# RozDavid/UnScene3D

Measured on AMD Instinct MI355X. Metric: training scenes/sec (Res16UNet34C+Mask3D, 150k voxels), higher is better.
Workload: dtype f32

## Files before the change

### include/usc3d.h

```cpp
#ifndef USC3D_H
#define USC3D_H

#include <stdint.h>

#ifdef __cplusplus
extern "C" {
#endif

typedef void* usc_stream_t;

enum usc_status {
  USC_OK = 0,
  USC_ERR_ARG = -1,
  USC_ERR_LAUNCH = -2,
  USC_ERR_RANGE = -3
};

const char* usc_last_error(void);
int usc_abi_version(void);
const char* usc_build_info(void);
int usc_device_count(void);


int usc_voxel_floor_f64(const double* xyz, int64_t n, double voxel_size,
// ... 167 lines not shown
int usc_conv_backward(const usc_kmap* m, int32_t kind, const float* x,
                      int32_t cin, const float* W, int32_t cout,
                      const float* dy, float* dx, int32_t dx_accumulate,
                      float* dW, int32_t dW_accumulate, void* ws,
                      int64_t ws_bytes, usc_stream_t s);
int usc_bn_eval_stats(const float* gamma, const float* beta,
                      const float* running_mean, const float* running_var,
                      float eps, int32_t c, float* mean, float* invstd,
                      float* scale, float* shift, usc_stream_t s);
int usc_conv_bn_act_forward(const usc_kmap* m, int32_t kind, const float* x,
                            int32_t cin, const float* W, int32_t cout,
                            const usc_bn* bn, const float* residual,
                            int32_t relu, float* y, float* stats, float* out,
                            void* ws, int64_t ws_bytes, usc_stream_t s);
int usc_conv_bn_act_backward(const usc_kmap* m, int32_t kind, const float* x,
                             int32_t cin, const float* W, int32_t cout,
                             const usc_bn* bn, const float* y,
                             const float* stats, const float* out_relu,
                             const float* dout, float* dy, float* dres,
                             float* dx, int32_t dx_accumulate, float* dW,
                             int32_t dW_accumulate, float* dgamma,
                             float* dbeta, int32_t dbn_accumulate, void* ws,
                             int64_t ws_bytes, usc_stream_t s);
int64_t usc_unit_bf16_ws_bytes(const usc_kmap* m, int32_t kind, int32_t cin,
                               int32_t cout);
int usc_conv_bn_act_forward_bf16(const usc_kmap* m, int32_t kind,
                                 const float* x, int32_t cin,
                                 const uint16_t* Wp, int32_t cout,
                                 const usc_bn* bn, const float* residual,
                                 int32_t relu, float* y, float* stats,
                                 float* out, void* ws, int64_t ws_bytes,
                                 usc_stream_t s);

int64_t usc_unit_split_ws_bytes(const usc_kmap* m, int32_t kind, int32_t cin,
                                int32_t cout, int32_t P);
int usc_conv_bn_act_forward_split(const usc_kmap* m, int32_t kind,
                                  const float* x, int32_t cin, const float* W,
                                  int32_t cout, int32_t P, const usc_bn* bn,
                                  const float* residual, int32_t relu, float* y,
                                  float* stats, float* out, void* ws,
                                  int64_t ws_bytes, usc_stream_t s);
int usc_conv_bn_act_backward_split(const usc_kmap* m, int32_t kind,
                                   const float* x, int32_t cin, const float* W,
                                   int32_t cout, int32_t P, const usc_bn* bn,
                                   const float* y, const float* stats,
                                   const float* out_relu, const float* dout,
                                   float* dy, float* dres, float* dx,
                                   int32_t dx_accumulate, float* dW,
                                   int32_t dW_accumulate, float* dgamma,
                                   float* dbeta, int32_t dbn_accumulate,
                                   void* ws, int64_t ws_bytes, usc_stream_t s);

enum usc_step_op { USC_STEP_UNIT_FWD = 0, USC_STEP_UNIT_BWD = 1, USC_STEP_CAT = 2, USC_STEP_SPLIT = 3, USC_STEP_ADD = 4,
                   USC_STEP_UNIT_FWD_BF16 = 5 };
typedef struct usc_step {
  int32_t op, kind, cin, cout, relu;
  int32_t dx_accumulate, dW_accumulate, dbn_accumulate, defer_wgrad, accumulate;
  const usc_kmap* map;
  const usc_bn* bn;
  const float* x;
  const float* W;
  const float* residual;
  float* y;
  float* stats;
  float* out;
  const float* dout;
  float* dy;
  float* dres;
  float* dx;
  float* dW;
  float* dgamma;
  float* dbeta;
  const float* a;
  const float* b;
  float* dst;
  float* dst2;
  int64_t n;
  int32_t ca, cb;
  int32_t split_planes, reserved;
} usc_step;
int32_t usc_step_size(void);
int64_t usc_program_ws_bytes(const usc_step* steps, int32_t n_steps);
int usc_program_run(const usc_step* steps, int32_t begin, int32_t end, void* ws, int64_t ws_bytes, usc_stream_t s);


int64_t usc_colstats_ws_bytes(int64_t n, int32_t c);
int usc_colstats(const float* x, const float* y, int64_t n, int32_t c,
                 double* sum1, double* sum2, void* ws, int64_t ws_bytes,
                 usc_stream_t s);
int usc_bn_forward_stats(const float* x, int64_t n, int32_t c, const float* gamma,
                         const float* beta, float eps, float momentum,
                         float* running_mean, float* running_var, int64_t* num_batches_tracked, float* mean,
                         float* invstd, float* scale, float* shift, void* ws,
                         int64_t ws_bytes, usc_stream_t s);
int usc_bn_apply(const float* x, const float* scale, const float* shift,
                 const float* residual, int32_t relu, float* y, int64_t n,
                 int32_t c, usc_stream_t s);
int usc_bn_backward_dx(const float* x, const float* dy, const float* y_out,
                       const float* mean, const float* invstd,
                       const float* gamma, const float* mean_g,
                       const float* mean_gxhat, float* dx, float* dres,
                       int64_t n, int32_t c, usc_stream_t s);
int64_t usc_bn_tile_max_rows(void);
int64_t usc_bn_plan(int64_t n, int32_t c, int32_t backward);
int usc_bn_tile_ok(int64_t n, int32_t c);
int64_t usc_bn_tile_ws_bytes(int32_t c);
int usc_bn_tile_forward(const float* partial, int32_t G, float* y, int64_t n,
                        int32_t c, const float* gamma, const float* beta,
                        float eps, float momentum, float* running_mean,
                        float* running_var, int64_t* num_batches_tracked,
                        float* mean, float* invstd, float* scale, float* shift,
                        const float* residual, int32_t relu, float* out,
                        void* ws, int64_t ws_bytes, usc_stream_t s);
int usc_bn_tile_backward(const float* partial, int32_t G, int32_t accumulate,
                         float* dout, const float* y, const float* y_out,
                         const float* mean, const float* invstd,
                         const float* gamma, int64_t n, int32_t c,
                         int32_t training, int32_t dbn_accumulate,
                         float* dgamma, float* dbeta, float* dy, float* dres,
                         void* ws, int64_t ws_bytes, usc_stream_t s);
int usc_bn_backward_reduce(const float* x, const float* dy, const float* y_out,
                           const float* mean, const float* invstd, int64_t n,
                           int32_t c, int32_t training, int32_t accumulate, float* dgamma,
                           float* dbeta, float* mean_g, float* mean_gxhat,
                           void* ws, int64_t ws_bytes, usc_stream_t s);
int usc_relu_fwd(const float* x, float* y, int64_t numel, usc_stream_t s);
int usc_relu_bwd(const float* y, const float* dy, float* dx, int64_t numel,
                 usc_stream_t s);

int usc_avgpool_down2(const float* in, int32_t c, const int32_t* nbr2,
                      int64_t n_coarse, float* out, usc_stream_t s);
int usc_avgpool_down2_ex(const float* in, int32_t c, int32_t ld,
                         const int64_t* row_of, const int32_t* nbr2,
                         int64_t n_coarse, float* out, uint8_t* mask_out,
                         usc_stream_t s);

int usc_gather_rows(const float* src, int32_t c, const int64_t* idx, int64_t n,
                    float* out, usc_stream_t s);

int usc_scatter_add_rows(const float* src, int32_t c, const int64_t* idx,
                         int64_t n, float* dst, usc_stream_t s);

int usc_scatter_rows_unique(const float* src, int32_t c, const int64_t* idx,
                            int64_t n, float* dst, usc_stream_t s);
int usc_scatter_rows_unique_add(const float* src, int32_t c, const int64_t* idx,
                                int64_t n, float* dst, usc_stream_t s);

int64_t usc_sample_keys_ws_bytes(int32_t n_scenes, int32_t K, int32_t q);
int usc_sample_keys(const float* feats, int32_t c, const uint8_t* mask, int32_t q, const float* pos, int32_t p,
                    const int64_t* idx, int32_t n_scenes, int32_t K, const int32_t* n_valid, float* out_feats,
                    uint8_t* out_mask, float* out_pos, void* ws, int64_t ws_bytes, usc_stream_t s);

int64_t usc_segment_csr_ws_bytes(int64_t n, int64_t S);
int usc_segment_csr(const int64_t* seg, int64_t n, int64_t S, int64_t* order,
                    int64_t* seg_off, void* ws, int64_t ws_bytes,
                    usc_stream_t s);
int usc_segment_mean_fwd(const float* src, int32_t c, const int64_t* order,
                         const int64_t* seg_off, int64_t S, float* out,
                         usc_stream_t s);
int usc_segment_mean_bwd(const float* dout, int32_t c, const int64_t* seg,
                         const int64_t* seg_off, int64_t n, float* dsrc,
                         usc_stream_t s);

int usc_segment_mean_nonzero(const float* feats, int32_t d,
                             const int64_t* order, const int64_t* seg_off,
                             int64_t S, float* out, int64_t* nonzero_cnt,
                             usc_stream_t s);
int usc_segment_max_nonzero(const float* feats, int32_t d,
                            const int64_t* order, const int64_t* seg_off,
                            int64_t S, float* out, int64_t* nonzero_cnt,
                            usc_stream_t s);

int32_t usc_attn_max_queries(void);
int32_t usc_attn_lse_stride(int32_t L);
int64_t usc_attn_ws_bytes(int32_t L, int32_t S, int32_t B, int32_t H);
int usc_attn_fwd(const float* q, const float* k, const float* v,
                 const uint8_t* mask, int32_t L, int32_t S, int32_t B, int32_t H,
                 int32_t E, float* o, float* lse, void* ws, int64_t ws_bytes,
                 usc_stream_t s);
int usc_attn_bwd(const float* q, const float* k, const float* v,
                 const uint8_t* mask, const float* o, const float* lse,
                 const float* dO, int32_t L, int32_t S, int32_t B, int32_t H,
                 int32_t E, float* dq, float* dk, float* dv,
                 int32_t mask_bits_in_ws ,
                 void* ws, int64_t ws_bytes, usc_stream_t s);

int usc_self_attn_fwd(const float* q, const float* k, const float* v, int32_t L,
                      int32_t B, int32_t H, int32_t E, float* o, float* lse,
                      usc_stream_t s);
int usc_self_attn_bwd(const float* q, const float* k, const float* v, const float* o,
                      const float* lse, const float* dO, int32_t L, int32_t B,
                      int32_t H, int32_t E, float* dq, float* dk, float* dv,
                      usc_stream_t s);

int usc_lsap_batch(const float* cost, int32_t n_prob, int32_t nr, int32_t nc,
                   int64_t* row_ind, int64_t* col_ind, int32_t* status, usc_stream_t s);

int64_t usc_criterion_ws_bytes(int32_t L, int32_t S, int32_t T);
int64_t usc_criterion_ws_bytes_q(int32_t L, int32_t S, int32_t T, int32_t Q);
int usc_criterion_target_bits(const uint8_t* tm, int32_t T, int32_t max_targets, int32_t S,
                              uint32_t* bits, int32_t* cnt, usc_stream_t s);
int usc_criterion_costs(const float* const* masks, int32_t L, int32_t ld, int32_t S,
                        int32_t Q, int32_t T, int32_t max_targets, const uint32_t* bits,
                        const int32_t* cnt, const float* logits, int64_t ls_level, int64_t ls_q,
                        int32_t C, const int64_t* labels, float w_mask, float w_class,
                        float w_dice, float* cost, float* cmask, float* cdice, float* nmat,
                        float* ssum, float* logp, void* ws, int64_t ws_bytes, usc_stream_t s);
int usc_criterion_drop_counts(const float* const* masks, int32_t L, int32_t ld, int32_t S,
                              int32_t Q, int32_t T, int32_t max_targets, const uint32_t* bits,
                              const int64_t* src, const int64_t* tid, int32_t* counts,
                              usc_stream_t s);
int usc_criterion_losses(const float* cmask, const float* cdice, const float* logp,
                         const int64_t* src, const int64_t* tid, const int64_t* labels,
                         const float* class_w, int32_t L, int32_t Q, int32_t T,
                         int32_t max_targets, int32_t C, int32_t noobj, int32_t* tcls, float* part,
                         const int32_t* counts, const int32_t* cnt, float thresh, float* wts,
                         usc_stream_t s);
int usc_criterion_table(const float* parts, int32_t B, int32_t L, float* table,
                        float* den_tot, usc_stream_t s);
int usc_criterion_backward(const float* const* masks, float* const* dmasks, int32_t L,
                           int32_t ld, int32_t S, int32_t Q, int32_t T, int32_t max_targets,
                           const uint32_t* bits, const int32_t* cnt, const int64_t* src,
                           const int64_t* tid, const float* nmat, const float* ssum,
                           const float* logp, const int32_t* tcls, const float* class_w,
                           const float* gtable, const float* den_tot, int32_t C, int64_t ls_level,
                           int64_t ls_q, float* dlogits, const float* wts, usc_stream_t s);

int usc_linear_fwd(const float* x, const float* W, const float* b, int32_t M,
                   int32_t N, int32_t K, float* y, usc_stream_t s);
int usc_linear_bwd(const float* dy, const float* x, const float* W, int32_t M,
                   int32_t N, int32_t K, float* dx, float* dW, float* db,
                   int32_t accumulate, usc_stream_t s);
int usc_linear_fwd_ex(const float* x, const float* x2, const float* W,
                      const float* b, int32_t M, int32_t N, int32_t K,
                      int32_t relu, float* y, usc_stream_t s);
int usc_linear_fwd_pad(const float* x, const float* x2, const float* W, const float* b, int32_t M, int32_t N, int32_t K,
                       int32_t relu, float* y, int32_t M_pad, usc_stream_t s);
int usc_linear_fwd_split(const float* x, const float* x2, const float* W, const float* b, int32_t M, int32_t N, int32_t K,
                         int32_t x2_cols, int32_t split_cols, float* y, usc_stream_t s);
int usc_linear_bwd_ex(const float* dy, const float* y_relu, const float* x,
                      const float* x2, const float* W, int32_t M, int32_t N,
                      int32_t K, float* dx, const float* dx_add, float* dW,
                      float* db, int32_t accumulate, usc_stream_t s);
int usc_linear_bwd_ex2(const float* dy, const float* y_relu, const float* x, const float* x2, const float* W, int32_t M,
                       int32_t N, int32_t K, float* dx, const float* dx_add, const float* dx_add2, float* dx_b, float* dW,
                       float* db, int32_t accumulate, usc_stream_t s);
int usc_qkv_proj_bwd(const float* dy3, const float* x, const float* pos, const float* W, int32_t M, int32_t E, float* dx,
                     float* dx_b, const float* dres, float* dW, float* db, int32_t accumulate, usc_stream_t s);
int64_t usc_col_sum_ws_bytes(int64_t n, int32_t c);
int usc_col_sum(const float* x, int64_t n, int32_t c, float* out,
                int32_t accumulate, void* ws, int64_t ws_bytes, usc_stream_t s);

int usc_layernorm_fwd(const float* x, const float* gamma, const float* beta,
                      int64_t rows, int32_t d, float eps, float* y, float* mean,
                      float* rstd, usc_stream_t s);
int usc_add_layernorm_fwd(const float* x, const float* res, const float* gamma,
                          const float* beta, int64_t rows, int32_t d, float eps,
                          float* y, float* sum_out, float* mean, float* rstd,
                          usc_stream_t s);
int64_t usc_layernorm_bwd_ws_bytes(int64_t rows, int32_t d);
int usc_layernorm_bwd(const float* dy, const float* x, const float* mean,
                      const float* rstd, const float* gamma, int64_t rows,
                      int32_t d, float* dx, float* dgamma, float* dbeta,
                      int32_t accumulate, void* ws, int64_t ws_bytes,
                      usc_stream_t s);
int usc_layernorm_bwd_ex(const float* dy, const float* x, const float* mean,
                         const float* rstd, const float* gamma, int64_t rows,
                         int32_t d, const float* dx_add, float* dx, float* dgamma,
                         float* dbeta, int32_t accumulate, void* ws,
                         int64_t ws_bytes, usc_stream_t s);

int usc_furthest_point_sampling(const float* xyz, int32_t b, int32_t n,
                                int32_t m, float* tmp, int32_t* idx,
                                usc_stream_t s);

int usc_fourier_posenc(const float* xyz, int64_t n, const float* lo,
                       const float* hi, const float* gauss_B, int32_t d,
                       float* out, usc_stream_t s);

int usc_ncut_similarity(const float* F, int64_t S, int32_t d,
                        int32_t cosine_mode, float* normed, float* sim,
                        usc_stream_t s);
int usc_ncut_similarity_masked(const float* F, const uint8_t* zero_rows, int64_t S,
                               int32_t d, int32_t cosine_mode, float* normed,
                               float* sim, usc_stream_t s);
int usc_ncut_normalize_mat(float* A, int64_t S, void* ws, int64_t ws_bytes,
                           usc_stream_t s);
int usc_ncut_binarize(const float* simA, const float* simB, int64_t S, float tau,
                      double eps, const uint8_t* painted, uint8_t* Abin,
                      double* deg, usc_stream_t s);
int64_t usc_ncut_fiedler_ws_bytes(int64_t S);
int usc_ncut_fiedler(const uint8_t* Abin, const double* deg, int64_t S, double eps,
                     double* evec, double* eval, void* ws, int64_t ws_bytes,
                     usc_stream_t s);
int usc_ncut_fiedler_ex(const uint8_t* Abin, const double* deg, int64_t S, double eps,
                        double* evec, double* eval, void* ws, int64_t ws_bytes,
                        usc_stream_t s, int32_t flags);
int32_t usc_ncut_fiedler_plan(int64_t S, int32_t cus, int32_t flags);

int usc_knn1(const float* query, int64_t nq, const float* ref, int64_t nr,
             int64_t* idx, float* dist2, usc_stream_t s);

int usc_cc_eps_init(int32_t* label, int64_t n, usc_stream_t s);
int usc_cc_eps_step(const float* xyz, int64_t n, float eps,
                    const int32_t* label_in, int32_t* label_out,
                    int32_t* changed, usc_stream_t s);
int usc_cc_eps_finish(const int32_t* label, int64_t n, int32_t* rank_ws,
                      int64_t* labels, usc_stream_t s);

int usc_project_planes_fwd(const int32_t* coords, const float* pred,
                           const float* target, int64_t V, int32_t inst,
                           int32_t dim_x, int32_t dim_y, int32_t dim_z,
                           float* pred_xy, float* pred_xz, float* pred_yz,
                           float* tgt_xy, float* tgt_xz, float* tgt_yz,
                           int32_t* cnt_xy, int32_t* cnt_xz, int32_t* cnt_yz,
                           usc_stream_t s);
int usc_project_planes_bwd(const int32_t* coords, int64_t V, int32_t inst,
                           int32_t dim_x, int32_t dim_y, int32_t dim_z,
                           const float* g_xy, const float* g_xz,
                           const float* g_yz, float* grad_pred,
                           usc_stream_t s);

int usc_brick_mask_build(const int32_t* coords, int64_t n, const int32_t* shift, int32_t B,
                         int32_t bricks_x, int32_t bricks_y, int32_t bricks_z,
                         uint32_t* mask, usc_stream_t s);
int usc_raycast_first_hit_map(const uint64_t* table_keys, const int32_t* table_vals,
                              int64_t cap, int64_t n_rows, const int32_t* shift,
                              const uint32_t* brick_mask , int32_t bricks_x,
                              int32_t bricks_y, int32_t bricks_z,
// ... 114 lines not shown
```

### unscene3d_amd/_lib.py

```python
from __future__ import annotations

import ctypes as C
import os

import torch

_HERE = os.path.dirname(os.path.abspath(__file__))
LIB_PATH = os.environ.get("USC3D_LIB") or os.path.join(_HERE, "libusc3d_hip.so")

_p = C.c_void_p
_i32 = C.c_int32
_i64 = C.c_int64
_f64 = C.c_double
_f32 = C.c_float

class KMap(C.Structure):
    _fields_ = [("nbr", _p), ("perm", _p), ("tile_mask", _p), ("pair_in", _p), ("pair_out", _p), ("koff", _p),
                ("n_in", _i64), ("n_out", _i64), ("pair_capacity", _i64), ("K", _i32), ("reserved", _i32)]


class BNDesc(C.Structure):
    _fields_ = [("gamma", _p), ("beta", _p), ("running_mean", _p), ("running_var", _p), ("num_batches_tracked", _p),
                ("eps", _f32), ("momentum", _f32), ("c", _i32), ("training", _i32)]


_kp = C.POINTER(KMap)
_bp = C.POINTER(BNDesc)


class Step(C.Structure):
    _fields_ = [("op", _i32), ("kind", _i32), ("cin", _i32), ("cout", _i32), ("relu", _i32),
                ("dx_accumulate", _i32), ("dW_accumulate", _i32), ("dbn_accumulate", _i32), ("defer_wgrad", _i32),
                ("accumulate", _i32),
                ("map", _p), ("bn", _p),
                ("x", _p), ("W", _p), ("residual", _p), ("y", _p), ("stats", _p), ("out", _p),
                ("dout", _p), ("dy", _p), ("dres", _p), ("dx", _p), ("dW", _p), ("dgamma", _p), ("dbeta", _p),
                ("a", _p), ("b", _p), ("dst", _p), ("dst2", _p), ("n", _i64), ("ca", _i32), ("cb", _i32),
                ("split_planes", _i32), ("reserved", _i32)]


_sp = C.POINTER(Step)
STEP_UNIT_FWD, STEP_UNIT_BWD, STEP_CAT, STEP_SPLIT, STEP_ADD, STEP_UNIT_FWD_BF16 = 0, 1, 2, 3, 4, 5

SIGNATURES = {
    "usc_last_error": (C.c_char_p, []),
    "usc_abi_version": (C.c_int, []),
    "usc_build_info": (C.c_char_p, []),
    "usc_device_count": (C.c_int, []),
    "usc_voxel_floor_f64": (C.c_int, [_p, _i64, _f64, _p, _p]),
    "usc_voxel_floor_f64_host": (C.c_int, [_p, _i64, C.c_double, _p]),
    "usc_unique_coords_host": (C.c_int, [_p, _i64, _i32, _p, _p, _p]),
    "usc_coordmap_capacity": (_i64, [_i64]),
    "usc_coordmap_ws_bytes": (_i64, [_i64]),
    "usc_coordmap_build": (C.c_int, [_p, _i64, _i32, _p, _p, _i64, _p, _p, _p, _p, _p, _i64, _p]),
    "usc_morton_cell_ids": (C.c_int, [_p, _i64, _i32, _i32, _i32, _i32, _i32, _p, _p]),
    "usc_kernel_map_cube": (C.c_int, [_p, _i64, _i32, _i32, _p, _p, _i64, _p, _p]),
    "usc_kernel_map_down2": (C.c_int, [_p, _i64, _i32, _p, _p, _i64, _p, _p, _p]),
    "usc_rulebook_ws_bytes": (_i64, [_i64, _i64]),
    "usc_rulebook_compact": (C.c_int, [_p, _i64, _i64, _p, _p, _p, _p, _i64, _p]),
    "usc_weight_transpose": (C.c_int, [_p, _i32, _i32, _i32, _i32, _p, _p]),
    "usc_spconv_plan": (C.c_int, [_i32, _i64, _i32, _i32, _i32]),
    "usc_spconv_gather_gemm_ws_bytes": (_i64, [_i64, _i32, _i32, _i32]),
    "usc_spconv_gather_gemm": (C.c_int, [_p, _i64, _i32, _p, _i32, _i32, _p, _i64, _p, _p, _i32, _i32, _p, _i64, _p]),
    "usc_rowsort_ws_bytes": (_i64, [_i32, _i64]),
    "usc_rowsort_build": (C.c_int, [_p, _i32, _i64, _p, _p, _p, _i64, _p]),
    "usc_spconv_sorted_ws_bytes": (_i64, [_i64, _i32, _i32, _i32]),
    "usc_spconv_sorted_gemm": (C.c_int, [_p, _i64, _i32, _p, _i32, _i32, _p, _p, _p, _i64, _p, _p, _i32, _i32, _p, _i64, _p]),
    "usc_spconv_sorted_gemm_ex": (C.c_int, [_p, _i64, _i32, _p, _i32, _i32, _p, _p, _p, _i64, _p, _p, _i32, _i32, _p, _i64, _p, _p]),
    "usc_group_reduce": (C.c_int, [_p, _i32, _i64, _i32, _p, _i32, _p, _p]),
    "usc_bn_tile_max_rows": (C.c_int64, []),
    "usc_bn_plan": (_i64, [_i64, _i32, _i32]),
    "usc_bn_tile_ok": (C.c_int, [_i64, _i32]),
    "usc_bn_tile_ws_bytes": (C.c_int64, [_i32]),
    "usc_bn_tile_forward": (C.c_int, [_p, _i32, _p, _i64, _i32, _p, _p, _f32, _f32, _p, _p, _p, _p, _p, _p, _p, _p, _i32, _p,
                                      _p, _i64, _p]),
    "usc_bn_tile_backward": (C.c_int, [_p, _i32, _i32, _p, _p, _p, _p, _p, _p, _i64, _i32, _i32, _i32, _p, _p, _p, _p, _p,
                                       _i64, _p]),
    "usc_spconv_pairs_gemm": (C.c_int, [_p, _i32, _p, _i32, _i32, _p, _p, _p, _i64, _p, _p]),
    "usc_cast_bf16": (C.c_int, [_p, _i64, _p, _p]),
    "usc_spconv_pack_w_bf16": (C.c_int, [_p, _i32, _i32, _i32, _p, _p]),
    "usc_spconv_gather_gemm_bf16_ws_bytes": (_i64, [_i64, _i32, _i32, _i32]),
    "usc_spconv_gather_gemm_bf16": (C.c_int, [_p, _i64, _i32, _p, _i32, _i32, _p, _i64, _p, _p, _i32, _p, _i64, _p]),
    "usc_split_bf16_rows": (C.c_int, [_p, _i64, _i32, _i32, _p, _p]),
    "usc_split_bf16": (C.c_int, [_p, _i64, _i32, _p, _p]),
    "usc_spconv_pack_w_split": (C.c_int, [_p, _i32, _i32, _i32, _i32, _i32, _p, _p]),
    "usc_spconv_gather_gemm_split_ws_bytes": (_i64, [_i64, _i32, _i32, _i32, _i32]),
    "usc_spconv_gather_gemm_split": (C.c_int, [_p, _i64, _i32, _p, _i32, _i32, _i32, _p, _i64, _p, _p, _i32, _p, _i64, _p]),
    "usc_spconv_wgrad_ws_bytes": (_i64, [_i32, _i32, _i32]),
    "usc_spconv_wgrad": (C.c_int, [_p, _i32, _p, _i32, _i32, _p, _p, _p, _i64, _p, _i32, _p, _i64, _p]),
    "usc_spconv_wgrad_ws_bytes_rows": (_i64, [_i32, _i32, _i32, _i64]),
    "usc_step_size": (_i32, []),
    "usc_program_ws_bytes": (_i64, [_sp, _i32]),
    "usc_program_run": (C.c_int, [_sp, _i32, _i32, _p, _i64, _p]),
    "usc_spconv_wgrad_group_max": (_i32, []),
    "usc_spconv_wgrad_grid_limit": (None, [_i32]),
    "usc_spconv_wgrad_group_ok": (C.c_int, [_i32, _i32, _i32, _i32, _i64]),
    "usc_spconv_wgrad_group": (C.c_int, [_i32, _p, _p, _p, _i32, _i32, _i32, _p, _p, _p, _i64, _i32, _p]),
    "usc_spconv_wgrad_table_ws_bytes": (_i64, [_i32, _i32, _i32]),
    "usc_spconv_wgrad_table": (C.c_int, [_p, _i32, _p, _i32, _p, _i32, _i64, _p, _i32, _p, _i64, _p]),
    "usc_set_wgrad_lane": (C.c_int, [_p, _p, _i64, _i64]),
    "usc_wgrad_lane_join": (C.c_int, [_p]),
    "usc_wgrad_lane_hold": (C.c_int, [_i32, _i64, _i64, _p]),
    "usc_wgrad_lane_holding": (_i32, []),
    "usc_launch_stats_begin": (C.c_int, [_p, _i64, _p]),
    "usc_launch_stats_end": (_i64, [_p, _i64]),
    "usc_wall_clock_khz": (_i64, []),
    "usc_conv_ws_bytes": (_i64, [_kp, _i32, _i32, _i32]),
    "usc_unit_ws_bytes": (_i64, [_kp, _i32, _i32, _i32]),
    "usc_conv_forward": (C.c_int, [_kp, _i32, _p, _i32, _p, _i32, _p, _p, _p, _i64, _p]),
    "usc_conv_backward": (C.c_int, [_kp, _i32, _p, _i32, _p, _i32, _p, _p, _i32, _p, _i32, _p, _i64, _p]),
    "usc_bn_eval_stats": (C.c_int, [_p, _p, _p, _p, _f32, _i32, _p, _p, _p, _p, _p]),
    "usc_conv_bn_act_forward": (C.c_int, [_kp, _i32, _p, _i32, _p, _i32, _bp, _p, _i32, _p, _p, _p, _p, _i64, _p]),
    "usc_unit_bf16_ws_bytes": (_i64, [_kp, _i32, _i32, _i32]),
    "usc_conv_bn_act_forward_bf16": (C.c_int, [_kp, _i32, _p, _i32, _p, _i32, _bp, _p, _i32, _p, _p, _p, _p, _i64, _p]),
    "usc_unit_split_ws_bytes": (_i64, [_kp, _i32, _i32, _i32, _i32]),
    "usc_conv_bn_act_forward_split": (C.c_int, [_kp, _i32, _p, _i32, _p, _i32, _i32, _bp, _p, _i32, _p, _p, _p, _p, _i64, _p]),
    "usc_conv_bn_act_backward_split": (C.c_int, [_kp, _i32, _p, _i32, _p, _i32, _i32, _bp, _p, _p, _p, _p, _p, _p, _p, _i32, _p,
                                                 _i32, _p, _p, _i32, _p, _i64, _p]),
    "usc_conv_bn_act_backward": (C.c_int, [_kp, _i32, _p, _i32, _p, _i32, _bp, _p, _p, _p, _p, _p, _p, _p, _i32, _p,
                                           _i32, _p, _p, _i32, _p, _i64, _p]),
    "usc_colstats_ws_bytes": (_i64, [_i64, _i32]),
    "usc_colstats": (C.c_int, [_p, _p, _i64, _i32, _p, _p, _p, _i64, _p]),
    "usc_bn_apply": (C.c_int, [_p, _p, _p, _p, _i32, _p, _i64, _i32, _p]),
    "usc_bn_backward_dx": (C.c_int, [_p, _p, _p, _p, _p, _p, _p, _p, _p, _p, _i64, _i32, _p]),
    "usc_bn_backward_reduce": (C.c_int, [_p, _p, _p, _p, _p, _i64, _i32, _i32, _i32, _p, _p, _p, _p, _p, _i64, _p]),
    "usc_bn_forward_stats": (C.c_int, [_p, _i64, _i32, _p, _p, _f32, _f32, _p, _p, _p, _p, _p, _p, _p, _p, _i64, _p]),
    "usc_relu_fwd": (C.c_int, [_p, _p, _i64, _p]),
    "usc_relu_bwd": (C.c_int, [_p, _p, _p, _i64, _p]),
    "usc_avgpool_down2": (C.c_int, [_p, _i32, _p, _i64, _p, _p]),
    "usc_avgpool_down2_ex": (C.c_int, [_p, _i32, _i32, _p, _p, _i64, _p, _p, _p]),
    "usc_gather_rows": (C.c_int, [_p, _i32, _p, _i64, _p, _p]),
    "usc_scatter_add_rows": (C.c_int, [_p, _i32, _p, _i64, _p, _p]),
    "usc_scatter_rows_unique": (C.c_int, [_p, _i32, _p, _i64, _p, _p]),
    "usc_scatter_rows_unique_add": (C.c_int, [_p, _i32, _p, _i64, _p, _p]),
    "usc_sample_keys_ws_bytes": (_i64, [_i32, _i32, _i32]),
    "usc_sample_keys": (C.c_int, [_p, _i32, _p, _i32, _p, _i32, _p, _i32, _i32, _p, _p, _p, _p, _p, _i64, _p]),
    "usc_segment_csr_ws_bytes": (_i64, [_i64, _i64]),
    "usc_segment_csr": (C.c_int, [_p, _i64, _i64, _p, _p, _p, _i64, _p]),
    "usc_segment_mean_fwd": (C.c_int, [_p, _i32, _p, _p, _i64, _p, _p]),
    "usc_segment_mean_bwd": (C.c_int, [_p, _i32, _p, _p, _i64, _p, _p]),
    "usc_segment_mean_nonzero": (C.c_int, [_p, _i32, _p, _p, _i64, _p, _p, _p]),
    "usc_segment_max_nonzero": (C.c_int, [_p, _i32, _p, _p, _i64, _p, _p, _p]),
    "usc_ncut_similarity": (C.c_int, [_p, _i64, _i32, _i32, _p, _p, _p]),
    "usc_ncut_similarity_masked": (C.c_int, [_p, _p, _i64, _i32, _i32, _p, _p, _p]),
    "usc_ncut_normalize_mat": (C.c_int, [_p, _i64, _p, _i64, _p]),
    "usc_ncut_binarize": (C.c_int, [_p, _p, _i64, _f32, _f64, _p, _p, _p, _p]),
    "usc_ncut_fiedler_ws_bytes": (_i64, [_i64]),
    "usc_ncut_fiedler": (C.c_int, [_p, _p, _i64, _f64, _p, _p, _p, _i64, _p]),
    "usc_ncut_fiedler_ex": (C.c_int, [_p, _p, _i64, _f64, _p, _p, _p, _i64, _p, _i32]),
    "usc_ncut_fiedler_plan": (_i32, [_i64, _i32, _i32]),
    "usc_knn1": (C.c_int, [_p, _i64, _p, _i64, _p, _p, _p]),
    "usc_cc_eps_init": (C.c_int, [_p, _i64, _p]),
    "usc_cc_eps_step": (C.c_int, [_p, _i64, _f32, _p, _p, _p, _p]),
    "usc_cc_eps_finish": (C.c_int, [_p, _i64, _p, _p, _p]),
    "usc_project_planes_fwd": (C.c_int, [_p, _p, _p, _i64, _i32, _i32, _i32, _i32] + [_p] * 10),
    "usc_project_planes_bwd": (C.c_int, [_p, _i64, _i32, _i32, _i32, _i32, _p, _p, _p, _p, _p]),
    "usc_brick_mask_build": (C.c_int, [_p, _i64, _p, _i32, _i32, _i32, _i32, _p, _p]),
    "usc_raycast_first_hit_map": (C.c_int, [_p, _p, _i64, _i64, _p, _p, _i32, _i32, _i32, _p, _p, _i32, _i32, _i32, _i32,
                                            _f32, _f32, _f32, _p, _p, _p]),
    "usc_raycast_first_hit_dense": (C.c_int, [_p, _i32, _i32, _i32, _i64, _p, _p, _i32, _i32, _i32, _i32, _f32, _f32,
                                              _f32, _p, _p, _p]),
    "usc_project_reduce": (C.c_int, [_p, _i32, _p, _p, _i64, _i32, _p, _p, _p]),
    "usc_project_fuse_tokens": (C.c_int, [_p, _i32, _i32, _i32, _i32, _i32, _i32, _p, _p, _i64, _p, _p, _p]),
    "usc_project_predictions": (C.c_int, [_p, _i32, _p, _i64, _p, _p]),
    "usc_unproject_depth": (C.c_int, [_p, _p, _p, _i32, _i32, _i32, _p, _p]),
    "usc_spin": (C.c_int, [_i64, C.c_int, _p]),
    "usc_adamw_step": (C.c_int, [_p, _p, _p, _p, _i64, _f32, _f32, _f32, _f32, _f32, _i64, _p]),
    "usc_adamw_step_scaled": (C.c_int, [_p, _p, _p, _p, _i64, _f32, _i32, _f32, _f32, _f32, _f32, _f32, _i64, _p]),
    "usc_elastic_displace": (C.c_int, [_p, _i32, _i64, _i32, _p, _i32, _i32, _i32, _p, _p, _p, _f64, _p, _p]),
    "usc_attn_max_queries": (_i32, []),
    "usc_attn_lse_stride": (_i32, [_i32]),
    "usc_attn_ws_bytes": (_i64, [_i32, _i32, _i32, _i32]),
    "usc_attn_fwd": (C.c_int, [_p, _p, _p, _p, _i32, _i32, _i32, _i32, _i32, _p, _p, _p, _i64, _p]),
    "usc_attn_bwd": (C.c_int, [_p, _p, _p, _p, _p, _p, _p, _i32, _i32, _i32, _i32, _i32, _p, _p, _p, _i32, _p, _i64, _p]),
    "usc_lsap_batch": (C.c_int, [_p, _i32, _i32, _i32, _p, _p, _p, _p]),
    "usc_criterion_ws_bytes": (_i64, [_i32, _i32, _i32]),
    "usc_criterion_ws_bytes_q": (_i64, [_i32, _i32, _i32, _i32]),
    "usc_criterion_target_bits": (C.c_int, [_p, _i32, _i32, _i32, _p, _p, _p]),
    "usc_criterion_costs": (C.c_int, [_p, _i32, _i32, _i32, _i32, _i32, _i32, _p, _p, _p, _i64, _i64, _i32, _p, _f32, _f32,
                                      _f32, _p, _p, _p, _p, _p, _p, _p, _i64, _p]),
    "usc_criterion_drop_counts": (C.c_int, [_p, _i32, _i32, _i32, _i32, _i32, _i32, _p, _p, _p, _p, _p]),
    "usc_criterion_losses": (C.c_int, [_p, _p, _p, _p, _p, _p, _p, _i32, _i32, _i32, _i32, _i32, _i32, _p, _p, _p, _p,
                                       _f32, _p, _p]),
    "usc_criterion_table": (C.c_int, [_p, _i32, _i32, _p, _p, _p]),
    "usc_criterion_backward": (C.c_int, [_p, _p, _i32, _i32, _i32, _i32, _i32, _i32, _p, _p, _p, _p, _p, _p, _p, _p, _p,
                                         _p, _p, _i32, _i64, _i64, _p, _p, _p]),
    "usc_self_attn_fwd": (C.c_int, [_p, _p, _p, _i32, _i32, _i32, _i32, _p, _p, _p]),
    "usc_self_attn_bwd": (C.c_int, [_p, _p, _p, _p, _p, _p, _i32, _i32, _i32, _i32, _p, _p, _p, _p]),
    "usc_linear_fwd": (C.c_int, [_p, _p, _p, _i32, _i32, _i32, _p, _p]),
    "usc_linear_bwd": (C.c_int, [_p, _p, _p, _i32, _i32, _i32, _p, _p, _p, _i32, _p]),
    "usc_layernorm_fwd": (C.c_int, [_p, _p, _p, _i64, _i32, _f32, _p, _p, _p, _p]),
    "usc_add_layernorm_fwd": (C.c_int, [_p, _p, _p, _p, _i64, _i32, _f32, _p, _p, _p, _p, _p]),
    "usc_linear_fwd_ex": (C.c_int, [_p, _p, _p, _p, _i32, _i32, _i32, _i32, _p, _p]),
    "usc_linear_fwd_pad": (C.c_int, [_p, _p, _p, _p, _i32, _i32, _i32, _i32, _p, _i32, _p]),
    "usc_linear_fwd_split": (C.c_int, [_p, _p, _p, _p, _i32, _i32, _i32, _i32, _i32, _p, _p]),
    "usc_linear_bwd_ex": (C.c_int, [_p, _p, _p, _p, _p, _i32, _i32, _i32, _p, _p, _p, _p, _i32, _p]),
    "usc_qkv_proj_bwd": (C.c_int, [_p, _p, _p, _p, _i32, _i32, _p, _p, _p, _p, _p, _i32, _p]),
    "usc_linear_bwd_ex2": (C.c_int, [_p, _p, _p, _p, _p, _i32, _i32, _i32, _p, _p, _p, _p, _p, _p, _i32, _p]),
    "usc_layernorm_bwd_ws_bytes": (_i64, [_i64, _i32]),
    "usc_layernorm_bwd": (C.c_int, [_p, _p, _p, _p, _p, _i64, _i32, _p, _p, _p, _i32, _p, _i64, _p]),
    "usc_layernorm_bwd_ex": (C.c_int, [_p, _p, _p, _p, _p, _i64, _i32, _p, _p, _p, _p, _i32, _p, _i64, _p]),
    "usc_affine_rows": (C.c_int, [_p, _i32, _i64, _i32, _p, _p, _p]),
    "usc_colsum_sequential": (C.c_int, [_p, _i64, _i32, _i32, _p, _p]),
    "usc_col_sum_ws_bytes": (_i64, [_i64, _i32]),
    "usc_col_sum": (C.c_int, [_p, _i64, _i32, _p, _i32, _p, _i64, _p]),
    "usc_color_lut": (C.c_int, [_p, _i64, _i32, _p, _p, _i32, _p]),
    "usc_felz_face_normals": (C.c_int, [_p, _p, _i64, _p, _p]),
    "usc_felz_vertex_normals": (C.c_int, [_p, _p, _p, _i64, _p, _p]),
    "usc_felz_edge_weights": (C.c_int, [_p, _p, _p, _p, _i64, _p, _p, _p, _p]),
    "usc_felz_merge_host": (C.c_int, [_p, _p, _p, _i64, _i32, _f32, _i32, _p]),
    "usc_furthest_point_sampling": (C.c_int, [_p, _i32, _i32, _i32, _p, _p, _p]),
    "usc_fourier_posenc": (C.c_int, [_p, _i64, _p, _p, _p, _i32, _p, _p]),
    "usc_mask_gt_overlap": (C.c_int, [_p, _i64, _i32, _i64, _p, _i32, _p, _p]),
    "usc_vit_attn_head_dim": (_i32, []),
    "usc_vit_attn_fwd": (C.c_int, [_p, _i32, _i32, _i32, _f32, _i32, _p, _p]),
    "usc_instance_index": (C.c_int, [_p, _i64, _i32, _p, _i32, _p, _p, _p, _p]),
    "usc_instance_select": (C.c_int, [_p, _i64, _i32, _p, _i32, _p, _p, _p, _i32, _i64, _p, _p, _p, _p]),
    "usc_instance_masks": (C.c_int, [_p, _i64, _p, _i32, _i32, _p, _p, _i32, _i64, _p, _p]),
    "usc_freemask_normalize": (C.c_int, [_p, _i64, _i32, _p, _p, _p]),
    "usc_freemask_ws_bytes": (_i64, [_i64, _i64]),
    "usc_freemask_rowstats": (C.c_int, [_p, _p, _i64, _p, _p, _i64, _i32, _p, _p, _p, _i64, _p]),
    "usc_freemask_bits": (C.c_int, [_p, _p, _i64, _p, _p, _p, _i64, _i32, _p, _p, _f32, _p, _p, _p, _p, _i64, _p]),
    "usc_freemask_soft_rows": (C.c_int, [_p, _p, _i64, _p, _p, _p, _i64, _i32, _p, _p, _p, _i32, _p, _p]),
    "usc_mask_bits_extent": (C.c_int, [_p, _i64, _i64, _p, _p, _p, _p]),
    "usc_mask_bits_nms_ws_bytes": (_i64, [_i64]),
    "usc_mask_bits_nms": (C.c_int, [_p, _p, _i64, _p, _i32, _f32, _p, _p, _i64, _p]),
    "usc_mask_bits_max_segments": (_i32, []),
    "usc_maxpool_down2_i32": (C.c_int, [_p, _i64, _p, _i64, _p, _p]),
    "usc_mask_bits_components": (C.c_int, [_p, _i64, _i32, _p, _i32, _p, _p, _p, _p, _p]),
    "usc_mask_bits_split": (C.c_int, [_p, _i32, _i32, _p, _p, _p, _p, _i64, _p, _p, _p, _p, _p, _p, _p, _p]),
    "usc_mask_bits_nms_weighted": (C.c_int, [_p, _p, _p, _i64, _p, _i32, _f32, _p, _p, _i64, _p]),
}


class LaunchStat(C.Structure):
    _fields_ = [("n_out", _i64), ("cin", _i32), ("cout", _i32), ("K", _i32), ("nb", _i32)]


def _load():
    if not os.path.exists(LIB_PATH):
        raise ImportError(
            f"{LIB_PATH} is missing: build the HIP extension first "
            "(`python -c 'import __graft_entry__ as g; g.build()'`). "
            "unscene3d_amd has no CPU fallback."
        )
    lib = C.CDLL(LIB_PATH)
    for name, (res, args) in SIGNATURES.items():
        fn = getattr(lib, name)
        fn.restype = res
        fn.argtypes = args
    return lib


lib = _load()
if lib.usc_step_size() != C.sizeof(Step):
    raise ImportError(f"unscene3d_amd._lib.Step ({C.sizeof(Step)} bytes) does not mirror usc_step "
                      f"({lib.usc_step_size()} bytes): rebuild the library or fix the binding")


def last_error() -> str:
    return lib.usc_last_error().decode("utf-8", "replace")


def check(rc: int, what: str = "") -> None:
    if rc != 0:
        raise RuntimeError(f"{what or 'libusc3d_hip'} failed (status {rc}): {last_error()}")


def require_device() -> None:
    n = lib.usc_device_count()
    if n <= 0:
        raise RuntimeError(
            "unscene3d_amd: no HIP device visible — the MI355X kernels cannot run and there is no CPU fallback"
        )
```

### unscene3d_amd/csrc/coords.hip

```cpp
#include "common.h"
#include "scan.h"

#include <stdarg.h>

namespace usc {

static thread_local char g_err[512] = "";

void set_error(const char* fmt, ...) {
  va_list ap;
  va_start(ap, fmt);
  vsnprintf(g_err, sizeof(g_err), fmt, ap);
  va_end(ap);
}

__global__ void voxel_floor_kernel(const double* __restrict__ xyz, int64_t n3, double voxel,
                                   int32_t* __restrict__ out) {
  for (int64_t i = (int64_t)blockIdx.x * blockDim.x + threadIdx.x; i < n3;
       i += (int64_t)gridDim.x * blockDim.x) {
    out[i] = (int32_t)floor(xyz[i] / voxel);
  }
}

__global__ void fill_i32_kernel(int32_t* p, int64_t n, int32_t v) {
// ... 97 lines not shown
  const int64_t o = (int64_t)blockIdx.x * blockDim.x + threadIdx.x;
  if (o >= n) return;
  const int4 c = *reinterpret_cast<const int4*>(coords + 4 * o);
  const int r = ksize / 2;
  int k = 0;
  for (int dz = -r; dz <= r; ++dz)
    for (int dy = -r; dy <= r; ++dy)
      for (int dx = -r; dx <= r; ++dx, ++k) {
        int v;
        if (dx == 0 && dy == 0 && dz == 0) {
          v = (int)o;
        } else {
          const int x = c.y + dx * ts, y = c.z + dy * ts, z = c.w + dz * ts;
          v = coord_in_range(c.x, x, y, z) ? table_lookup(keys, vals, cap, pack_key(c.x, x, y, z)) : -1;
        }
        nbr[(int64_t)k * n + o] = v;
      }
}

__global__ __launch_bounds__(256) void kernel_map_down2_kernel(const int32_t* __restrict__ fine, int64_t n_fine, int ts,
                                                              const int64_t* __restrict__ parent,
                                                              const int32_t* __restrict__ coarse, int64_t n_coarse,
                                                              int32_t* __restrict__ nbr2, uint8_t* __restrict__ kidx) {
  const int64_t i = (int64_t)blockIdx.x * blockDim.x + threadIdx.x;
  if (i >= n_fine) return;
  const int64_t p = parent[i];
  const int4 cf = *reinterpret_cast<const int4*>(fine + 4 * i);
  const int4 cc = *reinterpret_cast<const int4*>(coarse + 4 * p);
  const int ox = (cf.y - cc.y) / ts, oy = (cf.z - cc.z) / ts, oz = (cf.w - cc.w) / ts;
  const int k = ox + 2 * oy + 4 * oz;
  nbr2[(int64_t)k * n_coarse + p] = (int32_t)i;
  kidx[i] = (uint8_t)k;
}

__device__ inline uint32_t spread3(uint32_t v) {
  v &= 0x3ffu;
  v = (v | (v << 16)) & 0x030000FFu;
  v = (v | (v << 8)) & 0x0300F00Fu;
  v = (v | (v << 4)) & 0x030C30C3u;
  v = (v | (v << 2)) & 0x09249249u;
  return v;
}
__global__ __launch_bounds__(256) void morton_cells_kernel(const int32_t* __restrict__ coords, int64_t n, int shift,
                                                          int lox, int loy, int loz, int bits, int64_t* __restrict__ ids) {
  const int64_t i = (int64_t)blockIdx.x * blockDim.x + threadIdx.x;
  if (i >= n) return;
  const int4 c = *reinterpret_cast<const int4*>(coords + 4 * i);
  const uint32_t x = (uint32_t)((c.y - lox) >> shift), y = (uint32_t)((c.z - loy) >> shift),
                 z = (uint32_t)((c.w - loz) >> shift);
  const uint32_t m = spread3(x) | (spread3(y) << 1) | (spread3(z) << 2);
  ids[i] = ((int64_t)c.x << (3 * bits)) | (int64_t)(m & ((1u << (3 * bits)) - 1u));
}

struct NbrFlag {
  const int32_t* nbr;
  __device__ int operator()(int64_t j) const { return nbr[j] >= 0 ? 1 : 0; }
};
struct PairEmit {
  const int32_t* nbr;
  int64_t n_out;
  int32_t* in_idx;
  int32_t* out_idx;
  int64_t* koff;
  __device__ void operator()(int64_t j, int64_t pos, int flag) const {
    const int64_t k = j / n_out, o = j - k * n_out;
    if (o == 0) koff[k] = pos;
    if (flag) {
      in_idx[pos] = nbr[j];
      out_idx[pos] = (int32_t)o;
    }
  }
};
__global__ void store_total_kernel(const int64_t* __restrict__ total, int64_t* __restrict__ dst) {
  if (threadIdx.x == 0 && blockIdx.x == 0) *dst = *total;
}

}

using namespace usc;

extern "C" {

const char* usc_last_error(void) { return g_err; }
int usc_abi_version(void) { return 4; }

int usc_device_count(void) {
  int n = 0;
  hipError_t e = hipGetDeviceCount(&n);
  if (e != hipSuccess) {
    set_error("hipGetDeviceCount: %s", hipGetErrorString(e));
    return USC_ERR_LAUNCH;
  }
  return n;
}

int usc_voxel_floor_f64(const double* xyz, int64_t n, double voxel_size, int32_t* coords_out, usc_stream_t s) {
  USC_REQUIRE(n >= 0 && voxel_size > 0, "usc_voxel_floor_f64: bad n/voxel_size");
  if (n == 0) return USC_OK;
  USC_REQUIRE(xyz && coords_out, "usc_voxel_floor_f64: null pointer");
  hipLaunchKernelGGL(voxel_floor_kernel, dim3(stream_grid(n * 3, 256)), dim3(256), 0, as_stream(s), xyz, n * 3,
                     voxel_size, coords_out);
  USC_CHECK_LAUNCH("usc_voxel_floor_f64");
  return USC_OK;
}

int64_t usc_coordmap_capacity(int64_t n) {
  int64_t cap = 1024;
  while (cap < 2 * n) cap <<= 1;
  return cap;
}

static int64_t coordmap_fixed_ws(int64_t n) {
  return align_up(n * 4, 16) * 2 + 16;
}
int64_t usc_coordmap_ws_bytes(int64_t n) { return coordmap_fixed_ws(n) + scan_ws_bytes(n); }

int usc_coordmap_build(const int32_t* coords, int64_t n, int32_t quant, uint64_t* table_keys, int32_t* table_vals,
                       int64_t cap, int64_t* unique_idx, int64_t* inverse, int32_t* out_coords, int64_t* n_out,
                       void* ws, int64_t ws_bytes, usc_stream_t s) {
  USC_REQUIRE(n >= 0, "usc_coordmap_build: negative n");
  USC_REQUIRE(table_keys && table_vals && n_out && ws, "usc_coordmap_build: null pointer");
  USC_REQUIRE(n == 0 || (coords && unique_idx && inverse), "usc_coordmap_build: null pointer");
  USC_REQUIRE(cap >= usc_coordmap_capacity(n) && (cap & (cap - 1)) == 0,
              "usc_coordmap_build: table capacity %lld too small / not a power of two for n=%lld", (long long)cap,
              (long long)n);
  USC_REQUIRE(ws_bytes >= usc_coordmap_ws_bytes(n), "usc_coordmap_build: workspace too small");
  USC_REQUIRE(n < (1ll << 31), "usc_coordmap_build: n exceeds int32 rows");
  hipStream_t st = as_stream(s);
  char* w = (char*)ws;
  int32_t* slots = (int32_t*)w;
  int32_t* rank_of_row = (int32_t*)(w + align_up(n * 4, 16));
  int32_t* errflag = (int32_t*)(w + align_up(n * 4, 16) * 2);
  void* scan_ws = w + coordmap_fixed_ws(n);
  int64_t nb = scan_num_blocks(n);

  (void)hipMemsetAsync(table_keys, 0xFF, (size_t)cap * 8, st);
  hipLaunchKernelGGL(fill_i32_kernel, dim3(stream_grid(cap, 256)), dim3(256), 0, st, table_vals, cap, 0x7fffffff);
  (void)hipMemsetAsync(errflag, 0, 16, st);
  if (n > 0) {
    const unsigned g = (unsigned)ceil_div(n, 256);
    hipLaunchKernelGGL(coordmap_insert_kernel, dim3(g), dim3(256), 0, st, coords, n, (int)quant, table_keys,
                       table_vals, cap, slots, errflag);
    FirstOccFlag f{slots, table_vals};
    UniqueEmit e{coords, (int)quant, unique_idx, out_coords, rank_of_row};
    device_exclusive_scan(f, e, n, scan_ws, st);
    hipLaunchKernelGGL(coordmap_inverse_kernel, dim3(g), dim3(256), 0, st, slots, table_vals, rank_of_row, n,
                       inverse);
    hipLaunchKernelGGL(coordmap_finalize_kernel, dim3(g), dim3(256), 0, st, slots, table_vals, rank_of_row, n);
  } else {
    (void)hipMemsetAsync(scan_ws, 0, (size_t)scan_ws_bytes(0), st);
  }
  hipLaunchKernelGGL(coordmap_count_kernel, dim3(1), dim3(64), 0, st, (const int64_t*)scan_ws + nb, errflag, n_out);
  USC_CHECK_LAUNCH("usc_coordmap_build");
  return USC_OK;
}

int usc_kernel_map_cube(const int32_t* coords, int64_t n, int32_t tensor_stride, int32_t ksize,
                        const uint64_t* table_keys, const int32_t* table_vals, int64_t cap, int32_t* nbr,
                        usc_stream_t s) {
  USC_REQUIRE(n >= 0 && tensor_stride >= 1, "usc_kernel_map_cube: bad n/tensor_stride");
  USC_REQUIRE(ksize == 3 || ksize == 1 || ksize == 5, "usc_kernel_map_cube: unsupported kernel size %d", ksize);
  if (n == 0) return USC_OK;
  USC_REQUIRE(coords && table_keys && table_vals && nbr, "usc_kernel_map_cube: null pointer");
  hipLaunchKernelGGL(kernel_map_cube_kernel, dim3((unsigned)ceil_div(n, 256)), dim3(256), 0, as_stream(s), coords, n,
                     (int)tensor_stride, (int)ksize, table_keys, table_vals, cap, nbr);
  USC_CHECK_LAUNCH("usc_kernel_map_cube");
  return USC_OK;
// ... 50 lines not shown
```

### unscene3d_amd/csrc/decoder.hip

```cpp
#include "common.h"

namespace usc {
namespace {

constexpr int kLnMaxPerLane = 8;

template <int PER>
__global__ __launch_bounds__(256) void layernorm_fwd_kernel(const float* __restrict__ x, const float* __restrict__ res,
                                                           const float* __restrict__ gamma,
                                                           const float* __restrict__ beta, int64_t rows, int d, float eps,
                                                           float* __restrict__ y, float* __restrict__ sum_out,
                                                           float* __restrict__ mean, float* __restrict__ rstd) {
  const int lane = threadIdx.x & 63;
  const int64_t r = (int64_t)blockIdx.x * 4 + (threadIdx.x >> 6);
  if (r >= rows) return;
  float v[PER];
  float s = 0.f;
#pragma unroll
  for (int j = 0; j < PER; ++j) {
    v[j] = x[r * d + lane + 64 * j];
    if (res) {
      v[j] += res[r * d + lane + 64 * j];
      sum_out[r * d + lane + 64 * j] = v[j];
    }
// ... 187 lines not shown

}

namespace usc {
namespace {

typedef float f32x16 __attribute__((ext_vector_type(16)));
#define MFMA32(a, b, c) __builtin_amdgcn_mfma_f32_32x32x2f32((a), (b), (c), 0, 0, 0)
__device__ inline int acc_row16(int reg, int half) { return (reg & 3) + 8 * (reg >> 2) + 4 * half; }

__device__ inline void tile_reduce_store(f32x16 acc, float (*red)[16][64], int wave, int lane, float* __restrict__ out,
                                         int64_t ld, int row0, int col0, int max_row, const float* __restrict__ bias,
                                         int accumulate = 0, int relu = 0, const float* __restrict__ add = nullptr,
                                         const float* __restrict__ add2 = nullptr, float* __restrict__ out_b = nullptr,
                                         int zero_rows_to = 0) {
#pragma unroll
  for (int r = 0; r < 16; ++r) red[wave][r][lane] = acc[r];
  __syncthreads();
  const int i = lane & 31, h = lane >> 5;
#pragma unroll
  for (int q = 0; q < 4; ++q) {
    const int r = 4 * wave + q;
    const float v = red[0][r][lane] + red[1][r][lane] + red[2][r][lane] + red[3][r][lane];
    const int row = row0 + acc_row16(r, h);
    if (row < max_row) {
      float* dst = out + (int64_t)row * ld + col0 + i;
      float o = v + (bias ? bias[col0 + i] : 0.f) + (accumulate ? *dst : 0.f);
      if (add) o += add[(int64_t)row * ld + col0 + i];
      if (out_b) out_b[(int64_t)row * ld + col0 + i] = o;
      if (add2) o += add2[(int64_t)row * ld + col0 + i];
      *dst = relu ? fmaxf(o, 0.f) : o;
    } else if (row < zero_rows_to) {
      out[(int64_t)row * ld + col0 + i] = 0.f;
    }
  }
}

__global__ __launch_bounds__(256) void linear_fwd_kernel(const float* __restrict__ x, const float* __restrict__ x2,
                                                        const float* __restrict__ W, const float* __restrict__ b, int M,
                                                        int N, int K, int relu, float* __restrict__ y, int Mpad,
                                                        int x2_cols, int split) {
  __shared__ float red[4][16][64];
  const int lane = threadIdx.x & 63, wave = threadIdx.x >> 6, i = lane & 31, h = lane >> 5;
  const int n0 = blockIdx.x * 32, m0 = blockIdx.y * 32;
  const int m = m0 + i;
  const float* xa = x + (int64_t)(m < M ? m : 0) * K + 4 * h;
  const float* xa2 = (x2 && n0 < x2_cols) ? x2 + (int64_t)(m < M ? m : 0) * K + 4 * h : nullptr;
  const float* wb = W + (int64_t)(n0 + i) * K + 4 * h;
  const float keep = m < M ? 1.f : 0.f;
  f32x16 acc;
#pragma unroll
  for (int r = 0; r < 16; ++r) acc[r] = 0.f;
  const int nchunk = K >> 5;
  for (int c = wave; c < nchunk; c += 4) {
    const int k0 = c * 32;
    float4 a[4], bb[4];
#pragma unroll
    for (int t = 0; t < 4; ++t) { a[t] = *reinterpret_cast<const float4*>(xa + k0 + 8 * t); bb[t] = *reinterpret_cast<const float4*>(wb + k0 + 8 * t); }
    if (xa2) {
#pragma unroll
      for (int t = 0; t < 4; ++t) {
        const float4 e = *reinterpret_cast<const float4*>(xa2 + k0 + 8 * t);
        a[t].x += e.x; a[t].y += e.y; a[t].z += e.z; a[t].w += e.w;
      }
    }
#pragma unroll
    for (int t = 0; t < 4; ++t) {
      const float av[4] = {a[t].x * keep, a[t].y * keep, a[t].z * keep, a[t].w * keep};
      const float bv[4] = {bb[t].x, bb[t].y, bb[t].z, bb[t].w};
#pragma unroll
      for (int j = 0; j < 4; ++j) acc = MFMA32(av[j], bv[j], acc);
    }
  }
  if (split > 0) {
    const int j = n0 / split;
    tile_reduce_store(acc, red, wave, lane, y + (int64_t)j * M * split, split, m0, n0 - j * split, M,
                      b ? b + j * split : nullptr, 0, relu);
    return;
  }
  tile_reduce_store(acc, red, wave, lane, y, N, m0, n0, M, b, 0, relu, nullptr, nullptr, nullptr, Mpad);
}

template <bool EX>
__device__ inline void linear_dx_tile(const float* __restrict__ dy, const float* __restrict__ ymask,
                                      const float* __restrict__ W, int M, int N, int K, float* __restrict__ dx,
                                      const float* __restrict__ dx_add, const float* __restrict__ dx_add2,
                                      float* __restrict__ dx_b, int c0, int m0, float (*red)[16][64]) {
  const int lane = threadIdx.x & 63, wave = threadIdx.x >> 6, i = lane & 31, h = lane >> 5;
  const int m = m0 + i;
  const float* ya = dy + (int64_t)(m < M ? m : 0) * N + 4 * h;
  const float* ym = (EX && ymask) ? ymask + (int64_t)(m < M ? m : 0) * N + 4 * h : nullptr;
  const float* wb = W + (int64_t)(4 * h) * K + c0 + i;
  const float keep = m < M ? 1.f : 0.f;
  f32x16 acc;
#pragma unroll
  for (int r = 0; r < 16; ++r) acc[r] = 0.f;
  const int nchunk = N >> 5;
  float4 a[4], an[4];
  float bv[16], bn[16];
  auto load = [&](int c, float4* aa, float* bb) __attribute__((always_inline)) {
    const int n0 = c * 32;
#pragma unroll
    for (int t = 0; t < 4; ++t) aa[t] = *reinterpret_cast<const float4*>(ya + n0 + 8 * t);
    if (EX && ym) {
#pragma unroll
      for (int t = 0; t < 4; ++t) {
        const float4 o = *reinterpret_cast<const float4*>(ym + n0 + 8 * t);
        aa[t].x = o.x > 0.f ? aa[t].x : 0.f; aa[t].y = o.y > 0.f ? aa[t].y : 0.f;
        aa[t].z = o.z > 0.f ? aa[t].z : 0.f; aa[t].w = o.w > 0.f ? aa[t].w : 0.f;
      }
    }
#pragma unroll
    for (int t = 0; t < 4; ++t)
#pragma unroll
      for (int j = 0; j < 4; ++j) bb[4 * t + j] = wb[(int64_t)(n0 + 8 * t + j) * K];
  };
  int c = wave;
  if (c < nchunk) load(c, an, bn);
  for (; c < nchunk; c += 4) {
#pragma unroll
    for (int t = 0; t < 4; ++t) a[t] = an[t];
#pragma unroll
    for (int q = 0; q < 16; ++q) bv[q] = bn[q];
    if (c + 4 < nchunk) load(c + 4, an, bn);
#pragma unroll
    for (int t = 0; t < 4; ++t) {
      const float av[4] = {a[t].x * keep, a[t].y * keep, a[t].z * keep, a[t].w * keep};
#pragma unroll
      for (int j = 0; j < 4; ++j) acc = MFMA32(av[j], bv[4 * t + j], acc);
    }
  }
  tile_reduce_store(acc, red, wave, lane, dx, K, m0, c0, M, nullptr, 0, 0, EX ? dx_add : nullptr,
                    EX ? dx_add2 : nullptr, EX ? dx_b : nullptr);
}

template <bool EX>
__device__ inline void linear_dw_tile(const float* __restrict__ dy, const float* __restrict__ ymask,
                                      const float* __restrict__ x, const float* __restrict__ x2, int M, int N, int K,
                                      int accumulate, float* __restrict__ dW, float* __restrict__ db, int c0, int n0,
                                      float (*red)[16][64], float (*bred)[32]) {
  const int lane = threadIdx.x & 63, wave = threadIdx.x >> 6, i = lane & 31, h = lane >> 5;
  f32x16 acc;
#pragma unroll
  for (int r = 0; r < 16; ++r) acc[r] = 0.f;
  float bsum = 0.f;
  for (int mb = wave * 32; mb < M; mb += 128) {
    float av[16], bv[16];
#pragma unroll
    for (int t = 0; t < 4; ++t)
#pragma unroll
      for (int j = 0; j < 4; ++j) {
        const int m = mb + 8 * t + 4 * h + j;
        const bool ok = m < M;
        av[4 * t + j] = ok ? dy[(int64_t)m * N + n0 + i] : 0.f;
        bv[4 * t + j] = ok ? x[(int64_t)m * K + c0 + i] : 0.f;
      }
    if (EX && ymask) {
      float ov[16];
#pragma unroll
      for (int t = 0; t < 4; ++t)
#pragma unroll
        for (int j = 0; j < 4; ++j) {
          const int m = mb + 8 * t + 4 * h + j;
          ov[4 * t + j] = m < M ? ymask[(int64_t)m * N + n0 + i] : 1.f;
        }
#pragma unroll
      for (int q = 0; q < 16; ++q) av[q] = ov[q] > 0.f ? av[q] : 0.f;
    }
    if (EX && x2) {
      float ev[16];
#pragma unroll
      for (int t = 0; t < 4; ++t)
#pragma unroll
        for (int j = 0; j < 4; ++j) {
          const int m = mb + 8 * t + 4 * h + j;
          ev[4 * t + j] = m < M ? x2[(int64_t)m * K + c0 + i] : 0.f;
        }
#pragma unroll
      for (int q = 0; q < 16; ++q) bv[q] += ev[q];
    }
#pragma unroll
    for (int q = 0; q < 16; ++q) { acc = MFMA32(av[q], bv[q], acc); bsum += av[q]; }
  }
  const bool want_b = db && c0 == 0;
  if (want_b) {
    bsum += __shfl_xor(bsum, 32, 64);
    if (h == 0) bred[wave][i] = bsum;
  }
  tile_reduce_store(acc, red, wave, lane, dW, K, n0, c0, N, nullptr, accumulate);
  if (want_b && threadIdx.x < 32) {
    const float v = bred[0][threadIdx.x] + bred[1][threadIdx.x] + bred[2][threadIdx.x] + bred[3][threadIdx.x];
    db[n0 + threadIdx.x] = accumulate ? db[n0 + threadIdx.x] + v : v;
  }
}

template <bool EX>
__global__ __launch_bounds__(256) void linear_bwd_kernel(const float* __restrict__ dy, const float* __restrict__ ymask,
                                                        const float* __restrict__ x, const float* __restrict__ x2,
                                                        const float* __restrict__ W, int M, int N, int K, int dx_tiles,
                                                        int accumulate, float* __restrict__ dx,
                                                        const float* __restrict__ dx_add,
                                                        const float* __restrict__ dx_add2, float* __restrict__ dx_b,
                                                        float* __restrict__ dW, float* __restrict__ db) {
  __shared__ float red[4][16][64];
  __shared__ float bred[4][32];
  const int kt = K / 32;
  int b = blockIdx.x;
  if (b < dx_tiles) {
    linear_dx_tile<EX>(dy, ymask, W, M, N, K, dx, dx_add, dx_add2, dx_b, (b % kt) * 32, (b / kt) * 32, red);
  } else {
    b -= dx_tiles;
    linear_dw_tile<EX>(dy, ymask, x, x2, M, N, K, accumulate, dW, db, (b % kt) * 32, (b / kt) * 32, red, bred);
  }
}


__device__ inline void tile_reduce4(f32x16 acc, float (*red)[16][64], int wave, int lane, float (&out)[4]) {
#pragma unroll
  for (int r = 0; r < 16; ++r) red[wave][r][lane] = acc[r];
  __syncthreads();
#pragma unroll
  for (int q = 0; q < 4; ++q) {
    const int r = 4 * wave + q;
    out[q] = red[0][r][lane] + red[1][r][lane] + red[2][r][lane] + red[3][r][lane];
  }
  __syncthreads();
}

__global__ __launch_bounds__(256) void qkv_bwd_kernel(const float* __restrict__ dy3, const float* __restrict__ x,
                                                     const float* __restrict__ pos, const float* __restrict__ W, int M,
                                                     int E, int dx_tiles, int accumulate, float* __restrict__ dx,
                                                     float* __restrict__ dx_b, const float* __restrict__ dres,
                                                     float* __restrict__ dW, float* __restrict__ db) {
  __shared__ float red[4][16][64];
  __shared__ float bred[4][32];
  const int kt = E / 32;
  int b = blockIdx.x;
  if (b >= dx_tiles) {
    b -= dx_tiles;
    const int c0 = (b % kt) * 32, n0 = (b / kt) * 32, j = n0 / E;
    linear_dw_tile<true>(dy3 + (int64_t)j * M * E, nullptr, x, j < 2 ? pos : nullptr, M, E, E, accumulate,
                         dW + (int64_t)j * E * E, db ? db + j * E : nullptr, c0, n0 - j * E, red, bred);
    return;
  }
  const int lane = threadIdx.x & 63, wave = threadIdx.x >> 6, i = lane & 31, h = lane >> 5;
  const int c0 = (b % kt) * 32, m0 = (b / kt) * 32;
  const int m = m0 + i;
  const float keep = m < M ? 1.f : 0.f;
  f32x16 acc_qk, acc_v;
#pragma unroll
  for (int r = 0; r < 16; ++r) acc_qk[r] = acc_v[r] = 0.f;
#pragma unroll
  for (int j = 0; j < 3; ++j) {
    const float* ya = dy3 + ((int64_t)j * M + (m < M ? m : 0)) * E + 4 * h;
    const float* wb = W + ((int64_t)j * E + 4 * h) * E + c0 + i;
    for (int c = wave; c < kt; c += 4) {
      const int n0 = c * 32;
      float4 a[4];
      float bv[16];
#pragma unroll
      for (int t = 0; t < 4; ++t) a[t] = *reinterpret_cast<const float4*>(ya + n0 + 8 * t);
#pragma unroll
      for (int t = 0; t < 4; ++t)
#pragma unroll
        for (int jj = 0; jj < 4; ++jj) bv[4 * t + jj] = wb[(int64_t)(n0 + 8 * t + jj) * E];
#pragma unroll
      for (int t = 0; t < 4; ++t) {
        const float av[4] = {a[t].x * keep, a[t].y * keep, a[t].z * keep, a[t].w * keep};
#pragma unroll
        for (int jj = 0; jj < 4; ++jj) {
          if (j < 2) acc_qk = MFMA32(av[jj], bv[4 * t + jj], acc_qk);
          else acc_v = MFMA32(av[jj], bv[4 * t + jj], acc_v);
        }
      }
    }
  }
  float qk[4], vv[4];
  tile_reduce4(acc_qk, red, wave, lane, qk);
  tile_reduce4(acc_v, red, wave, lane, vv);
#pragma unroll
  for (int q = 0; q < 4; ++q) {
    const int row = m0 + acc_row16(4 * wave + q, h);
    if (row < M) {
      const int64_t o = (int64_t)row * E + c0 + i;
      if (dx_b) dx_b[o] = qk[q];
      float t = qk[q] + vv[q];
      if (dres) t += dres[o];
      dx[o] = t;
    }
  }
}

constexpr int kColSumRows = 64;
__global__ __launch_bounds__(256) void col_sum_partial_kernel(const float* __restrict__ x, int64_t n, int c,
                                                             float* __restrict__ partial) {
  __shared__ float red[4][64];
  const int tx = threadIdx.x & 63, ty = threadIdx.x >> 6;
  const int col = blockIdx.y * 64 + tx;
  const int64_t r0 = (int64_t)blockIdx.x * kColSumRows;
  float a[4] = {0.f, 0.f, 0.f, 0.f};
  if (col < c) {
#pragma unroll
    for (int q = 0; q < 4; ++q)
#pragma unroll
      for (int u = 0; u < 4; ++u) {
        const int64_t r = r0 + 16 * u + 4 * q + ty;
        if (r < n) a[u] += x[r * c + col];
      }
  }
  red[ty][tx] = (a[0] + a[1]) + (a[2] + a[3]);
  __syncthreads();
  if (ty == 0 && col < c) partial[(int64_t)blockIdx.x * c + col] = ((red[0][tx] + red[1][tx]) + red[2][tx]) + red[3][tx];
}

__global__ __launch_bounds__(256) void col_sum_final_kernel(const float* __restrict__ partial, int64_t parts, int c,
                                                           int accumulate, float* __restrict__ out) {
  __shared__ float red[16][17];
  const int tx = threadIdx.x & 15, ty = threadIdx.x >> 4;
  const int col = blockIdx.x * 16 + tx;
  float s = 0.f;
  if (col < c)
    for (int64_t p = ty; p < parts; p += 16) s += partial[p * c + col];
  red[ty][tx] = s;
  __syncthreads();
  if (ty == 0 && col < c) {
    float t = 0.f;
#pragma unroll
    for (int l = 0; l < 16; ++l) t += red[l][tx];
    out[col] = accumulate ? out[col] + t : t;
  }
}

}
}

extern "C" {

int usc_linear_fwd(const float* x, const float* W, const float* b, int32_t M, int32_t N, int32_t K, float* y,
                   usc_stream_t s) {
  return usc_linear_fwd_ex(x, nullptr, W, b, M, N, K, 0, y, s);
}

int usc_linear_fwd_ex(const float* x, const float* x2, const float* W, const float* b, int32_t M, int32_t N, int32_t K,
                      int32_t relu, float* y, usc_stream_t s) {
  return usc_linear_fwd_pad(x, x2, W, b, M, N, K, relu, y, M, s);
}

int usc_linear_fwd_pad(const float* x, const float* x2, const float* W, const float* b, int32_t M, int32_t N, int32_t K,
                       int32_t relu, float* y, int32_t M_pad, usc_stream_t s) {
  USC_REQUIRE(M >= 1 && N >= 32 && N % 32 == 0 && K >= 32 && K % 32 == 0, "usc_linear_fwd: N, K must be multiples of 32");
  USC_REQUIRE(M_pad >= M, "usc_linear_fwd_pad: M_pad < M");
  USC_REQUIRE(x && W && y, "usc_linear_fwd: null pointer");
  hipLaunchKernelGGL(usc::linear_fwd_kernel, dim3(N / 32, (M_pad + 31) / 32), dim3(256), 0, usc::as_stream(s), x, x2, W, b,
                     (int)M, (int)N, (int)K, (int)relu, y, (int)M_pad, (int)N, 0);
  USC_CHECK_LAUNCH("usc_linear_fwd");
  return USC_OK;
}

int usc_linear_fwd_split(const float* x, const float* x2, const float* W, const float* b, int32_t M, int32_t N, int32_t K,
                         int32_t x2_cols, int32_t split_cols, float* y, usc_stream_t s) {
  USC_REQUIRE(M >= 1 && N >= 32 && N % 32 == 0 && K >= 32 && K % 32 == 0, "usc_linear_fwd: N, K must be multiples of 32");
  USC_REQUIRE(split_cols >= 32 && split_cols % 32 == 0 && N % split_cols == 0 && x2_cols >= 0 && x2_cols % 32 == 0,
              "usc_linear_fwd_split: split_cols / x2_cols must be multiples of 32, split_cols a divisor of N");
  USC_REQUIRE(x && W && y, "usc_linear_fwd: null pointer");
  hipLaunchKernelGGL(usc::linear_fwd_kernel, dim3(N / 32, (M + 31) / 32), dim3(256), 0, usc::as_stream(s), x, x2, W, b,
                     (int)M, (int)N, (int)K, 0, y, (int)M, (int)x2_cols, (int)split_cols);
  USC_CHECK_LAUNCH("usc_linear_fwd");
  return USC_OK;
}

int usc_linear_bwd(const float* dy, const float* x, const float* W, int32_t M, int32_t N, int32_t K, float* dx, float* dW,
                   float* db, int32_t accumulate, usc_stream_t s) {
  return usc_linear_bwd_ex2(dy, nullptr, x, nullptr, W, M, N, K, dx, nullptr, nullptr, nullptr, dW, db, accumulate, s);
}

int usc_linear_bwd_ex(const float* dy, const float* y_relu, const float* x, const float* x2, const float* W, int32_t M,
                      int32_t N, int32_t K, float* dx, const float* dx_add, float* dW, float* db, int32_t accumulate,
                      usc_stream_t s) {
  return usc_linear_bwd_ex2(dy, y_relu, x, x2, W, M, N, K, dx, dx_add, nullptr, nullptr, dW, db, accumulate, s);
}

int usc_linear_bwd_ex2(const float* dy, const float* y_relu, const float* x, const float* x2, const float* W, int32_t M,
                       int32_t N, int32_t K, float* dx, const float* dx_add, const float* dx_add2, float* dx_b, float* dW,
                       float* db, int32_t accumulate, usc_stream_t s) {
  USC_REQUIRE(M >= 1 && N >= 32 && N % 32 == 0 && K >= 32 && K % 32 == 0, "usc_linear_bwd: N, K must be multiples of 32");
  USC_REQUIRE(dy && x && W, "usc_linear_bwd: null pointer");
  USC_REQUIRE(dx || !(dx_add || dx_add2 || dx_b), "usc_linear_bwd: dx_add / dx_add2 / dx_b need dx");
  USC_REQUIRE(dW || !db, "usc_linear_bwd: db is computed inside the dW tiles, it needs dW");
  hipStream_t st = usc::as_stream(s);
  const int dx_tiles = dx ? (K / 32) * ((M + 31) / 32) : 0;
  const int dw_tiles = dW ? (K / 32) * (N / 32) : 0;
  if (dx_tiles + dw_tiles > 0) {
    if (y_relu || x2 || dx_add || dx_add2 || dx_b)
      hipLaunchKernelGGL(usc::linear_bwd_kernel<true>, dim3(dx_tiles + dw_tiles), dim3(256), 0, st, dy, y_relu, x, x2, W,
                         (int)M, (int)N, (int)K, dx_tiles, (int)accumulate, dx, dx_add, dx_add2, dx_b, dW, db);
    else
      hipLaunchKernelGGL(usc::linear_bwd_kernel<false>, dim3(dx_tiles + dw_tiles), dim3(256), 0, st, dy, y_relu, x, x2, W,
                         (int)M, (int)N, (int)K, dx_tiles, (int)accumulate, dx, dx_add, dx_add2, dx_b, dW, db);
  }
  USC_CHECK_LAUNCH("usc_linear_bwd");
  return USC_OK;
}

int usc_qkv_proj_bwd(const float* dy3, const float* x, const float* pos, const float* W, int32_t M, int32_t E, float* dx,
                     float* dx_b, const float* dres, float* dW, float* db, int32_t accumulate, usc_stream_t s) {
  USC_REQUIRE(M >= 1 && E >= 32 && E % 32 == 0, "usc_qkv_proj_bwd: E must be a multiple of 32");
  USC_REQUIRE(dy3 && x && W && dx && dW, "usc_qkv_proj_bwd: null pointer");
  const int dx_tiles = (E / 32) * ((M + 31) / 32);
  const int dw_tiles = (E / 32) * (3 * E / 32);
  hipLaunchKernelGGL(usc::qkv_bwd_kernel, dim3(dx_tiles + dw_tiles), dim3(256), 0, usc::as_stream(s), dy3, x, pos, W, (int)M,
                     (int)E, dx_tiles, (int)accumulate, dx, dx_b, dres, dW, db);
  USC_CHECK_LAUNCH("usc_qkv_proj_bwd");
  return USC_OK;
}

int64_t usc_col_sum_ws_bytes(int64_t n, int32_t c) {
  const int64_t parts = n > 0 ? (n + usc::kColSumRows - 1) / usc::kColSumRows : 0;
  return parts * (c > 0 ? c : 0) * 4;
}

int usc_col_sum(const float* x, int64_t n, int32_t c, float* out, int32_t accumulate, void* ws, int64_t ws_bytes,
                usc_stream_t s) {
  USC_REQUIRE(n >= 0 && c >= 1, "usc_col_sum: bad sizes");
  USC_REQUIRE(out && (n == 0 || (x && ws)), "usc_col_sum: null pointer");
  USC_REQUIRE(ws_bytes >= usc_col_sum_ws_bytes(n, c), "usc_col_sum: workspace too small");
  hipStream_t st = usc::as_stream(s);
  const int64_t parts = n > 0 ? (n + usc::kColSumRows - 1) / usc::kColSumRows : 0;
  const unsigned cg = (unsigned)((c + 63) / 64);
  if (parts > 0)
    hipLaunchKernelGGL(usc::col_sum_partial_kernel, dim3((unsigned)parts, cg), dim3(256), 0, st, x, n, (int)c, (float*)ws);
  hipLaunchKernelGGL(usc::col_sum_final_kernel, dim3((unsigned)((c + 15) / 16)), dim3(256), 0, st, (const float*)ws, parts,
                     (int)c, (int)accumulate, out);
  USC_CHECK_LAUNCH("usc_col_sum");
  return USC_OK;
}

}
```

### unscene3d_amd/csrc/units.hip

```cpp
#include <stdlib.h>

#include <vector>

#include "common.h"

namespace usc { bool tile_rows_ok(int64_t n, int c); }

using namespace usc;

namespace {

struct WsCursor {
  char* base; int64_t bytes; int64_t off;
  void* take(int64_t n) {
    n = align_up(n > 0 ? n : 16, 256);
    if (off + n > bytes) return nullptr;
    void* p = base + off;
    off += n;
    return p;
  }
  int64_t left() const { return bytes - off; }
  void* rest() { return base + off; }
};

// ... 2 lines not shown
}
inline bool sorted_ok(const usc_kmap* m, int cin, int cout) {
  return m->nbr && m->perm && m->tile_mask && m->K > 1 && m->K <= 32 && cin % 32 == 0 && cout % 32 == 0 && cin <= 4096;
}

struct TableGemmPlan {
  bool sorted;
  int64_t wt_bytes;
  int64_t gemm_bytes;
};
TableGemmPlan plan_table_gemm(const usc_kmap* m, int64_t n_out, int cin, int cout, int K, bool wt) {
  const bool compact = m->nbr && table_is_compact(n_out, cin, cout, K);
  if (sorted_ok(m, cin, cout) && !compact) return {true, 0, usc_spconv_sorted_ws_bytes(n_out, cin, cout, K)};
  return {false, wt && !compact ? (int64_t)K * cin * cout * 4 : 0, usc_spconv_gather_gemm_ws_bytes(n_out, cin, cout, K)};
}

int64_t table_gemm_ws(const usc_kmap* m, int64_t n_out, int cin, int cout, int K, bool wt) {
  const TableGemmPlan pl = plan_table_gemm(m, n_out, cin, cout, K, wt);
  return align_up(pl.wt_bytes, 256) + align_up(pl.gemm_bytes, 256);
}

struct Slices { const float* partial = nullptr; int G = 0; };

int table_gemm(const usc_kmap* m, const float* in, int64_t n_in, int cin, const float* W, int K, int cout, int64_t n_out,
               const float* bias, float* out, int accumulate, int wt, WsCursor ws, usc_stream_t s, Slices* left = nullptr) {
  if (left) *left = Slices{};
  if (n_out == 0) return USC_OK;
  const TableGemmPlan pl = plan_table_gemm(m, n_out, cin, cout, K, wt != 0);
  if (pl.wt_bytes > 0) {
    float* Wt = (float*)ws.take(pl.wt_bytes);
    USC_REQUIRE(Wt, "usc unit: workspace too small (weight transpose)");
    int rc = usc_weight_transpose(W, K, cout, cin, K > 1 ? 1 : 0, Wt, s);
    if (rc) return rc;
    W = Wt;
    wt = 0;
  }
  const int64_t b = pl.gemm_bytes;
  void* w = b > 0 ? ws.take(b) : nullptr;
  USC_REQUIRE(b == 0 || w, "usc unit: workspace too small (%s gemm)", pl.sorted ? "sorted" : "gather");
  if (!pl.sorted) return usc_spconv_gather_gemm(in, n_in, cin, W, K, cout, m->nbr, n_out, bias, out, accumulate, wt, w, b, s);
  int32_t G = 0;
  const int rc = usc_spconv_sorted_gemm_ex(in, n_in, cin, W, K, cout, m->nbr, m->perm, m->tile_mask, n_out, bias, out,
                                           accumulate, wt, w, b, left ? &G : nullptr, s);
  if (!rc && left && G > 0) { left->partial = (const float*)w; left->G = G; }
  return rc;
}

struct ConvShape { int64_t n_in, n_out; };
inline ConvShape conv_shape(const usc_kmap* m, int kind) {
  return kind == USC_CONV_UP ? ConvShape{m->n_out, m->n_in} : ConvShape{m->n_in, m->n_out};
}

struct WgradJob {
  const float* x; const float* dy; float* dW;
  const int32_t* a_idx; const int32_t* b_idx; const int64_t* koff;
  int64_t rows; int cin, cout, K;
  int64_t list_bytes;
  const int32_t* nbr; int64_t n_out, table_bytes;
};
WgradJob wgrad_job(const usc_kmap* m, int kind, ConvShape sh, const float* x, const float* dy, float* dW, int cin, int cout) {
  WgradJob j{};
  j.x = x; j.dy = dy; j.dW = dW; j.cin = cin; j.cout = cout;
  if (m->nbr) {
    const bool up = kind == USC_CONV_UP;
    j.a_idx = up ? m->pair_out : m->pair_in;
    j.b_idx = up ? m->pair_in : m->pair_out;
    j.koff = m->koff; j.K = m->K; j.rows = m->pair_capacity;
  } else {
    j.K = 1; j.rows = sh.n_in;
  }
  j.list_bytes = usc_spconv_wgrad_ws_bytes_rows(m->K, cin, cout, j.rows);
  if (kind == USC_CONV_SAME && m->nbr && cin <= 4 && cout == 32 && m->K <= 32) {
    j.nbr = m->nbr; j.n_out = sh.n_out;
    j.table_bytes = usc_spconv_wgrad_table_ws_bytes(m->K, cin, cout);
  }
  return j;
}
int issue_wgrad(const WgradJob& j, int accumulate, void* ws, int64_t ws_bytes, usc_stream_t s) {
  if (j.nbr && j.table_bytes <= ws_bytes)
    return usc_spconv_wgrad_table(j.x, j.cin, j.dy, j.cout, j.nbr, j.K, j.n_out, j.dW, accumulate, ws, j.table_bytes, s);
  return usc_spconv_wgrad(j.x, j.cin, j.dy, j.cout, j.K, j.a_idx, j.b_idx, j.koff, j.rows, j.dW, accumulate, ws, j.list_bytes, s);
}

struct Lane { hipStream_t st = nullptr; hipEvent_t fork = nullptr, join = nullptr; void* ws = nullptr; int64_t ws_bytes = 0;
              int64_t max_rows = 0; bool dirty = false;
              bool hold = false; int64_t hold_min_rows = 0, release_max_rows = 0; std::vector<WgradJob> held; };
Lane g_lane[16];
Lane* lane_for_current_device() {
  int dev = 0;
  if (hipGetDevice(&dev) != hipSuccess || dev < 0 || dev >= 16) return nullptr;
  return g_lane[dev].st ? &g_lane[dev] : nullptr;
}

int lane_release(Lane* lane, usc_stream_t s) {
  lane->hold = false;
  if (lane->held.empty()) return USC_OK;
  if (hipEventRecord(lane->fork, as_stream(s)) != hipSuccess || hipStreamWaitEvent(lane->st, lane->fork, 0) != hipSuccess) {
    lane->held.clear();
    set_error("usc wgrad lane: releasing the held weight gradients failed (event)");
    return USC_ERR_LAUNCH;
  }
  int rc = USC_OK;
  lane->dirty = true;
  for (size_t i = 0; i < lane->held.size() && !rc; ++i)
    rc = issue_wgrad(lane->held[i], 1, lane->ws, lane->ws_bytes, (usc_stream_t)lane->st);
  lane->held.clear();
  return rc;
}

int check_map(const usc_kmap* m, int kind, int cin, int cout, const char* who) {
  USC_REQUIRE(m, "%s: null kernel map", who);
  USC_REQUIRE(kind == USC_CONV_SAME || kind == USC_CONV_DOWN || kind == USC_CONV_UP, "%s: unknown conv kind %d", who, kind);
  USC_REQUIRE(cin >= 1 && cout >= 1 && m->K >= 1 && m->n_in >= 0 && m->n_out >= 0, "%s: bad sizes", who);
  USC_REQUIRE(m->nbr || (m->K == 1 && kind == USC_CONV_SAME), "%s: K>1 needs a neighbour table", who);
  USC_REQUIRE(kind != USC_CONV_SAME || m->n_in == m->n_out, "%s: a stride-1 map has n_in == n_out", who);
  return USC_OK;
}

__global__ __launch_bounds__(256) void cat_cols_kernel(const float4* __restrict__ a, int ca4, const float4* __restrict__ b,
                                                      int cb4, float4* __restrict__ dst, int64_t total4) {
  const int c4 = ca4 + cb4;
  for (int64_t e = (int64_t)blockIdx.x * 256 + threadIdx.x; e < total4; e += (int64_t)gridDim.x * 256) {
    const int64_t r = e / c4;
    const int j = (int)(e - r * c4);
    dst[e] = j < ca4 ? a[r * ca4 + j] : b[r * cb4 + (j - ca4)];
  }
}
__global__ __launch_bounds__(256) void split_cols_kernel(const float4* __restrict__ src, int ca4, int cb4, float4* __restrict__ da,
                                                        float4* __restrict__ db, int accumulate, int64_t total4) {
  const int c4 = ca4 + cb4;
  for (int64_t e = (int64_t)blockIdx.x * 256 + threadIdx.x; e < total4; e += (int64_t)gridDim.x * 256) {
    const int64_t r = e / c4;
    const int j = (int)(e - r * c4);
    const float4 v = src[e];
    if (j < ca4) {
      da[r * ca4 + j] = v;
    } else {
      float4* o = db + r * cb4 + (j - ca4);
      if (accumulate) { const float4 t = *o; *o = make_float4(t.x + v.x, t.y + v.y, t.z + v.z, t.w + v.w); }
      else *o = v;
    }
  }
}
__global__ __launch_bounds__(256) void add_inplace_kernel(float* __restrict__ dst, const float* __restrict__ src, int64_t n) {
  const int64_t n4 = n >> 2;
  for (int64_t e = (int64_t)blockIdx.x * 256 + threadIdx.x; e < n4; e += (int64_t)gridDim.x * 256) {
    float4 d = reinterpret_cast<float4*>(dst)[e];
    const float4 v = reinterpret_cast<const float4*>(src)[e];
    d.x += v.x; d.y += v.y; d.z += v.z; d.w += v.w;
    reinterpret_cast<float4*>(dst)[e] = d;
  }
  for (int64_t e = (n4 << 2) + (int64_t)blockIdx.x * 256 + threadIdx.x; e < n; e += (int64_t)gridDim.x * 256) dst[e] += src[e];
}
inline unsigned ew_grid(int64_t work) {
  int64_t g = ceil_div(work, (int64_t)256 * 4);
  if (g < 1) g = 1;
  if (g > 2048) g = 2048;
  return (unsigned)g;
}

struct DeferredWgrads {
  const usc_kmap* map = nullptr; int cin = 0, cout = 0, n = 0;
  const float* a[16]; const float* b[16]; float* dW[16];
};
int flush_deferred(DeferredWgrads& q, void* ws, int64_t ws_bytes, usc_stream_t s) {
  if (q.n == 0) return USC_OK;
  const usc_kmap* m = q.map;
  int rc = USC_OK;
  if (q.n >= 2 && usc_spconv_wgrad_group_ok(q.n, q.cin, q.cout, m->K, m->pair_capacity)) {
// ... 220 lines not shown

int unit_backward_impl(const usc_kmap* m, int32_t kind, const float* x, int32_t cin, const float* W, int32_t cout,
                       const usc_bn* bn, const float* y, const float* stats, const float* out_relu,
                       const float* dout, float* dy, float* dres, float* dx, int32_t dx_accumulate, float* dW,
                       int32_t dW_accumulate, float* dgamma, float* dbeta, int32_t dbn_accumulate, void* ws,
                       int64_t ws_bytes, usc_stream_t s, Pending* in, Pending* out, int planes = 0) {
  if (out) *out = Pending{};
  USC_REQUIRE(bn && bn->c == cout, "usc_conv_bn_act_backward: batch-norm width must equal the conv's output width");
  USC_REQUIRE(y && stats && dout && dy && dgamma && dbeta && bn->gamma, "usc_conv_bn_act_backward: null pointer");
  const ConvShape sh = conv_shape(m, kind);
  if (sh.n_out == 0) return USC_OK;
  if (planes > 0)
    USC_REQUIRE(ws && ws_bytes >= usc_unit_split_ws_bytes(m, kind, cin, cout, planes),
                "usc_conv_bn_act_backward_split: workspace too small (usc_unit_split_ws_bytes)");
  WsCursor cur{(char*)ws, ws ? ws_bytes : 0, 0};
  const int64_t sb = usc_colstats_ws_bytes(sh.n_out, cout);
  void* sws = cur.take(sb);
  float* red = (float*)cur.take(2 * (int64_t)cout * 4);
  USC_REQUIRE(sws && red, "usc_conv_bn_act_backward: workspace too small");
  const float* mean = stats, *invstd = stats + cout;
  int rc;
  const bool has_in = in && in->G > 0;
  if (has_in) USC_REQUIRE(in->dx == dout && in->n == sh.n_out && in->c == cout, "usc unit: pending slices do not belong to this unit");
  if (tile_rows_ok(sh.n_out, cout) && sb >= usc_bn_tile_ws_bytes(cout)) {
    rc = usc_bn_tile_backward(has_in ? in->partial : nullptr, has_in ? in->G : 0, has_in ? in->accumulate : 0, (float*)dout, y,
                              out_relu, mean, invstd, bn->gamma, sh.n_out, cout, bn->training, dbn_accumulate, dgamma,
                              dbeta, dy, dres, sws, sb, s);
    if (has_in) *in = Pending{};
    if (rc) return rc;
  } else {
    if (has_in) { rc = flush_pending(*in, s); if (rc) return rc; }
    rc = usc_bn_backward_reduce(y, dout, out_relu, mean, invstd, sh.n_out, cout, bn->training, dbn_accumulate, dgamma,
                                dbeta, red, red + cout, sws, sb, s);
    if (rc) return rc;
    rc = usc_bn_backward_dx(y, dout, out_relu, mean, invstd, bn->gamma, red, red + cout, dy, dres, sh.n_out, cout, s);
    if (rc) return rc;
  }
  return conv_backward_impl(m, kind, x, cin, W, cout, dy, dx, dx_accumulate, dW, dW_accumulate, cur.rest(), cur.left(), s, out,
                            planes);
}

int check_split(const usc_kmap* m, int32_t kind, int32_t P, const char* who) {
  USC_REQUIRE(m, "%s: null kernel map", who);
  USC_REQUIRE(P == 2 || P == 3, "%s: P must be 2 or 3 (got %d)", who, P);
  USC_REQUIRE(kind == USC_CONV_SAME, "%s: the split precision covers stride-1 units only", who);
  return USC_OK;
}

int64_t program_half_bytes(const usc_step* steps, int32_t n_steps) {
  int64_t need = 256;
  if (!steps) return need;
  for (int i = 0; i < n_steps; ++i) {
    const usc_step& t = steps[i];
    if ((t.op == USC_STEP_UNIT_FWD || t.op == USC_STEP_UNIT_BWD) && t.map) {
      int64_t b = usc_unit_ws_bytes(t.map, t.kind, t.cin, t.cout);
      if (t.split_planes) {
        const int64_t sb = usc_unit_split_ws_bytes(t.map, t.kind, t.cin, t.cout, t.split_planes);
        if (sb > b) b = sb;
      }
      if (b > need) need = b;
    } else if (t.op == USC_STEP_UNIT_FWD_BF16 && t.map) {
      const int64_t b = usc_unit_bf16_ws_bytes(t.map, t.kind, t.cin, t.cout);
      if (b > need) need = b;
    }
  }
  return align_up(need, 256);
}

}

extern "C" {

int usc_set_wgrad_lane(usc_stream_t lane, void* lane_ws, int64_t lane_ws_bytes, int64_t max_rows) {
  int dev = 0;
  if (hipGetDevice(&dev) != hipSuccess || dev < 0 || dev >= 16) {
    set_error("usc_set_wgrad_lane: unsupported device index");
    return USC_ERR_ARG;
  }
  Lane& e = g_lane[dev];
  if (!lane) {
    e.st = nullptr;
    e.held.clear();
    e.hold = false;
    return USC_OK;
  }
  USC_REQUIRE(lane_ws && lane_ws_bytes > 0 && max_rows > 0, "usc_set_wgrad_lane: the lane needs its own scratch and a row bound");
  if (!e.fork) {
    if (hipEventCreateWithFlags(&e.fork, hipEventDisableTiming) != hipSuccess ||
        hipEventCreateWithFlags(&e.join, hipEventDisableTiming) != hipSuccess) {
      set_error("usc_set_wgrad_lane: hipEventCreate failed");
      return USC_ERR_LAUNCH;
    }
  }
  e.st = as_stream(lane);
  e.ws = lane_ws;
  e.ws_bytes = lane_ws_bytes;
  e.max_rows = max_rows;
  e.dirty = false;
  return USC_OK;
}

int usc_wgrad_lane_hold(int32_t mode, int64_t hold_min_rows, int64_t release_max_rows, usc_stream_t s) {
  Lane* lane = lane_for_current_device();
  if (!lane) return USC_OK;
  if (mode > 0) {
    USC_REQUIRE(hold_min_rows > release_max_rows && release_max_rows >= 0, "usc_wgrad_lane_hold: hold_min_rows must exceed release_max_rows");
    if (!lane->held.empty()) { const int rc = lane_release(lane, s); if (rc) return rc; }
    lane->hold = true;
    lane->hold_min_rows = hold_min_rows;
    lane->release_max_rows = release_max_rows;
    return USC_OK;
  }
  if (mode < 0) {
    lane->held.clear();
    lane->hold = false;
    return USC_OK;
  }
  return lane_release(lane, s);
}

int32_t usc_wgrad_lane_holding(void) {
  Lane* lane = lane_for_current_device();
  return lane && lane->hold ? 1 : 0;
}

int usc_wgrad_lane_join(usc_stream_t s) {
  Lane* lane = lane_for_current_device();
  if (lane && !lane->held.empty()) { const int rc = lane_release(lane, s); if (rc) return rc; }
  if (!lane || !lane->dirty) return USC_OK;
  if (hipEventRecord(lane->join, lane->st) != hipSuccess || hipStreamWaitEvent(as_stream(s), lane->join, 0) != hipSuccess) {
    set_error("usc_wgrad_lane_join: joining the lane failed");
    return USC_ERR_LAUNCH;
  }
  lane->dirty = false;
  return USC_OK;
}

int64_t usc_conv_ws_bytes(const usc_kmap* m, int32_t kind, int32_t cin, int32_t cout) {
  if (!m) return 0;
  int64_t fwd, dgrad, wg;
  conv_ws_parts(m, kind, cin, cout, &fwd, &dgrad, &wg);
  const int64_t bwd = dgrad + wg;
  return (fwd > bwd ? fwd : bwd) + 256;
}

int usc_conv_forward(const usc_kmap* m, int32_t kind, const float* x, int32_t cin, const float* W, int32_t cout,
                     const float* bias, float* y, void* ws, int64_t ws_bytes, usc_stream_t s) {
  return conv_forward_impl(m, kind, x, cin, W, cout, bias, y, ws, ws_bytes, s, nullptr);
}

int usc_conv_backward(const usc_kmap* m, int32_t kind, const float* x, int32_t cin, const float* W, int32_t cout,
                      const float* dy, float* dx, int32_t dx_accumulate, float* dW, int32_t dW_accumulate, void* ws,
                      int64_t ws_bytes, usc_stream_t s) {
  return conv_backward_impl(m, kind, x, cin, W, cout, dy, dx, dx_accumulate, dW, dW_accumulate, ws, ws_bytes, s, nullptr);
}

int64_t usc_unit_ws_bytes(const usc_kmap* m, int32_t kind, int32_t cin, int32_t cout) {
  return usc_conv_ws_bytes(m, kind, cin, cout) + align_up(usc_colstats_ws_bytes(0, cout), 256) +
         align_up(2 * (int64_t)cout * 4, 256) + 256;
}

int usc_conv_bn_act_forward(const usc_kmap* m, int32_t kind, const float* x, int32_t cin, const float* W, int32_t cout,
                            const usc_bn* bn, const float* residual, int32_t relu, float* y, float* stats, float* out,
                            void* ws, int64_t ws_bytes, usc_stream_t s) {
  return forward_unit({"usc_conv_bn_act_forward", "usc_conv_forward", "", 0}, m, kind, x, cin, W, nullptr, cout, bn, residual,
                      relu, y, stats, out, ws, ws_bytes, s);
}

int64_t usc_unit_bf16_ws_bytes(const usc_kmap* m, int32_t kind, int32_t cin, int32_t cout) {
  if (!m) return 0;
  const ConvShape sh = conv_shape(m, kind);
  const int64_t g = usc_spconv_gather_gemm_bf16_ws_bytes(sh.n_out, cin, cout, m->K);
  if (g < 0) return -1;
  int64_t b = align_up(usc_colstats_ws_bytes(sh.n_out, cout), 256) + align_up(sh.n_in * cin * 2, 256) + align_up(g, 256);
  if (kind == USC_CONV_UP) b += align_up((int64_t)m->K * sh.n_out * 4, 256);
  return b + 256;
}

int usc_conv_bn_act_forward_bf16(const usc_kmap* m, int32_t kind, const float* x, int32_t cin, const uint16_t* Wp,
                                 int32_t cout, const usc_bn* bn, const float* residual, int32_t relu, float* y,
                                 float* stats, float* out, void* ws, int64_t ws_bytes, usc_stream_t s) {
  const char* who = "usc_conv_bn_act_forward_bf16";
  return forward_unit({who, who, " (usc_unit_bf16_ws_bytes)", 1}, m, kind, x, cin, nullptr, Wp, cout, bn, residual, relu, y,
                      stats, out, ws, ws_bytes, s);
}

int usc_conv_bn_act_backward(const usc_kmap* m, int32_t kind, const float* x, int32_t cin, const float* W, int32_t cout,
                             const usc_bn* bn, const float* y, const float* stats, const float* out_relu,
                             const float* dout, float* dy, float* dres, float* dx, int32_t dx_accumulate, float* dW,
                             int32_t dW_accumulate, float* dgamma, float* dbeta, int32_t dbn_accumulate, void* ws,
                             int64_t ws_bytes, usc_stream_t s) {
  return unit_backward_impl(m, kind, x, cin, W, cout, bn, y, stats, out_relu, dout, dy, dres, dx, dx_accumulate, dW,
                            dW_accumulate, dgamma, dbeta, dbn_accumulate, ws, ws_bytes, s, nullptr, nullptr);
}

int64_t usc_unit_split_ws_bytes(const usc_kmap* m, int32_t kind, int32_t cin, int32_t cout, int32_t P) {
  if (!m) return 0;
  if ((P != 2 && P != 3) || kind != USC_CONV_SAME) return -1;
  if (usc_spconv_gather_gemm_split_ws_bytes(m->n_out, cin, cout, m->K, P) < 0) return -1;
  const int64_t f = split_gemm_ws(m, m->n_in, cin, cout, P);
  const int64_t b = split_dgrad_ok(m, cin, cout, P) ? split_gemm_ws(m, m->n_out, cout, cin, P) : 0;
  return usc_unit_ws_bytes(m, kind, cin, cout) + (f > b ? f : b) + 256;
}

int usc_conv_bn_act_forward_split(const usc_kmap* m, int32_t kind, const float* x, int32_t cin, const float* W, int32_t cout,
                                  int32_t P, const usc_bn* bn, const float* residual, int32_t relu, float* y, float* stats,
                                  float* out, void* ws, int64_t ws_bytes, usc_stream_t s) {
  const char* who = "usc_conv_bn_act_forward_split";
  const int rc = check_split(m, kind, P, who);
  if (rc) return rc;
  return forward_unit({who, who, " (usc_unit_split_ws_bytes)", P}, m, kind, x, cin, W, nullptr, cout, bn, residual, relu, y,
                      stats, out, ws, ws_bytes, s);
}

int usc_conv_bn_act_backward_split(const usc_kmap* m, int32_t kind, const float* x, int32_t cin, const float* W, int32_t cout,
                                   int32_t P, const usc_bn* bn, const float* y, const float* stats, const float* out_relu,
                                   const float* dout, float* dy, float* dres, float* dx, int32_t dx_accumulate, float* dW,
                                   int32_t dW_accumulate, float* dgamma, float* dbeta, int32_t dbn_accumulate, void* ws,
                                   int64_t ws_bytes, usc_stream_t s) {
  const int rc = check_split(m, kind, P, "usc_conv_bn_act_backward_split");
  if (rc) return rc;
  return unit_backward_impl(m, kind, x, cin, W, cout, bn, y, stats, out_relu, dout, dy, dres, dx, dx_accumulate, dW,
                            dW_accumulate, dgamma, dbeta, dbn_accumulate, ws, ws_bytes, s, nullptr, nullptr, P);
}

int32_t usc_step_size(void) { return (int32_t)sizeof(usc_step); }

int64_t usc_program_ws_bytes(const usc_step* steps, int32_t n_steps) { return 2 * program_half_bytes(steps, n_steps) + 256; }

int usc_program_run(const usc_step* steps, int32_t begin, int32_t end, void* ws_all, int64_t ws_all_bytes, usc_stream_t s) {
  USC_REQUIRE(steps && begin >= 0 && end >= begin, "usc_program_run: bad step range");
  hipStream_t st = as_stream(s);
  DeferredWgrads q;
  Pending pend;
  int rc = USC_OK;
  const int64_t half = ws_all_bytes > 256 ? (((ws_all_bytes - 256) / 2) & ~(int64_t)255) : 0;
  const bool two = ws_all && half >= program_half_bytes(steps + begin, end - begin);
  void* ws = ws_all;
  int64_t ws_bytes = two ? half : ws_all_bytes;
  for (int i = begin; i < end && !rc; ++i) {
    const usc_step& t = steps[i];
    if (two) ws = (char*)ws_all + (i & 1) * half;
    if (pend.G > 0 && !(t.op == USC_STEP_UNIT_BWD && t.dout == pend.dx)) {
      rc = flush_pending(pend, s);
      if (rc) break;
    }
    switch (t.op) {
      case USC_STEP_UNIT_FWD:
        rc = t.split_planes ? usc_conv_bn_act_forward_split(t.map, t.kind, t.x, t.cin, t.W, t.cout, t.split_planes, t.bn,
                                                            t.residual, t.relu, t.y, t.stats, t.out, ws, ws_bytes, s)
                            : usc_conv_bn_act_forward(t.map, t.kind, t.x, t.cin, t.W, t.cout, t.bn, t.residual, t.relu, t.y,
                                                      t.stats, t.out, ws, ws_bytes, s);
        break;
      case USC_STEP_UNIT_FWD_BF16:
        rc = usc_conv_bn_act_forward_bf16(t.map, t.kind, t.x, t.cin, (const uint16_t*)t.W, t.cout, t.bn, t.residual, t.relu,
                                          t.y, t.stats, t.out, ws, ws_bytes, s);
        break;
      case USC_STEP_UNIT_BWD: {
        USC_REQUIRE(t.map, "usc_program_run: step %d has no kernel map", i);
        const bool defer = t.defer_wgrad && t.dW && t.dW_accumulate && t.kind == USC_CONV_SAME && t.map->K > 1 && t.map->pair_in &&
                           t.cin % 32 == 0 && t.cout % 32 == 0 &&
                           (usc_spconv_wgrad_group_ok(2, t.cin, t.cout, t.map->K, t.map->pair_capacity) ||
                            usc_spconv_wgrad_group_ok(usc_spconv_wgrad_group_max(), t.cin, t.cout, t.map->K, t.map->pair_capacity));
        if (defer && q.n > 0 && (q.map != t.map || q.cin != t.cin || q.cout != t.cout || q.n == 16)) {
          rc = flush_deferred(q, ws, ws_bytes, s);
          if (rc) break;
        }
        Pending next;
        if (t.split_planes) rc = check_split(t.map, t.kind, t.split_planes, "usc_program_run");
        if (rc) break;
        rc = unit_backward_impl(t.map, t.kind, t.x, t.cin, t.W, t.cout, t.bn, t.y, t.stats, t.out, t.dout, t.dy, t.dres,
                                t.dx, t.dx_accumulate, defer ? nullptr : t.dW, t.dW_accumulate, t.dgamma, t.dbeta,
                                t.dbn_accumulate, ws, ws_bytes, s, &pend, two ? &next : nullptr, t.split_planes);
        if (!rc && pend.G > 0) rc = flush_pending(pend, s);
        pend = next;
        if (!rc && defer) {
          q.map = t.map; q.cin = t.cin; q.cout = t.cout;
          q.a[q.n] = t.x; q.b[q.n] = t.dy; q.dW[q.n] = t.dW;
          ++q.n;
        }
        break;
      }
      case USC_STEP_CAT: {
        USC_REQUIRE(t.a && t.b && t.dst && t.ca % 4 == 0 && t.cb % 4 == 0 && t.n >= 0, "usc_program_run: bad cat step %d", i);
        const int64_t total4 = t.n * ((t.ca + t.cb) / 4);
        if (total4 > 0)
          hipLaunchKernelGGL(cat_cols_kernel, dim3(ew_grid(total4)), dim3(256), 0, st, (const float4*)t.a, t.ca / 4,
                             (const float4*)t.b, t.cb / 4, (float4*)t.dst, total4);
        break;
      }
      case USC_STEP_SPLIT: {
        USC_REQUIRE(t.a && t.dst && t.dst2 && t.ca % 4 == 0 && t.cb % 4 == 0 && t.n >= 0, "usc_program_run: bad split step %d", i);
        const int64_t total4 = t.n * ((t.ca + t.cb) / 4);
        if (total4 > 0)
          hipLaunchKernelGGL(split_cols_kernel, dim3(ew_grid(total4)), dim3(256), 0, st, (const float4*)t.a, t.ca / 4, t.cb / 4,
                             (float4*)t.dst, (float4*)t.dst2, (int)t.accumulate, total4);
        break;
      }
      case USC_STEP_ADD:
        USC_REQUIRE(t.a && t.dst && t.n >= 0, "usc_program_run: bad add step %d", i);
        if (t.n > 0) hipLaunchKernelGGL(add_inplace_kernel, dim3(ew_grid(t.n / 4 + 1)), dim3(256), 0, st, t.dst, t.a, t.n);
        break;
      default:
        set_error("usc_program_run: unknown step op");
        rc = USC_ERR_ARG;
    }
  }
  const int rc3 = flush_pending(pend, s);
  const int rc2 = flush_deferred(q, ws, ws_bytes, s);
  if (rc) return rc;
  if (rc3) return rc3;
  if (rc2) return rc2;
  USC_CHECK_LAUNCH("usc_program_run");
  return USC_OK;
}

}
```

### unscene3d_amd/models/mask3d.py

```python
import contextlib
import os

import torch
import torch.nn as nn
from torch.nn import functional as F

from .. import MinkowskiEngine as ME
from .. import ops
from ..MinkowskiEngine import MinkowskiOps as me
from ..MinkowskiEngine.MinkowskiPooling import MinkowskiAvgPooling
from ..pointnet2_utils import furthest_point_sample
from .modules.common import conv
from .modules.helpers_3detr import GenericMLP
from .position_embedding import PositionEmbeddingCoordsSine

SINGLE_POINT_ERROR = "only a single point gives nans in cross-attention"


class Mask3D(nn.Module):
    def __init__(self, config, hidden_dim, num_queries, num_heads, dim_feedforward, sample_sizes, shared_decoder,
                 num_classes, num_decoders, dropout, pre_norm, positional_encoding_type, non_parametric_queries,
                 train_on_segments, normalize_pos_enc, use_level_embed, scatter_type, hlevels, use_np_features,
                 voxel_size, max_sample_size, random_queries, gauss_scale, random_query_both, random_normal):
        super().__init__()
# ... 160 lines not shown
        if geo["key_samples"] is not None:
            self._gather_pos_keys(geo["key_samples"], geo["pos_encodings_pcd"], geo)
        if self.train_on_segments and point2segment is not None and _FUSED_ATTN_MASK and len(point2segment) >= 1:
            if len(point2segment) == 1:
                rows = point2segment[0].to(torch.int64).contiguous()
            else:
                off, parts = 0, []
                for p2s, csr in zip(point2segment, geo["seg_csr"]):
                    parts.append(p2s.to(torch.int64) + off)
                    off += csr.S
                rows = torch.cat(parts).contiguous()
                cm._usc_p2s_batched = rows
            geo["p2s_rows"] = rows
            _child_segment_table(cm, x._ts(), rows)
        x._usc_geometry = geo
        return geo

    def _gather_pos_keys(self, samples, pos_encodings_pcd, geo):
        out = []
        for pidx, plan in enumerate(samples["passes"]):
            hlevel = self.hlevels[pidx % self.num_levels]
            per_scene = pos_encodings_pcd[hlevel][0]
            n_scenes, K = len(per_scene), plan["k"]
            if plan["gidx"] is not None and per_scene[0].is_cuda:
                if n_scenes == 1:
                    pos_l = per_scene[0]
                else:
                    cat = geo.setdefault("pos_cat", {})
                    if hlevel not in cat:
                        cat[hlevel] = torch.cat(per_scene)
                    pos_l = cat[hlevel]
                out.append(ops.gather_rows(pos_l.contiguous(), plan["gidx"]).view(n_scenes, K, -1))
            else:
                out.append(_stack([per_scene[k][plan["rand_idx"][k], :] for k in range(n_scenes)]))
        samples["pos_keys"] = out

    def _graph_key(self):
        g = getattr(self, "_graphed_passes", None)
        return None if g is None else id(g)

    def _draw_key_samples(self, coords, is_eval):
        dev = coords[0].F.device
        level_sizes = [[f.shape[0] for f in lv.decomposed_features] for lv in coords]
        slices = [lv.coordinate_manager.batch_slices(lv._ts()) for lv in coords]
        graphed = getattr(self, "_graphed_passes", None) is not None
        passes = []
        for decoder_counter in range(self.num_decoders):
            for i, hlevel in enumerate(self.hlevels):
                sizes = level_sizes[hlevel]
                curr = max(sizes)
                if not (self.max_sample_size or is_eval):
                    curr = min(curr, self.sample_sizes[hlevel])
                if graphed:
                    want = self._graph_shapes[decoder_counter * self.num_levels + i][2][0]
                    if curr < want:
                        curr = want
                rand_idx, mask_idx = [], []
                for pcd_size in sizes:
                    if pcd_size <= curr:
                        idx, midx = _padded_index(pcd_size, curr, dev)
                    else:
                        idx = self.randperm(pcd_size, dev)[:curr]
                        midx = _padded_index(curr, curr, dev)[1]
                    rand_idx.append(idx)
                    mask_idx.append(midx)
                gidx = None
                if all(isinstance(sl, slice) for sl in slices[hlevel]):
                    gidx = rand_idx[0] if len(sizes) == 1 else torch.cat(
                        [rand_idx[k] + slices[hlevel][k].start for k in range(len(sizes))])
                passes.append({"k": curr, "rand_idx": rand_idx, "mask_idx": mask_idx, "gidx": gidx,
                               "all_sampled": all(n > curr for n in sizes), "sizes": sizes})
        return {"passes": passes, "is_eval": bool(is_eval), "graph_key": self._graph_key()}

    def forward(self, x, point2segment=None, raw_coordinates=None, is_eval=False, num_segments=None):
        pcd_features, aux = self.backbone(x)
        n_scenes = len(x.decomposed_coordinates)

        geo = getattr(x, "_usc_geometry", None)
        if geo is None or geo.get("n_levels") != len(aux):
            geo = self.precompute_geometry(x, raw_coordinates, point2segment, num_segments, n_levels=len(aux),
                                           is_eval=is_eval)
        coordinates, coords, pos_encodings_pcd = geo["coordinates"], geo["coords"], geo["pos_encodings_pcd"]

        mask_features = self.mask_features_head(pcd_features)
        mask_segments, seg_csr = None, None
        if self.train_on_segments:
            seg_csr = geo["seg_csr"]
            if self.scatter_type == "mean":
                mask_segments = [ops.segment_mean(f, csr) for f, csr in zip(mask_features.decomposed_features, seg_csr)]
            else:
                mask_segments = [_segment_max(f, csr.seg, csr.S) for f, csr in zip(mask_features.decomposed_features, seg_csr)]

        sampled_coords = None
        if self.non_parametric_queries:
            fps_idx, sampled_coords = geo["fps_idx"], geo["sampled_coords"]
            query_pos = self.query_projection(geo["query_pos_enc"])
            if self.use_np_features:
                queries = _stack([pcd_features.decomposed_features[i][fps_idx[i]] for i in range(n_scenes)])
                queries = self.np_feature_projection(queries)
            else:
                queries = torch.zeros_like(query_pos).permute(0, 2, 1)
            query_pos = query_pos.permute(2, 0, 1).contiguous()
        elif self.random_queries:
            query_pos = torch.rand(n_scenes, self.mask_dim, self.num_queries, device=x.device) - 0.5
            queries = torch.zeros_like(query_pos).permute(0, 2, 1)
            query_pos = query_pos.permute(2, 0, 1)
        elif self.random_query_both:
            shape = (n_scenes, 2 * self.mask_dim, self.num_queries)
            qpf = torch.randn(*shape, device=x.device) if self.random_normal else torch.rand(*shape, device=x.device) - 0.5
            queries = qpf[:, :self.mask_dim, :].permute(0, 2, 1)
            query_pos = qpf[:, self.mask_dim:, :].permute(2, 0, 1)
        else:
            queries = self.query_feat.weight.unsqueeze(0).repeat(n_scenes, 1, 1)
            query_pos = self.query_pos.weight.unsqueeze(1).repeat(1, n_scenes, 1)

        samples = geo.pop("key_samples", None)
        if samples is None or samples["is_eval"] != bool(is_eval) or samples["graph_key"] != self._graph_key():
            samples = self._draw_key_samples(coords, is_eval)
        if samples.get("pos_keys") is None:
            self._gather_pos_keys(samples, pos_encodings_pcd, geo)

        predictions_class, predictions_mask = [], []
        p2s_arg = point2segment if self.train_on_segments else None
        sinks = {}
        use_side = _KV_SIDE_STREAM and x.F.is_cuda
        main = torch.cuda.current_stream() if x.F.is_cuda else None
        side = self._side_stream(x.device) if use_side else None
        if use_side:
            ready = torch.cuda.Event()
            ready.record(main)
            side.wait_event(ready)
        for decoder_counter in range(self.num_decoders):
            dec = 0 if self.shared_decoder else decoder_counter
            for i, hlevel in enumerate(self.hlevels):
                pidx = decoder_counter * self.num_levels + i
                plan = samples["passes"][pidx]
                decomposed_aux = aux[hlevel].decomposed_features
                sizes = [f.shape[0] for f in decomposed_aux]
                if min(sizes) == 1:
                    raise RuntimeError(SINGLE_POINT_ERROR)
                if plan["sizes"] != sizes:
                    raise RuntimeError(f"key samples were drawn for level sizes {plan['sizes']}, the backbone produced "
                                       f"{sizes}")
                curr_sample_size, rand_idx, mask_idx = plan["k"], plan["rand_idx"], plan["mask_idx"]
                n_valid = [min(n, curr_sample_size) for n in sizes]
                graph_shapes = (self._graph_shapes[pidx] if getattr(self, "_graphed_passes", None) is not None else None)
                step_fn = self._decoder_pass(decoder_counter, dec, i)
                bufs = None
                d_model = self.mask_dim
                if graph_shapes is not None:
                    have = (queries.shape, query_pos.shape, (curr_sample_size, n_scenes, d_model),
                            (curr_sample_size, n_scenes, d_model), (n_scenes, curr_sample_size, self.num_queries))
                    if tuple(tuple(h) for h in have) != tuple(tuple(w) for w in graph_shapes):
                        step_fn = self._eager_pass(dec, i)
                    elif plan["gidx"] is not None:
                        bufs = step_fn.input_buffers
                feats_l = aux[hlevel].F
                fused = (plan["gidx"] is not None and feats_l.is_cuda
                         and feats_l.dtype == torch.float32 and n_scenes <= 16 and feats_l.shape[1] % 4 == 0
                         and self.num_queries <= fused_attn_max_queries())

                on_side = use_side and fused
                if on_side:
                    for t in (plan["gidx"], samples["pos_keys"][pidx], feats_l):
                        if t is not None and t.is_cuda:
                            t.record_stream(side)
                with (torch.cuda.stream(side) if on_side else contextlib.nullcontext()):
                    if fused:
                        batched_aux = ops.sample_keys(
                            feats_l.contiguous(), None, None, plan["gidx"], n_scenes, curr_sample_size, n_valid,
                            unique=plan["all_sampled"], valid_unique=True,
                            sink=sinks.setdefault((hlevel, bool(plan["all_sampled"])), ops.GradSink()))
                    else:
                        batched_aux = _stack([ops.gather_rows(decomposed_aux[k].contiguous(), rand_idx[k],
                                                              unique=sizes[k] > curr_sample_size) for k in range(n_scenes)])
                    k_keys, v_keys = self._key_prep(dec, i)(batched_aux, samples["pos_keys"][pidx],
                                                            outs=None if bufs is None else (bufs[2], bufs[3]))
                    if on_side:
                        kv_done = torch.cuda.Event()
                        kv_done.record(side)
                        if bufs is None:
                            k_keys.record_stream(main)
                            v_keys.record_stream(main)

                normed, queries = self._norm_queries(queries)
                output_class, outputs_mask, attn_mask = self.mask_module(
                    queries, mask_features, mask_segments, len(aux) - hlevel - 1, ret_attn_mask=True,
                    point2segment=p2s_arg, coords=coords, defer_class=True, normed=normed)
                decomposed_attn = attn_mask.decomposed_features
                if fused and attn_mask.F.dtype == torch.bool and attn_mask.F.shape[1] <= fused_attn_max_queries():
                    batched_attn = ops.sample_keys(None, attn_mask.F.contiguous(), None, plan["gidx"], n_scenes,
                                                   curr_sample_size, n_valid,
                                                   outs=None if bufs is None else (None, bufs[4], None))
                else:
                    batched_attn = _stack([decomposed_attn[k][rand_idx[k], :] for k in range(n_scenes)])
                    batched_attn.permute(0, 2, 1)[batched_attn.sum(1) == curr_sample_size] = False
                    if not plan["all_sampled"]:
                        batched_attn = torch.logical_or(batched_attn, _stack(mask_idx)[..., None])
                    if bufs is not None:
                        bufs[4].copy_(batched_attn)
                        batched_attn = bufs[4]

                rec = getattr(self, "attn_mask_record", None)
                if rec is not None:
                    rec.append(batched_attn.detach().clone())
                if on_side:
                    main.wait_event(kv_done)
                queries = step_fn(queries, query_pos, k_keys, v_keys, batched_attn.contiguous())

                predictions_class.append(output_class)
                predictions_mask.append(outputs_mask)

        output_class, outputs_mask = self.mask_module(queries, mask_features, mask_segments, 0, ret_attn_mask=False,
                                                      point2segment=p2s_arg, coords=coords, defer_class=True)
        predictions_class.append(output_class)
        predictions_mask.append(outputs_mask)
        predictions_class = list(self.class_embed_head(torch.stack(predictions_class)).unbind(0))

        return {
            "pred_logits": predictions_class[-1],
            "pred_masks": predictions_mask[-1],
            "aux_outputs": self._set_aux_loss(predictions_class, predictions_mask),
            "sampled_coords": _host_array(sampled_coords) if sampled_coords is not None else None,
            "backbone_features": pcd_features,
        }

    def _norm_queries(self, queries):
        norm = self.decoder_norm
        if (queries.is_cuda and queries.dtype == torch.float32 and queries.requires_grad
                and isinstance(norm, LayerNorm) and norm.elementwise_affine and norm.bias is not None
                and len(norm.normalized_shape) == 1 and norm.normalized_shape[0] in ops._LN_DIMS):
            return ops.layer_norm(queries, norm.weight, norm.bias, norm.eps, passthrough=True)
        return norm(queries), queries

    def mask_module(self, query_feat, mask_features, mask_segments, num_pooling_steps, ret_attn_mask=True,
                    point2segment=None, coords=None, defer_class=False, normed=None):
        query_feat = self.decoder_norm(query_feat) if normed is None else normed
        head = self.mask_embed_head
        Q = query_feat.shape[-2]
        q_pad = (-Q) % 32
        if query_feat.is_cuda and query_feat.dtype == torch.float32:
            if defer_class and query_feat.requires_grad:
                hidden, query_feat = ops.linear(query_feat, head[0].weight, head[0].bias, relu=True, passthrough=True)
            else:
                hidden = ops.linear(query_feat, head[0].weight, head[0].bias, relu=True)
            if (q_pad and query_feat.dim() == 3 and query_feat.shape[0] == 1
                    and isinstance(head[2], Linear) and head[2].out_features % 32 == 0):
                mask_embed = ops.linear(hidden, head[2].weight, head[2].bias, pad_rows_to=Q + q_pad)
                mask_embed = _PaddedRows(mask_embed, Q)
            else:
                mask_embed = head[2](hidden)
        else:
            mask_embed = head(query_feat)
        outputs_class = query_feat if defer_class else self.class_embed_head(query_feat)

        output_masks, output_segments = [], []
        if (point2segment is not None and ret_attn_mask and num_pooling_steps >= 1 and query_feat.is_cuda
                and _FUSED_ATTN_MASK):
            for i, seg_feat in enumerate(mask_segments):
                logits, mask_segments[i] = _mask_logits(seg_feat, mask_embed[i], chain=True)
                output_segments.append(logits)
            cm, ts = mask_features.coordinate_manager, mask_features._ts()
            if len(output_segments) == 1:
                pooled = output_segments[0].detach()
                rows = point2segment[0].to(torch.int64).contiguous()
            else:
                Q = output_segments[0].shape[1]
                pooled = torch.cat([getattr(o, "_usc_padded", o).detach() for o in output_segments])[:, :Q]
                rows = getattr(cm, "_usc_p2s_batched", None)
                if rows is None or rows.shape[0] != mask_features.F.shape[0]:
                    off, parts = 0, []
                    for p2s, seg in zip(point2segment, mask_segments):
                        parts.append(p2s.to(torch.int64) + off)
                        off += seg.shape[0]
                    rows = torch.cat(parts).contiguous()
                    cm._usc_p2s_batched = rows
            for step in range(num_pooling_steps):
                if step == 0:
                    pooled = ops.avgpool_down2(pooled, _child_segment_table(cm, ts, rows),
                                               threshold=num_pooling_steps == 1)
                else:
                    pooled = ops.avgpool_down2(pooled, cm.stride_map(ts)["nbr2"],
                                               threshold=step == num_pooling_steps - 1)
                ts *= 2
            attn_mask = me.SparseTensor(features=pooled, coordinate_manager=cm,
                                        coordinate_map_key=ME.CoordinateMapKey(ts))
            return outputs_class, output_segments, attn_mask
        if point2segment is not None:
            for i, seg_feat in enumerate(mask_segments):
                output_segments.append(_mask_logits(seg_feat, mask_embed[i]))
                if ret_attn_mask:
                    with torch.no_grad():
                        output_masks.append(ops.gather_rows(output_segments[-1].detach().contiguous(),
                                                            point2segment[i].to(torch.int64).contiguous()))
        else:
            per_scene = mask_features.decomposed_features
            for i in range(len(per_scene)):
                output_masks.append(_mask_logits(per_scene[i], mask_embed[i]))

        if ret_attn_mask:
            attn_mask = me.SparseTensor(features=torch.cat(output_masks).detach(),
                                        coordinate_manager=mask_features.coordinate_manager,
                                        coordinate_map_key=mask_features.coordinate_map_key)
            for _ in range(num_pooling_steps):
                attn_mask = self.pooling(attn_mask.float())
            attn_mask = me.SparseTensor(features=(attn_mask.F.detach().sigmoid() < 0.5),
                                        coordinate_manager=attn_mask.coordinate_manager,
                                        coordinate_map_key=attn_mask.coordinate_map_key)
            if point2segment is not None:
                return outputs_class, output_segments, attn_mask
            return outputs_class, output_masks, attn_mask
        if point2segment is not None:
            return outputs_class, output_segments
        return outputs_class, output_masks

    @torch.jit.unused
    def _set_aux_loss(self, outputs_class, outputs_seg_masks):
        return [{"pred_logits": a, "pred_masks": b} for a, b in zip(outputs_class[:-1], outputs_seg_masks[:-1])]


class HostArrayLater:

    def __init__(self, t):
        t = t.detach()
        self._host = torch.empty(t.shape, dtype=t.dtype, pin_memory=True)
        self._host.copy_(t, non_blocking=True)
        self._event = torch.cuda.Event()
        self._event.record()
        self.shape, self.dtype = tuple(t.shape), self._host.numpy().dtype

    def numpy(self):
        self._event.synchronize()
        return self._host.numpy()

    def __array__(self, dtype=None, copy=None):
        a = self.numpy()
        return a if dtype is None else a.astype(dtype)

    def __getitem__(self, i):
        return self.numpy()[i]

    def __len__(self):
        return self.shape[0]


def _host_array(t):
    if t.is_cuda:
        return HostArrayLater(t)
    return t.detach().cpu().numpy()


class Linear(nn.Linear):

    def forward(self, x):
        if x.is_cuda and x.dtype == torch.float32:
            return ops.linear(x, self.weight, self.bias)
        return super().forward(x)


class _PaddedRows:

    def __init__(self, table, q):
        self.table, self.q = table, q

    def __getitem__(self, i):
        t = self.table
        if t.shape[0] == 1 and i == 0:
            return (t.view(t.shape[1], t.shape[2]), self.q)
        return (t[i], self.q)


def _mask_logits(feats, mask_embed, chain=False):
    if isinstance(mask_embed, tuple):
        W, Q = mask_embed
        pad = W.shape[0] - Q
        if not (feats.is_cuda and feats.dtype == torch.float32 and feats.shape[1] % 32 == 0):
            out = feats @ W[:Q].T
            return (out, feats) if chain else out
    else:
        Q = mask_embed.shape[0]
        if not (feats.is_cuda and feats.dtype == torch.float32 and feats.shape[1] % 32 == 0):
            out = feats @ mask_embed.T
            return (out, feats) if chain else out
        pad = (-Q) % 32
        W = F.pad(mask_embed, (0, 0, 0, pad)) if pad else mask_embed
    nxt = feats
    if chain and feats.requires_grad and torch.is_grad_enabled():
        out, nxt = ops.linear(feats, W.contiguous(), passthrough=True)
    else:
        out = ops.linear(feats, W.contiguous())
    if pad:
        view = out[:, :Q]
        view._usc_padded = out
        out = view
    return (out, nxt) if chain else out


def multihead_attention(mha: nn.MultiheadAttention, query, key, value, attn_mask=None, pos_q=None, pos_k=None,
                        residual=False):
    L, B, E = query.shape
    S = key.shape[0]
    H = mha.num_heads
    hd = E // H
    res = None
    if residual:
        q, k, v, res = ops.in_proj(query, key, value, mha.in_proj_weight, mha.in_proj_bias, pos_q=pos_q, pos_k=pos_k,
                                   residual=True)
    else:
        q, k, v = ops.in_proj(query, key, value, mha.in_proj_weight, mha.in_proj_bias, pos_q=pos_q, pos_k=pos_k)
    done = (lambda o: (o, res)) if residual else (lambda o: o)
    if attn_mask is None and hd == 16 and L == S and L <= fused_attn_max_queries():
        out = ops.self_attention(q, k, v, H)
        return done(ops.linear(out, mha.out_proj.weight, mha.out_proj.bias))
    q = q.reshape(L, B * H, hd).transpose(0, 1).reshape(B, H, L, hd)
    k = k.reshape(S, B * H, hd).transpose(0, 1).reshape(B, H, S, hd)
    v = v.reshape(S, B * H, hd).transpose(0, 1).reshape(B, H, S, hd)
    if attn_mask is None:
        out = F.scaled_dot_product_attention(q, k, v)
    else:
        mask = torch.zeros(attn_mask.shape, dtype=q.dtype, device=q.device).masked_fill_(attn_mask, float("-inf"))
        scores = torch.baddbmm(mask, q.reshape(B * H, L, hd), k.reshape(B * H, S, hd).transpose(1, 2),
                               alpha=1.0 / (hd ** 0.5))
        out = torch.bmm(torch.softmax(scores, dim=-1), v.reshape(B * H, S, hd)).reshape(B, H, L, hd)
    out = out.permute(2, 0, 1, 3).reshape(L, B, E)
    return done(ops.linear(out, mha.out_proj.weight, mha.out_proj.bias))


class LayerNorm(nn.LayerNorm):

    def forward(self, x):
        if (x.is_cuda and x.dtype == torch.float32 and self.elementwise_affine and len(self.normalized_shape) == 1
                and self.normalized_shape[0] in ops._LN_DIMS and self.bias is not None):
            return ops.layer_norm(x, self.weight, self.bias, self.eps)
        return super().forward(x)


class _KeyPrep:

    def __init__(self, squeeze, cross, level_embed, level):
        self.squeeze, self.cross, self.level_embed, self.level = squeeze, cross, level_embed, level

    def __call__(self, batched_aux, batched_pos, outs=None):
        src = self.squeeze(batched_aux.permute(1, 0, 2))
        if self.level_embed is not None:
            src = src + self.level_embed.weight[self.level]
        mha = self.cross.multihead_attn
        pos = batched_pos.permute(1, 0, 2)
        if src.is_cuda and src.dtype == torch.float32:
            return ops.in_proj_kv(src, mha.in_proj_weight, mha.in_proj_bias, pos=pos.contiguous(), outs=outs)
        E = src.shape[-1]
        W, b = mha.in_proj_weight, mha.in_proj_bias
        k, v = F.linear(src + pos, W[E:2 * E], b[E:2 * E]), F.linear(src, W[2 * E:], b[2 * E:])
        if outs is not None:
            outs[0].copy_(k), outs[1].copy_(v)
            k, v = outs
        return k, v


class _DecoderPass(nn.Module):

    def __init__(self, cross, self_attn, ffn, num_heads):
        super().__init__()
        self.cross, self.self_attn, self.ffn, self.num_heads = cross, self_attn, ffn, num_heads

    def forward(self, queries, query_pos, k, v, batched_attn):
        out = self.cross.forward_kv(queries.permute(1, 0, 2), k, v, batched_attn, query_pos)
        out = self.self_attn(out, tgt_mask=None, tgt_key_padding_mask=None, query_pos=query_pos)
        return self.ffn(out).permute(1, 0, 2)


_KV_SIDE_STREAM = os.environ.get("USC3D_KV_SIDE_STREAM", "1") != "0"


def set_kv_side_stream(on: bool):
    global _KV_SIDE_STREAM
    if torch.cuda.is_available():
        torch.cuda.synchronize()
    _KV_SIDE_STREAM = bool(on)
# ... 202 lines not shown
```

### unscene3d_amd/ops.py

```python
from __future__ import annotations

from dataclasses import dataclass

import ctypes
import os

import torch

from . import profiler as _prof
from ._lib import check, lib, require_device


def _stream():
    return torch._C._cuda_getCurrentRawStream(torch._C._cuda_getDevice())


def _chk(t: torch.Tensor, dtype, name: str):
    if not isinstance(t, torch.Tensor):
        raise RuntimeError(f"{name} must be a torch.Tensor")
    if not t.is_cuda:
        raise RuntimeError(f"{name} must be a HIP (cuda) tensor — unscene3d_amd has no CPU path")
    if t.dtype != dtype:
        raise RuntimeError(f"{name} must be {dtype}, got {t.dtype}")
    if not t.is_contiguous():
# ... 1120 lines not shown
    M, K = x2.shape
    N = W.shape[0]
    if _small_linear_ok(M, K, N):
        Mp = M if pad_rows_to is None else int(pad_rows_to)
        y = torch.empty((Mp, N), dtype=torch.float32, device=x2.device) if out is None else out
        if tuple(y.shape) != (Mp, N) or y.dtype != torch.float32 or not y.is_contiguous():
            raise RuntimeError(f"linear: `out` must be a contiguous f32 [{Mp}, {N}] tensor")
        check(lib.usc_linear_fwd_pad(_ptr(x2), _ptr(add), _ptr(W), _ptr(b), M, N, K, int(relu), _ptr(y), Mp, _stream()),
              "usc_linear_fwd")
        return y
    if pad_rows_to is not None:
        raise RuntimeError("linear: pad_rows_to needs the few-row kernels (rows <= 1024, widths multiples of 32)")
    if add is not None:
        x2 = x2 + add
    if relu:
        return torch.relu_(_lin_fwd(x2, W, b, out=out))
    if _rows_gemm_ok(M, K, N) and W.is_contiguous():
        return gather_gemm(x2, W.view(1, N, K), None, M, bias=b, out=out, w_transposed=True)
    y = torch.addmm(b, x2, W.t()) if b is not None else x2 @ W.t()
    return y if out is None else out.copy_(y)


def col_sum(x2, out, accumulate=False):
    _chk(x2, torch.float32, "x2")
    if not out.is_contiguous() or out.dtype != torch.float32 or out.numel() != x2.shape[1]:
        raise RuntimeError("col_sum: `out` must be a contiguous f32 vector with one entry per column")
    wsb = lib.usc_col_sum_ws_bytes(x2.shape[0], x2.shape[1])
    ws = _ws(wsb, x2.device)
    check(lib.usc_col_sum(_ptr(x2), x2.shape[0], x2.shape[1], _ptr(out), int(accumulate), _ptr(ws), wsb, _stream()),
          "usc_col_sum")
    return out


def _lin_bwd(dy2, x2, W, dW_out, db_out, need_dx=True, accumulate=False, add=None, y_relu=None, dx_add=None,
             dx_add2=None, want_dx_b=False):
    M, N = dy2.shape
    K = x2.shape[1]
    if want_dx_b or dx_add2 is not None:
        if not need_dx:
            _lin_bwd(dy2, x2, W, dW_out, db_out, False, accumulate, add, y_relu)
            return (None, None) if want_dx_b else None
        if _small_linear_ok(M, K, N):
            dx = torch.empty((M, K), dtype=torch.float32, device=dy2.device)
            dx_b = torch.empty_like(dx) if want_dx_b else None
            check(lib.usc_linear_bwd_ex2(_ptr(dy2), _ptr(y_relu), _ptr(x2), _ptr(add), _ptr(W), M, N, K, _ptr(dx),
                                         _ptr(dx_add), _ptr(dx_add2), _ptr(dx_b), _ptr(dW_out), _ptr(db_out),
                                         int(accumulate), _stream()), "usc_linear_bwd")
        else:
            dx_b = _lin_bwd(dy2, x2, W, dW_out, db_out, True, accumulate, add, y_relu, dx_add)
            dx = dx_b if dx_add2 is None else dx_b + dx_add2
        return (dx, dx_b) if want_dx_b else dx
    if _small_linear_ok(M, K, N):
        dx = torch.empty((M, K), dtype=torch.float32, device=dy2.device) if need_dx else None
        check(lib.usc_linear_bwd_ex(_ptr(dy2), _ptr(y_relu), _ptr(x2), _ptr(add), _ptr(W), M, N, K, _ptr(dx),
                                    _ptr(dx_add) if need_dx else None, _ptr(dW_out), _ptr(db_out), int(accumulate),
                                    _stream()), "usc_linear_bwd")
        return dx
    if y_relu is not None:
        dy2 = dy2 * (y_relu > 0)
    if add is not None:
        x2 = x2 + add
    if dx_add is not None:
        dx = _lin_bwd(dy2, x2, W, dW_out, db_out, need_dx, accumulate)
        return None if dx is None else dx.add_(dx_add)
    rows_ok = _rows_gemm_ok(M, K, N) and W.is_contiguous()
    if rows_ok and dW_out.is_contiguous():
        if accumulate:
            wgrad(dy2, x2, 1, into=dW_out)
        else:
            wgrad(dy2, x2, 1, out=dW_out)
    elif accumulate:
        dW_out.addmm_(dy2.t(), x2)
    else:
        torch.mm(dy2.t(), x2, out=dW_out)
    if db_out is not None:
        col_sum(dy2, db_out, accumulate)
    if not need_dx:
        return None
    if rows_ok:
        return gather_gemm(dy2, W.view(1, N, K), None, M)
    return dy2 @ W


class _LinearRows(torch.autograd.Function):
    @staticmethod
    def forward(ctx, x, W, b, relu=False, passthrough=False, pad_rows_to=None):
        x2 = x.contiguous().view(-1, x.shape[-1])
        ctx.rows = x2.shape[0]
        if pad_rows_to is not None:
            if relu or passthrough or x2.shape[0] != x.shape[-2] or pad_rows_to < x2.shape[0]:
                raise RuntimeError("linear: pad_rows_to is for one [.., M, K] table, M <= pad_rows_to, without relu")
            y = _lin_fwd(x2, W, b, pad_rows_to=pad_rows_to)
            ctx.save_for_backward(x2, W, None)
            ctx.shape = x.shape
            ctx.w_param, ctx.b_param = W, b
            return y.view(*x.shape[:-2], int(pad_rows_to), W.shape[0])
        y = _lin_fwd(x2, W, b, relu=relu)
        ctx.save_for_backward(x2, W, y if relu else None)
        ctx.shape = x.shape
        ctx.w_param, ctx.b_param = W, b
        y = y.view(*x.shape[:-1], W.shape[0])
        return (y, x) if passthrough else y

    @staticmethod
    def backward(ctx, dy, dres=None):
        x2, W, y_relu = ctx.saved_tensors
        dy2 = dy.contiguous().view(-1, W.shape[0])[:ctx.rows]
        (dW, db), in_place, finish = _param_grads((ctx.w_param, ctx.b_param))
        dres2 = None if dres is None else dres.contiguous().view(-1, x2.shape[1])
        dx = _lin_bwd(dy2, x2, W, dW, db, need_dx=ctx.needs_input_grad[0], accumulate=in_place, y_relu=y_relu,
                      dx_add=dres2)
        return (None if dx is None else dx.view(ctx.shape),) + finish() + (None, None, None)


def linear(x, W, b=None, relu=False, passthrough=False, pad_rows_to=None):
    _chk(W, torch.float32, "W")
    return _LinearRows.apply(x, W, b, relu, passthrough, pad_rows_to)




def _rows(t, E):
    return None if t is None else t.contiguous().view(-1, E)


def _same_tensor(a, c):
    return a.data_ptr() == c.data_ptr() and a.shape == c.shape and a.stride() == c.stride()


class _InProjSelf(torch.autograd.Function):

    @staticmethod
    def forward(ctx, x, W, b, pos, residual=False):
        E = W.shape[1]
        x2, p2 = _rows(x, E), _rows(pos, E)
        M = x2.shape[0]
        xp = x2
        if p2 is not None and not _small_linear_ok(M, E, E):
            xp, p2 = x2 + p2, None
        if _small_linear_ok(M, E, 3 * E) and W.is_contiguous():
            y3 = torch.empty((3, M, E), dtype=torch.float32, device=W.device)
            check(lib.usc_linear_fwd_split(_ptr(x2), _ptr(p2), _ptr(W), _ptr(b), M, 3 * E, E, 2 * E, E, _ptr(y3),
                                           _stream()), "usc_linear_fwd_split")
            outs = (y3[0], y3[1], y3[2])
        else:
            outs = (_lin_fwd(xp, W[:E], b[:E], add=p2), _lin_fwd(xp, W[E:2 * E], b[E:2 * E], add=p2),
                    _lin_fwd(x2, W[2 * E:], b[2 * E:]))
        ctx.save_for_backward(xp, x2, W, p2)
        ctx.shape, ctx.pos_shape = x.shape, None if pos is None else pos.shape
        ctx.w_param, ctx.b_param = W, b
        out = tuple(o.view(*x.shape[:-1], E) for o in outs)
        return out + (x,) if residual else out

    @staticmethod
    def backward(ctx, dq, dk, dv, dres=None):
        xp, x2, W, p2 = ctx.saved_tensors
        E = W.shape[1]
        M = x2.shape[0]
        dres2 = _rows(dres, E)
        (dW, db), in_place, finish = _param_grads((ctx.w_param, ctx.b_param))
        need_x, need_pos = ctx.needs_input_grad[0], ctx.pos_shape is not None and ctx.needs_input_grad[3]
        adjacent = (dq.is_contiguous() and dk.is_contiguous() and dv.is_contiguous()
                    and dk.data_ptr() == dq.data_ptr() + 4 * M * E and dv.data_ptr() == dk.data_ptr() + 4 * M * E)
        if (need_x and adjacent and W.is_contiguous() and _small_linear_ok(M, 3 * E, E) and dW.is_contiguous()
                and db.is_contiguous()):
            gx = torch.empty((M, E), dtype=torch.float32, device=W.device)
# ... 200 lines not shown
```

### unscene3d_amd/program.py

```python
from __future__ import annotations

import ctypes as C
import os

import torch

from . import ops, precision, units
from ._lib import STEP_ADD, STEP_CAT, STEP_SPLIT, STEP_UNIT_BWD, STEP_UNIT_FWD, STEP_UNIT_FWD_BF16, Step, check, lib

ENABLED = os.environ.get("USC3D_BACKBONE_PROGRAM", "1") == "1"
SAME, DOWN, UP = units.SAME, units.DOWN, units.UP
_ALIGN = 64


class _Plan:

    def __init__(self):
        self.ops, self.bufs, self.levels = [], {}, []
        self.input = None
        self.params = []

    def new(self, level, c):
        i = len(self.bufs)
        self.bufs[i] = (level, c)
# ... 5 lines not shown
    from .models.modules.resnet_block import BasicBlockBase
    pl = _Plan()

    def unit(stage, conv, norm, kind, level, x, res, relu):
        if not (conv.bias is None and isinstance(norm, MinkowskiBatchNorm) and norm.bn.affine
                and norm.bn.momentum is not None):
            raise NotImplementedError
        if kind == SAME and not (isinstance(conv, MinkowskiConvolution) and conv.stride == 1):
            raise NotImplementedError
        if kind == DOWN and not (isinstance(conv, MinkowskiConvolution) and conv.stride == 2 and conv.ksize == 2):
            raise NotImplementedError
        if kind == UP and not (isinstance(conv, MinkowskiConvolutionTranspose) and conv.stride == 2 and conv.ksize == 2):
            raise NotImplementedError
        lout = level + 1 if kind == DOWN else (level - 1 if kind == UP else level)
        y, out = pl.new(lout, conv.out_channels), pl.new(lout, conv.out_channels)
        pl.ops.append(dict(t="unit", stage=stage, conv=conv, bn=norm.bn, kind=kind, lin=level, lout=lout, x=x, res=res,
                           relu=relu, y=y, out=out, cin=conv.in_channels, cout=conv.out_channels,
                           ksize=conv.ksize, kvol=conv.kernel_volume))
        return out

    def blocks(stage, seq, level, x):
        for blk in seq:
            if not isinstance(blk, BasicBlockBase) or blk.conv1.stride != 1 or blk.conv2.stride != 1 \
                    or blk.conv1.kernel_volume == 1 or blk.conv1.ksize != blk.conv2.ksize:
                raise NotImplementedError
            a1 = unit(stage, blk.conv1, blk.norm1, SAME, level, x, None, True)
            r = x
            if blk.downsample is not None:
                ds = blk.downsample
                if len(ds) != 2 or ds[0].kernel_volume != 1:
                    raise NotImplementedError
                r = unit(stage, ds[0], ds[1], SAME, level, x, None, False)
            x = unit(stage, blk.conv2, blk.norm2, SAME, level, a1, r, True)
        return x

    try:
        pl.input = pl.new(0, model.conv0p1s1.in_channels)
        x = unit("conv0p1s1", model.conv0p1s1, model.bn0, SAME, 0, pl.input, None, True)
        skip = [x]
        for i, (cname, nname, bname) in enumerate(model._DOWN):
            x = unit(cname, getattr(model, cname), getattr(model, nname), DOWN, i, x, None, True)
            x = blocks(bname, getattr(model, bname), i + 1, x)
            skip.append(x)
        pl.levels = [x]
        top = len(model._DOWN)
        for j, (cname, nname, bname) in enumerate(model._UP):
            u = unit(cname, getattr(model, cname), getattr(model, nname), UP, top - j, x, None, True)
            s = skip[top - 1 - j]
            ca, cb = pl.bufs[u][1], pl.bufs[s][1]
            if ca % 4 or cb % 4:
                raise NotImplementedError
            c = pl.new(top - 1 - j, ca + cb)
            pl.ops.append(dict(t="cat", stage=cname, a=u, b=s, out=c, level=top - 1 - j, ca=ca, cb=cb))
            x = blocks(bname, getattr(model, bname), top - 1 - j, c)
            pl.levels.append(x)
    except (NotImplementedError, AttributeError):
        return None
    n_levels = top + 1
    pl.n_levels = n_levels
    act, grad = [0] * n_levels, [0] * n_levels
    n_act = n_grad = 0
    for op in pl.ops:
        if op["t"] == "unit":
            act[op["lout"]] += 2 * op["cout"]
            n_act += 3
            grad[op["lout"]] += 2 * op["cout"]
            grad[op["lin"]] += 2 * op["cin"]
            n_grad += 4
        else:
            act[op["level"]] += op["ca"] + op["cb"]
            n_act += 1
            grad[op["level"]] += op["ca"] + op["cb"]
            n_grad += 2
    pl.act_floats, pl.grad_floats, pl.n_act, pl.n_grad = act, grad, n_act, n_grad
    pl.stat_floats = sum(4 * op["cout"] for op in pl.ops if op["t"] == "unit")
    seen, params = set(), []
    for op in pl.ops:
        if op["t"] == "unit":
            for p in (op["conv"].kernel, op["bn"].weight, op["bn"].bias):
                if id(p) not in seen:
                    seen.add(id(p))
                    params.append(p)
    pl.params = params
    return pl


def _module_key(model):
    return tuple(id(m) for m in model.modules())


def plan_of(model):
    cached = model.__dict__.get("_usc_program_plan")
    key = _module_key(model)
    if cached is None or cached[1] != key:
        cached = model.__dict__["_usc_program_plan"] = (_plan(model) or False, key)
    return cached[0] or None


class _Carver:

    def __init__(self, floats, device):
        self.arena = torch.empty(int(floats), dtype=torch.float32, device=device)
        self.base, self.off, self.cap = self.arena.data_ptr(), 0, int(floats)

    def take(self, n):
        off = self.off
        self.off = (off + int(n) + _ALIGN - 1) // _ALIGN * _ALIGN
        if self.off > self.cap:
            raise RuntimeError("step program: arena too small (planning bug)")
        return self.base + 4 * off, off

    def view(self, off, n, c):
        return self.arena[off:off + n * c].view(n, c)


class _Pool:

    def __init__(self, device, chunk_floats):
        self.device, self.chunk_floats = device, int(chunk_floats)
        self.chunks, self.base, self.off, self.cap = [], 0, 0, 0
        self.free = {}

    def take(self, n):
        n = (int(n) + _ALIGN - 1) // _ALIGN * _ALIGN
        lst = self.free.get(n)
        if lst:
            return lst.pop()
        if self.off + n > self.cap:
            self.cap = max(self.chunk_floats, n)
            t = torch.empty(self.cap, dtype=torch.float32, device=self.device)
            self.chunks.append(t)
            self.base, self.off = t.data_ptr(), 0
        p = self.base + 4 * self.off
        self.off += n
        return p

    def release(self, p, n):
        n = (int(n) + _ALIGN - 1) // _ALIGN * _ALIGN
        self.free.setdefault(n, []).append(p)


def usable(model, x):
    if not (ENABLED and units.usable(x.F, None) and x.F.shape[0] > 0):
        return None
    pl = plan_of(model)
    if pl is None:
        return None
    if torch.is_grad_enabled():
        need = [p.requires_grad for p in pl.params]
        if any(need):
            if not all(need) or x.F.requires_grad:
                return None
            for p in pl.params:
                if ops._grad_target(p) is None:
                    return None
    return pl


class _Trunk(torch.autograd.Function):
    @staticmethod
    def forward(ctx, model, pl, cm, ts, bf16, split, feats, *params):
        dev = feats.device
        rows = [cm.coord_map(ts << l).n for l in range(pl.n_levels)]
        floats = sum(r * f for r, f in zip(rows, pl.act_floats)) + pl.stat_floats + (pl.n_act + 8) * _ALIGN
        car = _Carver(floats, dev)
        ptr, offs = {pl.input: feats.data_ptr()}, {}
        steps = (Step * len(pl.ops))()
        kcache = {}

        def kmap(op):
            key = (op["kind"], op["lin"], op["kvol"])
            k = kcache.get(key)
            if k is None:
                t = ts << op["lin"]
                if op["kind"] == SAME:
                    k = cm.kmap_identity(t) if op["kvol"] == 1 else cm.kmap_cube(t, op["ksize"])
                elif op["kind"] == DOWN:
                    k = cm.kmap_down(t)
                else:
                    k = cm.kmap_down(t >> 1)
                kcache[key] = k
            return k

        stats_ptr, kmaps, bnrefs = [], [], []
        for i, op in enumerate(pl.ops):
            st = steps[i]
            if op["t"] == "unit":
                n_out, cout = rows[op["lout"]], op["cout"]
                py, offs[op["y"]] = car.take(n_out * cout)
                po, offs[op["out"]] = car.take(n_out * cout)
                ps, _ = car.take(4 * cout)
                ptr[op["y"]], ptr[op["out"]] = py, po
                km = kmap(op)
                bdesc, _ = units._bn_desc(op["bn"], units._training(op["bn"]))
                bref = C.addressof(bdesc)
                st.op, st.kind, st.cin, st.cout, st.relu = STEP_UNIT_FWD, op["kind"], op["cin"], cout, int(op["relu"])
                st.map, st.bn = C.addressof(km.struct), bref
                st.x, st.W = ptr[op["x"]], op["conv"].kernel.data_ptr()
                wp = bf16.get(id(op["conv"].kernel)) if bf16 else None
                if wp is not None:
                    st.op, st.W = STEP_UNIT_FWD_BF16, wp.data_ptr()
                if split:
                    st.split_planes = split.get(i, 0)
                st.residual = ptr[op["res"]] if op["res"] is not None else None
                st.y, st.stats, st.out = py, ps, po
                stats_ptr.append(ps)
                kmaps.append(km)
                bnrefs.append((bref, bdesc))
            else:
                n = rows[op["level"]]
                pc, offs[op["out"]] = car.take(n * (op["ca"] + op["cb"]))
                ptr[op["out"]] = pc
                st.op, st.a, st.b, st.dst, st.n, st.ca, st.cb = STEP_CAT, ptr[op["a"]], ptr[op["b"]], pc, n, op["ca"], op["cb"]
                stats_ptr.append(None)
                kmaps.append(None)
                bnrefs.append(None)
        wsb = lib.usc_program_ws_bytes(steps, len(pl.ops))
        ws = units.workspace(wsb, dev)
        check(lib.usc_program_run(steps, 0, len(pl.ops), ws.data_ptr(), ws.numel(), ops._stream()), "usc_program_run")
        outs = tuple(car.view(offs[b], rows[pl.bufs[b][0]], pl.bufs[b][1]) for b in pl.levels)
        ctx.state = (model, pl, cm, ts, feats, car, ptr, stats_ptr, kmaps, bnrefs, rows, split)
        return outs

    @staticmethod
    def backward(ctx, *gouts):
        model, pl, cm, ts, feats, car, ptr, stats_ptr, kmaps, bnrefs, rows, split = ctx.state
        dev = feats.device
        gar = _Pool(dev, max(rows[0] * 256, 1 << 20))
        lane = units._lane(dev)
        if lane is not None:
            gar.release = lambda p_, n_: None
            car.arena.record_stream(lane[0])
        keep = [g.contiguous() if g is not None else None for g in gouts]
        G = {}
        held_dy = []
        for b, g in zip(pl.levels, keep):
            if g is not None:
                G[b] = [g.data_ptr(), True, g.numel()]
        steps = (Step * (3 * len(pl.ops) + 8))()
        ns = 0
        segments, cur_params, stage = [], [], None

        def add_step(dst, src, n):
            nonlocal ns
            st = steps[ns]
            ns += 1
            st.op, st.dst, st.a, st.n = STEP_ADD, dst, src, n

        def contribute(bid, numel, can_accumulate):
            cur = G.get(bid)
            if cur is None:
                p = gar.take(numel)
                G[bid] = [p, False, numel]
                return p, 0, None
            if can_accumulate and not cur[1]:
                return cur[0], 1, None
            p = gar.take(numel)
            if cur[1]:
                def fin(p=p, old=cur[0]):
                    add_step(p, old, numel)
                    G[bid] = [p, False, numel]
            else:
                def fin(p=p, old=cur[0]):
                    add_step(old, p, numel)
                    gar.release(p, numel)
            return p, 0, fin

        def consumed(bid):
            cur = G.pop(bid, None)
            if cur is not None and not cur[1]:
                gar.release(cur[0], cur[2])

        for i in range(len(pl.ops) - 1, -1, -1):
            op = pl.ops[i]
            if op["stage"] != stage:
                if stage is not None:
                    segments.append((ns, cur_params))
                    cur_params = []
                    for p_, n_ in held_dy:
                        gar.release(p_, n_)
                    held_dy = []
                stage = op["stage"]
            if op["t"] == "cat":
                g = G.get(op["out"])
                if g is None:
                    continue
                n = rows[op["level"]]
                pa, _, fa = contribute(op["a"], n * op["ca"], False)
                cur_b = G.get(op["b"])
                if cur_b is not None and not cur_b[1]:
                    pb, acc_b, fb = cur_b[0], 1, None
                else:
                    pb, acc_b, fb = contribute(op["b"], n * op["cb"], False)
                st = steps[ns]
                ns += 1
                st.op, st.a, st.dst, st.dst2, st.n, st.ca, st.cb, st.accumulate = STEP_SPLIT, g[0], pa, pb, n, op["ca"], \
                    op["cb"], acc_b
                for f in (fa, fb):
                    if f is not None:
                        f()
                consumed(op["out"])
                continue
            g = G.get(op["out"])
            if g is None:
                continue
            n_out, n_in, cin, cout = rows[op["lout"]], rows[op["lin"]], op["cin"], op["cout"]
            pdy = gar.take(n_out * cout)
            pres, fres = None, None
            if op["res"] is not None:
                pres, _, fres = contribute(op["res"], n_out * cout, False)
            need_dx = op["x"] != pl.input
            pdx, acc, fdx = (None, 0, None)
            if need_dx:
                pdx, acc, fdx = contribute(op["x"], n_in * cin, op["kind"] != DOWN)
            conv, bn = op["conv"], op["bn"]
            tW, tg, tb = ops._grad_target(conv.kernel), ops._grad_target(bn.weight), ops._grad_target(bn.bias)
            if tW is None or tg is None or tb is None:
                raise RuntimeError("step program: a parameter lost its in-place gradient target between forward and "
                                   "backward (keep p.grad allocated: optimizer.zero_grad(set_to_none=False))")
            st = steps[ns]
            ns += 1
            st.op, st.kind, st.cin, st.cout = STEP_UNIT_BWD, op["kind"], cin, cout
            st.map, st.bn = C.addressof(kmaps[i].struct), bnrefs[i][0]
            st.x, st.W = ptr[op["x"]], conv.kernel.data_ptr()
            st.y, st.stats = ptr[op["y"]], stats_ptr[i]
            st.out = ptr[op["out"]] if op["relu"] else None
            st.dout, st.dy, st.dres, st.dx, st.dx_accumulate = g[0], pdy, pres, pdx, acc
            st.dW, st.dW_accumulate, st.dgamma, st.dbeta, st.dbn_accumulate = tW.data_ptr(), 1, tg.data_ptr(), \
                tb.data_ptr(), 1
            st.defer_wgrad = int(units.GROUP_WGRAD)
            if split:
                st.split_planes = split.get(i, 0)
            cur_params.extend((conv.kernel, bn.weight, bn.bias))
            for f in (fres, fdx):
                if f is not None:
                    f()
            consumed(op["out"])
            if st.defer_wgrad and op["kind"] == SAME and op["kvol"] > 1:
                held_dy.append((pdy, n_out * cout))
            else:
                gar.release(pdy, n_out * cout)
        segments.append((ns, cur_params))
        wsb = lib.usc_program_ws_bytes(steps, ns)
        ws = units.workspace(wsb, dev)
        stream = ops._stream()
        begin = 0
        holding = lane is not None and units.LANE_HOLD_MIN_ROWS > units.LANE_RELEASE_ROWS > 0 and \
            any(min(rows[o["lin"]], rows[o["lout"]]) <= units.LANE_RELEASE_ROWS for o in pl.ops if o["t"] == "unit")
        unreported = []
        if holding:
            check(lib.usc_wgrad_lane_hold(1, units.LANE_HOLD_MIN_ROWS, units.LANE_RELEASE_ROWS, stream), "usc_wgrad_lane_hold")
        try:
            for end, plist in segments:
                if end > begin:
                    check(lib.usc_program_run(steps, begin, end, ws.data_ptr(), ws.numel(), stream), "usc_program_run")
                if holding and lib.usc_wgrad_lane_holding():
                    unreported.extend(plist)
                elif plist or unreported:
                    ops._grad_written(*unreported, *plist)
                    ops._params_final(unreported + plist)
                    unreported = []
                begin = end
            if holding:
                check(lib.usc_wgrad_lane_hold(0, 0, 0, stream), "usc_wgrad_lane_hold")
                if unreported:
                    ops._grad_written(*unreported)
                    ops._params_final(unreported)
        except BaseException:
            if holding:
                lib.usc_wgrad_lane_hold(-1, 0, 0, None)
            raise
        if lane is not None:
            for t in gar.chunks:
                t.record_stream(lane[0])
            units.queue_lane_join(units._dev_key(dev))
        ctx.state = None
        return (None, None, None, None, None, None, None) + (None,) * len(pl.params)


def trunk(model, x):
    pl = usable(model, x)
    if pl is None:
        return None
    cm, ts = x.coordinate_manager, x._ts()
    feats = x.F.contiguous()
    bf16 = None
    if precision.bf16_active():
        bf16 = {}
        for op in pl.ops:
            if op["t"] == "unit":
                wp = precision.unit_weights(op["conv"].kernel, op["kind"] == SAME, cm.coord_map(ts << op["lout"]).n)
                if wp is not None:
                    bf16[id(op["conv"].kernel)] = wp
    split = None
    if precision.current_training() != "f32" and torch.is_grad_enabled():
        split = {}
        for i, op in enumerate(pl.ops):
            if op["t"] == "unit":
                planes = precision.train_planes(op["conv"].kernel, op["kind"] == SAME, cm.coord_map(ts << op["lout"]).n)
                if planes:
                    split[i] = planes
        split = split or None
    return list(_Trunk.apply(model, pl, cm, ts, bf16, split, feats, *pl.params))
```

Measured before the change: 44.65.

## Issue last backbone stage backward early on lane stream, overlapping decoder backward

Adds an early-stage path: once the mask-feature head's gradient is available, it computes the s1 feature gradient from all mask-logit heads with a fused multi-head dx kernel. It then launches the final trunk stage's backward program on the weight-gradient lane stream, chained by an event, so it overlaps with the remaining decoder/autograd backward work. A new linear_heads_dx kernel sums dy·W across up to 16 heads in one launch instead of separate linear backward calls. This adds considerable bookkeeping (handles, abandoned-state settling, gradient-target checks) and risks ordering or lifetime bugs across streams.

New measurement: 46.81, median of 6. 1.05x the previous value.

```diff
diff --git a/include/usc3d.h b/include/usc3d.h
--- a/include/usc3d.h
+++ b/include/usc3d.h
@@ -273,6 +273,8 @@
 int32_t usc_step_size(void);
 int64_t usc_program_ws_bytes(const usc_step* steps, int32_t n_steps);
 int usc_program_run(const usc_step* steps, int32_t begin, int32_t end, void* ws, int64_t ws_bytes, usc_stream_t s);
+int usc_program_run_lane(const usc_step* steps, int32_t begin, int32_t end, void* ws, int64_t ws_bytes, usc_stream_t s);
+int usc_wgrad_lane_wait_chain(usc_stream_t s);
 
 
 int64_t usc_colstats_ws_bytes(int64_t n, int32_t c);
@@ -436,6 +438,9 @@
 int usc_linear_bwd_ex2(const float* dy, const float* y_relu, const float* x, const float* x2, const float* W, int32_t M,
                        int32_t N, int32_t K, float* dx, const float* dx_add, const float* dx_add2, float* dx_b, float* dW,
                        float* db, int32_t accumulate, usc_stream_t s);
+int32_t usc_linear_heads_max(void);
+int usc_linear_heads_dx(const float* const* dy, const float* const* W, int32_t L, int32_t M, int32_t N, int32_t K, float* dx,
+                        usc_stream_t s);
 int usc_qkv_proj_bwd(const float* dy3, const float* x, const float* pos, const float* W, int32_t M, int32_t E, float* dx,
                      float* dx_b, const float* dres, float* dW, float* db, int32_t accumulate, usc_stream_t s);
 int64_t usc_col_sum_ws_bytes(int64_t n, int32_t c);
diff --git a/unscene3d_amd/_lib.py b/unscene3d_amd/_lib.py
--- a/unscene3d_amd/_lib.py
+++ b/unscene3d_amd/_lib.py
@@ -92,6 +92,8 @@
     "usc_step_size": (_i32, []),
     "usc_program_ws_bytes": (_i64, [_sp, _i32]),
     "usc_program_run": (C.c_int, [_sp, _i32, _i32, _p, _i64, _p]),
+    "usc_program_run_lane": (C.c_int, [_sp, _i32, _i32, _p, _i64, _p]),
+    "usc_wgrad_lane_wait_chain": (C.c_int, [_p]),
     "usc_spconv_wgrad_group_max": (_i32, []),
     "usc_spconv_wgrad_grid_limit": (None, [_i32]),
     "usc_spconv_wgrad_group_ok": (C.c_int, [_i32, _i32, _i32, _i32, _i64]),
@@ -197,6 +199,8 @@
     "usc_linear_bwd_ex": (C.c_int, [_p, _p, _p, _p, _p, _i32, _i32, _i32, _p, _p, _p, _p, _i32, _p]),
     "usc_qkv_proj_bwd": (C.c_int, [_p, _p, _p, _p, _i32, _i32, _p, _p, _p, _p, _p, _i32, _p]),
     "usc_linear_bwd_ex2": (C.c_int, [_p, _p, _p, _p, _p, _i32, _i32, _i32, _p, _p, _p, _p, _p, _p, _i32, _p]),
+    "usc_linear_heads_max": (_i32, []),
+    "usc_linear_heads_dx": (C.c_int, [_p, _p, _i32, _i32, _i32, _i32, _p, _p]),
     "usc_layernorm_bwd_ws_bytes": (_i64, [_i64, _i32]),
     "usc_layernorm_bwd": (C.c_int, [_p, _p, _p, _p, _p, _i64, _i32, _p, _p, _p, _i32, _p, _i64, _p]),
     "usc_layernorm_bwd_ex": (C.c_int, [_p, _p, _p, _p, _p, _i64, _i32, _p, _p, _p, _p, _i32, _p, _i64, _p]),
diff --git a/unscene3d_amd/csrc/coords.hip b/unscene3d_amd/csrc/coords.hip
--- a/unscene3d_amd/csrc/coords.hip
+++ b/unscene3d_amd/csrc/coords.hip
@@ -203,7 +203,7 @@
 extern "C" {
 
 const char* usc_last_error(void) { return g_err; }
-int usc_abi_version(void) { return 4; }
+int usc_abi_version(void) { return 5; }
 
 int usc_device_count(void) {
   int n = 0;
diff --git a/unscene3d_amd/csrc/decoder.hip b/unscene3d_amd/csrc/decoder.hip
--- a/unscene3d_amd/csrc/decoder.hip
+++ b/unscene3d_amd/csrc/decoder.hip
@@ -293,10 +293,8 @@
 }
 
 template <bool EX>
-__device__ inline void linear_dx_tile(const float* __restrict__ dy, const float* __restrict__ ymask,
-                                      const float* __restrict__ W, int M, int N, int K, float* __restrict__ dx,
-                                      const float* __restrict__ dx_add, const float* __restrict__ dx_add2,
-                                      float* __restrict__ dx_b, int c0, int m0, float (*red)[16][64]) {
+__device__ inline f32x16 linear_dx_acc(const float* __restrict__ dy, const float* __restrict__ ymask,
+                                       const float* __restrict__ W, int M, int N, int K, int c0, int m0) {
   const int lane = threadIdx.x & 63, wave = threadIdx.x >> 6, i = lane & 31, h = lane >> 5;
   const int m = m0 + i;
   const float* ya = dy + (int64_t)(m < M ? m : 0) * N + 4 * h;
@@ -341,6 +339,15 @@
       for (int j = 0; j < 4; ++j) acc = MFMA32(av[j], bv[4 * t + j], acc);
     }
   }
+  return acc;
+}
+template <bool EX>
+__device__ inline void linear_dx_tile(const float* __restrict__ dy, const float* __restrict__ ymask,
+                                      const float* __restrict__ W, int M, int N, int K, float* __restrict__ dx,
+                                      const float* __restrict__ dx_add, const float* __restrict__ dx_add2,
+                                      float* __restrict__ dx_b, int c0, int m0, float (*red)[16][64]) {
+  const int lane = threadIdx.x & 63, wave = threadIdx.x >> 6;
+  const f32x16 acc = linear_dx_acc<EX>(dy, ymask, W, M, N, K, c0, m0);
   tile_reduce_store(acc, red, wave, lane, dx, K, m0, c0, M, nullptr, 0, 0, EX ? dx_add : nullptr,
                     EX ? dx_add2 : nullptr, EX ? dx_b : nullptr);
 }
@@ -502,6 +509,34 @@
   }
 }
 
+constexpr int kMaxHeads = 16;
+struct HeadPtrs { const float* dy[kMaxHeads]; const float* W[kMaxHeads]; };
+
+__global__ __launch_bounds__(256) void linear_heads_dx_kernel(HeadPtrs hp, int L, int M, int N, int K,
+                                                             float* __restrict__ dx) {
+  __shared__ float red[4][16][64];
+  const int lane = threadIdx.x & 63, wave = threadIdx.x >> 6, i = lane & 31, h = lane >> 5;
+  const int kt = K / 32;
+  const int c0 = ((int)blockIdx.x % kt) * 32, m0 = ((int)blockIdx.x / kt) * 32;
+  float run[4] = {0.f, 0.f, 0.f, 0.f};
+  for (int l = L - 1; l >= 0; --l) {
+    const f32x16 acc = linear_dx_acc<false>(hp.dy[l], nullptr, hp.W[l], M, N, K, c0, m0);
+    float v[4];
+    tile_reduce4(acc, red, wave, lane, v);
+#pragma unroll
+    for (int q = 0; q < 4; ++q) {
+      float o = v[q] + 0.f + 0.f;
+      if (l < L - 1) o += run[q];
+      run[q] = o;
+    }
+  }
+#pragma unroll
+  for (int q = 0; q < 4; ++q) {
+    const int row = m0 + acc_row16(4 * wave + q, h);
+    if (row < M) dx[(int64_t)row * K + c0 + i] = run[q];
+  }
+}
+
 constexpr int kColSumRows = 64;
 __global__ __launch_bounds__(256) void col_sum_partial_kernel(const float* __restrict__ x, int64_t n, int c,
                                                              float* __restrict__ partial) {
@@ -625,6 +660,25 @@
   return USC_OK;
 }
 
+int32_t usc_linear_heads_max(void) { return usc::kMaxHeads; }
+
+int usc_linear_heads_dx(const float* const* dy, const float* const* W, int32_t L, int32_t M, int32_t N, int32_t K, float* dx,
+                        usc_stream_t s) {
+  USC_REQUIRE(L >= 1 && L <= usc::kMaxHeads, "usc_linear_heads_dx: 1 <= L <= %d heads", usc::kMaxHeads);
+  USC_REQUIRE(M >= 1 && N >= 32 && N % 32 == 0 && K >= 32 && K % 32 == 0, "usc_linear_heads_dx: N, K must be multiples of 32");
+  USC_REQUIRE(dy && W && dx, "usc_linear_heads_dx: null pointer");
+  usc::HeadPtrs hp{};
+  for (int l = 0; l < L; ++l) {
+    USC_REQUIRE(dy[l] && W[l], "usc_linear_heads_dx: null pointer (head %d)", l);
+    hp.dy[l] = dy[l];
+    hp.W[l] = W[l];
+  }
+  hipLaunchKernelGGL(usc::linear_heads_dx_kernel, dim3((K / 32) * ((M + 31) / 32)), dim3(256), 0, usc::as_stream(s), hp,
+                     (int)L, (int)M, (int)N, (int)K, dx);
+  USC_CHECK_LAUNCH("usc_linear_heads_dx");
+  return USC_OK;
+}
+
 int64_t usc_col_sum_ws_bytes(int64_t n, int32_t c) {
   const int64_t parts = n > 0 ? (n + usc::kColSumRows - 1) / usc::kColSumRows : 0;
   return parts * (c > 0 ? c : 0) * 4;
diff --git a/unscene3d_amd/csrc/units.hip b/unscene3d_amd/csrc/units.hip
--- a/unscene3d_amd/csrc/units.hip
+++ b/unscene3d_amd/csrc/units.hip
@@ -108,9 +108,10 @@
   return usc_spconv_wgrad(j.x, j.cin, j.dy, j.cout, j.K, j.a_idx, j.b_idx, j.koff, j.rows, j.dW, accumulate, ws, j.list_bytes, s);
 }
 
-struct Lane { hipStream_t st = nullptr; hipEvent_t fork = nullptr, join = nullptr; void* ws = nullptr; int64_t ws_bytes = 0;
+struct Lane { hipStream_t st = nullptr; hipEvent_t fork = nullptr, join = nullptr, chain = nullptr; void* ws = nullptr; int64_t ws_bytes = 0;
               int64_t max_rows = 0; bool dirty = false;
-              bool hold = false; int64_t hold_min_rows = 0, release_max_rows = 0; std::vector<WgradJob> held; };
+              bool hold = false; int64_t hold_min_rows = 0, release_max_rows = 0; std::vector<WgradJob> held;
+              bool chain_set = false; };
 Lane g_lane[16];
 Lane* lane_for_current_device() {
   int dev = 0;
@@ -497,12 +498,14 @@
     e.st = nullptr;
     e.held.clear();
     e.hold = false;
+    e.chain_set = false;
     return USC_OK;
   }
   USC_REQUIRE(lane_ws && lane_ws_bytes > 0 && max_rows > 0, "usc_set_wgrad_lane: the lane needs its own scratch and a row bound");
   if (!e.fork) {
     if (hipEventCreateWithFlags(&e.fork, hipEventDisableTiming) != hipSuccess ||
-        hipEventCreateWithFlags(&e.join, hipEventDisableTiming) != hipSuccess) {
+        hipEventCreateWithFlags(&e.join, hipEventDisableTiming) != hipSuccess ||
+        hipEventCreateWithFlags(&e.chain, hipEventDisableTiming) != hipSuccess) {
       set_error("usc_set_wgrad_lane: hipEventCreate failed");
       return USC_ERR_LAUNCH;
     }
@@ -512,6 +515,7 @@
   e.ws_bytes = lane_ws_bytes;
   e.max_rows = max_rows;
   e.dirty = false;
+  e.chain_set = false;
   return USC_OK;
 }
 
@@ -643,7 +647,9 @@
 
 int64_t usc_program_ws_bytes(const usc_step* steps, int32_t n_steps) { return 2 * program_half_bytes(steps, n_steps) + 256; }
 
-int usc_program_run(const usc_step* steps, int32_t begin, int32_t end, void* ws_all, int64_t ws_all_bytes, usc_stream_t s) {
+namespace {
+int program_run_impl(const usc_step* steps, int32_t begin, int32_t end, void* ws_all, int64_t ws_all_bytes, usc_stream_t s,
+                     hipEvent_t chain_done) {
   USC_REQUIRE(steps && begin >= 0 && end >= begin, "usc_program_run: bad step range");
   hipStream_t st = as_stream(s);
   DeferredWgrads q;
@@ -721,7 +727,11 @@
         rc = USC_ERR_ARG;
     }
   }
-  const int rc3 = flush_pending(pend, s);
+  int rc3 = flush_pending(pend, s);
+  if (chain_done && !rc && !rc3 && hipEventRecord(chain_done, st) != hipSuccess) {
+    set_error("usc_program_run_lane: recording the chain's event failed");
+    rc3 = USC_ERR_LAUNCH;
+  }
   const int rc2 = flush_deferred(q, ws, ws_bytes, s);
   if (rc) return rc;
   if (rc3) return rc3;
@@ -729,5 +739,46 @@
   USC_CHECK_LAUNCH("usc_program_run");
   return USC_OK;
 }
-
-}
+}
+
+int usc_program_run(const usc_step* steps, int32_t begin, int32_t end, void* ws_all, int64_t ws_all_bytes, usc_stream_t s) {
+  return program_run_impl(steps, begin, end, ws_all, ws_all_bytes, s, nullptr);
+}
+
+int usc_program_run_lane(const usc_step* steps, int32_t begin, int32_t end, void* ws, int64_t ws_bytes, usc_stream_t s) {
+  Lane* lane = lane_for_current_device();
+  USC_REQUIRE(lane, "usc_program_run_lane: no weight-gradient lane on this device (usc_set_wgrad_lane)");
+  USC_REQUIRE(ws != lane->ws, "usc_program_run_lane: the range needs scratch of its own, not the lane's");
+  const usc_stream_t ls = (usc_stream_t)lane->st;
+  if (!lane->held.empty() || lane->hold) { const int rc = lane_release(lane, s); if (rc) return rc; }
+  if (as_stream(s) != lane->st &&
+      (hipEventRecord(lane->fork, as_stream(s)) != hipSuccess || hipStreamWaitEvent(lane->st, lane->fork, 0) != hipSuccess)) {
+    set_error("usc_program_run_lane: putting the lane behind the caller's stream failed (event)");
+    return USC_ERR_LAUNCH;
+  }
+  lane->hold = true;
+  lane->hold_min_rows = 0;
+  lane->release_max_rows = -1;
+  lane->dirty = true;
+  lane->chain_set = false;
+  int rc = program_run_impl(steps, begin, end, ws, ws_bytes, ls, lane->chain);
+  if (rc) {
+    lane->held.clear();
+    lane->hold = false;
+    return rc;
+  }
+  lane->chain_set = true;
+  return lane_release(lane, ls);
+}
+
+int usc_wgrad_lane_wait_chain(usc_stream_t s) {
+  Lane* lane = lane_for_current_device();
+  USC_REQUIRE(lane && lane->chain_set, "usc_wgrad_lane_wait_chain: no range has been issued on the lane (usc_program_run_lane)");
+  if (as_stream(s) != lane->st && hipStreamWaitEvent(as_stream(s), lane->chain, 0) != hipSuccess) {
+    set_error("usc_wgrad_lane_wait_chain: waiting for the chain's event failed");
+    return USC_ERR_LAUNCH;
+  }
+  return USC_OK;
+}
+
+}
diff --git a/unscene3d_amd/models/mask3d.py b/unscene3d_amd/models/mask3d.py
--- a/unscene3d_amd/models/mask3d.py
+++ b/unscene3d_amd/models/mask3d.py
@@ -266,11 +266,16 @@
                                            is_eval=is_eval)
         coordinates, coords, pos_encodings_pcd = geo["coordinates"], geo["coords"], geo["pos_encodings_pcd"]
 
-        mask_features = self.mask_features_head(pcd_features)
+        early = self._early_stage(pcd_features, aux, point2segment)
+        with (torch.no_grad() if early is not None else contextlib.nullcontext()):
+            mask_features = self.mask_features_head(pcd_features)
         mask_segments, seg_csr = None, None
         if self.train_on_segments:
             seg_csr = geo["seg_csr"]
-            if self.scatter_type == "mean":
+            if early is not None:
+                with torch.no_grad():
+                    mask_segments = [ops.segment_mean(f, csr) for f, csr in zip(mask_features.decomposed_features, seg_csr)]
+            elif self.scatter_type == "mean":
                 mask_segments = [ops.segment_mean(f, csr) for f, csr in zip(mask_features.decomposed_features, seg_csr)]
             else:
                 mask_segments = [_segment_max(f, csr.seg, csr.S) for f, csr in zip(mask_features.decomposed_features, seg_csr)]
@@ -399,6 +404,8 @@
                                                       point2segment=p2s_arg, coords=coords, defer_class=True)
         predictions_class.append(output_class)
         predictions_mask.append(outputs_mask)
+        if early is not None:
+            predictions_mask = _early_stage_gate(self, early, pcd_features, mask_features, seg_csr, predictions_mask)
         predictions_class = list(self.class_embed_head(torch.stack(predictions_class)).unbind(0))
 
         return {
@@ -408,6 +415,27 @@
             "sampled_coords": _host_array(sampled_coords) if sampled_coords is not None else None,
             "backbone_features": pcd_features,
         }
+
+    def _early_stage(self, pcd_features, aux, point2segment):
+        from .. import program
+        feats = pcd_features.F
+        handle = program.handle_of(feats)
+        if not (self.training and torch.is_grad_enabled() and self.train_on_segments and self.scatter_type == "mean"
+                and not self.use_np_features and point2segment is not None and feats.is_cuda
+                and feats.dtype == torch.float32 and self.mask_dim % 32 == 0 and (len(aux) - 1) not in self.hlevels
+                and program.early_possible(handle)):
+            return None
+        head = self.mask_features_head
+        bias = head.bias
+        if head.kernel_volume != 1 or head.stride != 1 or ops._grad_target(head.kernel) is None:
+            return None
+        if bias is not None and (not bias.requires_grad or bias.grad is None or bias._backward_hooks
+                                 or getattr(bias, "_post_accumulate_grad_hooks", None)):
+            return None
+        cm = pcd_features.coordinate_manager
+        if not all(isinstance(sl, slice) for sl in cm.batch_slices(pcd_features._ts())):
+            return None
+        return handle
 
     def _norm_queries(self, queries):
         norm = self.decoder_norm
@@ -569,15 +597,93 @@
         pad = (-Q) % 32
         W = F.pad(mask_embed, (0, 0, 0, pad)) if pad else mask_embed
     nxt = feats
+    Wc = W.contiguous()
     if chain and feats.requires_grad and torch.is_grad_enabled():
-        out, nxt = ops.linear(feats, W.contiguous(), passthrough=True)
+        out, nxt = ops.linear(feats, Wc, passthrough=True)
     else:
-        out = ops.linear(feats, W.contiguous())
+        out = ops.linear(feats, Wc)
     if pad:
         view = out[:, :Q]
         view._usc_padded = out
         out = view
+    out._usc_embed = Wc
     return (out, nxt) if chain else out
+
+
+EARLY_STAGE_STEPS = 0
+
+
+class _EarlyStageGate(torch.autograd.Function):
+
+    @staticmethod
+    def forward(ctx, run, *tables):
+        ctx.run = run
+        return tables
+
+    @staticmethod
+    def backward(ctx, *grads):
+        run, ctx.run = ctx.run, None
+        run(grads)
+        return (None,) + grads
+
+
+def _early_stage_gate(model, handle, pcd_features, mask_features, seg_csr, predictions_mask):
+    from .. import program, units
+    tables, embeds, where = [], [], []
+    for c, per_scene in enumerate(predictions_mask):
+        for i, o in enumerate(per_scene):
+            if getattr(o, "_usc_embed", None) is None:
+                raise RuntimeError("early stage: a mask-logit table did not come from the device product")
+            tables.append(getattr(o, "_usc_padded", o))
+            embeds.append(o._usc_embed.detach())
+            where.append((c, i, o.shape[1]))
+    n_scenes = len(seg_csr)
+    head = model.mask_features_head
+    x = pcd_features.F
+    slices = pcd_features.coordinate_manager.batch_slices(pcd_features._ts())
+    d = mask_features.F.shape[1]
+    dev = x.device
+
+    def run(grads):
+        global EARLY_STAGE_STEPS
+        lane = units._lane(dev)[0]
+        ready = torch.cuda.Event()
+        ready.record()
+        lane.wait_event(ready)
+        grads = [g.contiguous() for g in grads]
+        for t in grads + embeds + [t for csr in seg_csr for t in (csr.seg, csr.seg_off)]:
+            t.record_stream(lane)
+        with torch.cuda.stream(lane), torch.no_grad():
+            dmask = torch.empty((x.shape[0], d), dtype=torch.float32, device=dev)
+            kept = [grads, embeds, dmask]
+            for i in range(n_scenes):
+                mine = [k for k, w in enumerate(where) if w[1] == i]
+                dseg = ops.linear_heads_dx([grads[k] for k in mine], [embeds[k] for k in mine])
+                csr = seg_csr[i]
+                rows = dmask[slices[i]]
+                ops.check(ops.lib.usc_segment_mean_bwd(dseg.data_ptr(), d, csr.seg.data_ptr(), csr.seg_off.data_ptr(),
+                                                       rows.shape[0], rows.data_ptr(), ops._stream()), "usc_segment_mean_bwd")
+                kept.extend((dseg, csr))
+            W = head.kernel
+            W3 = (W if W.dim() == 3 else W[None]).contiguous()
+            dfeats = ops.gather_gemm(dmask, ops.weight_transpose(W3, mirror=False), None, x.shape[0])
+            ops.wgrad(x, dmask, 1, into=ops._grad_target(W))
+            ops._grad_written(W)
+            if head.bias is not None:
+                head.bias.grad.add_(ops.colsum(dmask).view_as(head.bias.grad))
+            kept.extend((x, W3, dfeats))
+            program.early_backward(handle, dfeats, keep=kept)
+        EARLY_STAGE_STEPS += 1
+
+    outs = _EarlyStageGate.apply(run, *tables)
+    result = [list(per_scene) for per_scene in predictions_mask]
+    for t, (c, i, q) in zip(outs, where):
+        if t.shape[1] != q:
+            view = t[:, :q]
+            view._usc_padded = t
+            t = view
+        result[c][i] = t
+    return result
 
 
 def multihead_attention(mha: nn.MultiheadAttention, query, key, value, attn_mask=None, pos_q=None, pos_k=None,
diff --git a/unscene3d_amd/ops.py b/unscene3d_amd/ops.py
--- a/unscene3d_amd/ops.py
+++ b/unscene3d_amd/ops.py
@@ -1226,6 +1226,32 @@
     return dy2 @ W
 
 
+def linear_heads_dx(dys, Ws):
+    L = len(dys)
+    M, N = dys[0].shape
+    K = Ws[0].shape[1]
+    for dy, W in zip(dys, Ws):
+        _chk(dy, torch.float32, "dy")
+        _chk(W, torch.float32, "W")
+        if tuple(dy.shape) != (M, N) or tuple(W.shape) != (N, K):
+            raise RuntimeError("linear_heads_dx: every head needs dy [M, N] and W [N, K] of the same shape")
+    if _small_linear_ok(M, K, N):
+        if L > lib.usc_linear_heads_max():
+            raise RuntimeError(f"linear_heads_dx: at most {lib.usc_linear_heads_max()} heads in one launch, got {L}")
+        pd = (ctypes.c_void_p * L)(*[dy.data_ptr() for dy in dys])
+        pw = (ctypes.c_void_p * L)(*[W.data_ptr() for W in Ws])
+        dx = torch.empty((M, K), dtype=torch.float32, device=dys[0].device)
+        check(lib.usc_linear_heads_dx(pd, pw, L, M, N, K, _ptr(dx), _stream()), "usc_linear_heads_dx")
+        return dx
+    dx = None
+    rows_ok = _rows_gemm_ok(M, K, N)
+    for l in range(L - 1, -1, -1):
+        W = Ws[l]
+        p = gather_gemm(dys[l], W.view(1, N, K), None, M) if rows_ok and W.is_contiguous() else dys[l] @ W
+        dx = p if dx is None else p.add_(dx)
+    return dx
+
+
 class _LinearRows(torch.autograd.Function):
     @staticmethod
     def forward(ctx, x, W, b, relu=False, passthrough=False, pad_rows_to=None):
diff --git a/unscene3d_amd/program.py b/unscene3d_amd/program.py
--- a/unscene3d_amd/program.py
+++ b/unscene3d_amd/program.py
@@ -111,6 +111,15 @@
                     seen.add(id(p))
                     params.append(p)
     pl.params = params
+    pl.early_from = None
+    if model._UP:
+        last = (model._UP[-1][0], model._UP[-1][2])
+        k = len(pl.ops)
+        while k > 0 and pl.ops[k - 1]["stage"] in last:
+            k -= 1
+        first = pl.ops[k] if k < len(pl.ops) else None
+        if first is not None and first["t"] == "unit" and first["kind"] == UP and first["x"] == pl.levels[-2]:
+            pl.early_from = k
     return pl
 
 
@@ -186,10 +195,14 @@
     return pl
 
 
+_N_PLAIN_ARGS = 8
+
+
 class _Trunk(torch.autograd.Function):
     @staticmethod
-    def forward(ctx, model, pl, cm, ts, bf16, split, feats, *params):
+    def forward(ctx, model, pl, cm, ts, bf16, split, holder, feats, *params):
         dev = feats.device
+        settle_abandoned(dev)
         rows = [cm.coord_map(ts << l).n for l in range(pl.n_levels)]
         floats = sum(r * f for r, f in zip(rows, pl.act_floats)) + pl.stat_floats + (pl.n_act + 8) * _ALIGN
         car = _Carver(floats, dev)
@@ -249,10 +262,14 @@
         check(lib.usc_program_run(steps, 0, len(pl.ops), ws.data_ptr(), ws.numel(), ops._stream()), "usc_program_run")
         outs = tuple(car.view(offs[b], rows[pl.bufs[b][0]], pl.bufs[b][1]) for b in pl.levels)
         ctx.state = (model, pl, cm, ts, feats, car, ptr, stats_ptr, kmaps, bnrefs, rows, split)
+        ctx.holder = holder
+        if holder is not None:
+            holder.state = ctx.state
         return outs
 
     @staticmethod
     def backward(ctx, *gouts):
+        holder = ctx.holder
         model, pl, cm, ts, feats, car, ptr, stats_ptr, kmaps, bnrefs, rows, split = ctx.state
         dev = feats.device
         gar = _Pool(dev, max(rows[0] * 256, 1 << 20))
@@ -261,118 +278,32 @@
             gar.release = lambda p_, n_: None
             car.arena.record_stream(lane[0])
         keep = [g.contiguous() if g is not None else None for g in gouts]
-        G = {}
-        held_dy = []
-        for b, g in zip(pl.levels, keep):
-            if g is not None:
-                G[b] = [g.data_ptr(), True, g.numel()]
-        steps = (Step * (3 * len(pl.ops) + 8))()
-        ns = 0
-        segments, cur_params, stage = [], [], None
-
-        def add_step(dst, src, n):
-            nonlocal ns
-            st = steps[ns]
-            ns += 1
-            st.op, st.dst, st.a, st.n = STEP_ADD, dst, src, n
-
-        def contribute(bid, numel, can_accumulate):
-            cur = G.get(bid)
-            if cur is None:
-                p = gar.take(numel)
-                G[bid] = [p, False, numel]
-                return p, 0, None
-            if can_accumulate and not cur[1]:
-                return cur[0], 1, None
-            p = gar.take(numel)
-            if cur[1]:
-                def fin(p=p, old=cur[0]):
-                    add_step(p, old, numel)
-                    G[bid] = [p, False, numel]
-            else:
-                def fin(p=p, old=cur[0]):
-                    add_step(old, p, numel)
-                    gar.release(p, numel)
-            return p, 0, fin
-
-        def consumed(bid):
-            cur = G.pop(bid, None)
-            if cur is not None and not cur[1]:
-                gar.release(cur[0], cur[2])
-
-        for i in range(len(pl.ops) - 1, -1, -1):
-            op = pl.ops[i]
-            if op["stage"] != stage:
-                if stage is not None:
-                    segments.append((ns, cur_params))
-                    cur_params = []
-                    for p_, n_ in held_dy:
-                        gar.release(p_, n_)
-                    held_dy = []
-                stage = op["stage"]
-            if op["t"] == "cat":
-                g = G.get(op["out"])
+        early = _take_early(holder)
+        stream = ops._stream()
+        if early is None:
+            walk = _BackwardWalk(ctx.state, gar, {})
+            for b, g in zip(pl.levels, keep):
+                if g is not None:
+                    walk.G[b] = [g.data_ptr(), True, g.numel()]
+            hi = len(pl.ops)
+        else:
+            check(lib.usc_wgrad_lane_wait_chain(stream), "usc_wgrad_lane_wait_chain")
+            walk = _BackwardWalk(ctx.state, gar, early["G"])
+            for b, g in zip(pl.levels[:-1], keep[:-1]):
                 if g is None:
                     continue
-                n = rows[op["level"]]
-                pa, _, fa = contribute(op["a"], n * op["ca"], False)
-                cur_b = G.get(op["b"])
-                if cur_b is not None and not cur_b[1]:
-                    pb, acc_b, fb = cur_b[0], 1, None
+                cur = walk.G.get(b)
+                if cur is None:
+                    walk.G[b] = [g.data_ptr(), True, g.numel()]
                 else:
-                    pb, acc_b, fb = contribute(op["b"], n * op["cb"], False)
-                st = steps[ns]
-                ns += 1
-                st.op, st.a, st.dst, st.dst2, st.n, st.ca, st.cb, st.accumulate = STEP_SPLIT, g[0], pa, pb, n, op["ca"], \
-                    op["cb"], acc_b
-                for f in (fa, fb):
-                    if f is not None:
-                        f()
-                consumed(op["out"])
-                continue
-            g = G.get(op["out"])
-            if g is None:
-                continue
-            n_out, n_in, cin, cout = rows[op["lout"]], rows[op["lin"]], op["cin"], op["cout"]
-            pdy = gar.take(n_out * cout)
-            pres, fres = None, None
-            if op["res"] is not None:
-                pres, _, fres = contribute(op["res"], n_out * cout, False)
-            need_dx = op["x"] != pl.input
-            pdx, acc, fdx = (None, 0, None)
-            if need_dx:
-                pdx, acc, fdx = contribute(op["x"], n_in * cin, op["kind"] != DOWN)
-            conv, bn = op["conv"], op["bn"]
-            tW, tg, tb = ops._grad_target(conv.kernel), ops._grad_target(bn.weight), ops._grad_target(bn.bias)
-            if tW is None or tg is None or tb is None:
-                raise RuntimeError("step program: a parameter lost its in-place gradient target between forward and "
-                                   "backward (keep p.grad allocated: optimizer.zero_grad(set_to_none=False))")
-            st = steps[ns]
-            ns += 1
-            st.op, st.kind, st.cin, st.cout = STEP_UNIT_BWD, op["kind"], cin, cout
-            st.map, st.bn = C.addressof(kmaps[i].struct), bnrefs[i][0]
-            st.x, st.W = ptr[op["x"]], conv.kernel.data_ptr()
-            st.y, st.stats = ptr[op["y"]], stats_ptr[i]
-            st.out = ptr[op["out"]] if op["relu"] else None
-            st.dout, st.dy, st.dres, st.dx, st.dx_accumulate = g[0], pdy, pres, pdx, acc
-            st.dW, st.dW_accumulate, st.dgamma, st.dbeta, st.dbn_accumulate = tW.data_ptr(), 1, tg.data_ptr(), \
-                tb.data_ptr(), 1
-            st.defer_wgrad = int(units.GROUP_WGRAD)
-            if split:
-                st.split_planes = split.get(i, 0)
-            cur_params.extend((conv.kernel, bn.weight, bn.bias))
-            for f in (fres, fdx):
-                if f is not None:
-                    f()
-            consumed(op["out"])
-            if st.defer_wgrad and op["kind"] == SAME and op["kvol"] > 1:
-                held_dy.append((pdy, n_out * cout))
-            else:
-                gar.release(pdy, n_out * cout)
-        segments.append((ns, cur_params))
+                    walk.add_step(cur[0], g.data_ptr(), g.numel())
+            hi = pl.early_from
+            ops._grad_written(*early["params"])
+            ops._params_final(early["params"])
+        walk.emit(hi, 0)
+        steps, ns, segments = walk.steps, walk.ns, walk.segments
         wsb = lib.usc_program_ws_bytes(steps, ns)
         ws = units.workspace(wsb, dev)
-        stream = ops._stream()
         begin = 0
         holding = lane is not None and units.LANE_HOLD_MIN_ROWS > units.LANE_RELEASE_ROWS > 0 and \
             any(min(rows[o["lin"]], rows[o["lout"]]) <= units.LANE_RELEASE_ROWS for o in pl.ops if o["t"] == "unit")
@@ -403,8 +334,228 @@
             for t in gar.chunks:
                 t.record_stream(lane[0])
             units.queue_lane_join(units._dev_key(dev))
+        if early is not None:
+            _close_early(early, dev)
+        if holder is not None:
+            holder.state = None
         ctx.state = None
-        return (None, None, None, None, None, None, None) + (None,) * len(pl.params)
+        return (None,) * _N_PLAIN_ARGS + (None,) * len(pl.params)
+
+
+class _BackwardWalk:
+
+    def __init__(self, state, gar, G):
+        self.state, self.gar, self.G = state, gar, G
+        pl = state[1]
+        self.steps = (Step * (3 * len(pl.ops) + 8))()
+        self.ns = 0
+        self.segments = []
+
+    def add_step(self, dst, src, n):
+        st = self.steps[self.ns]
+        self.ns += 1
+        st.op, st.dst, st.a, st.n = STEP_ADD, dst, src, n
+
+    def emit(self, hi, lo):
+        model, pl, cm, ts, feats, car, ptr, stats_ptr, kmaps, bnrefs, rows, split = self.state
+        G, gar, steps, add_step = self.G, self.gar, self.steps, self.add_step
+        held_dy = []
+        cur_params, stage = [], None
+
+        def contribute(bid, numel, can_accumulate):
+            cur = G.get(bid)
+            if cur is None:
+                p = gar.take(numel)
+                G[bid] = [p, False, numel]
+                return p, 0, None
+            if can_accumulate and not cur[1]:
+                return cur[0], 1, None
+            p = gar.take(numel)
+            if cur[1]:
+                def fin(p=p, old=cur[0]):
+                    add_step(p, old, numel)
+                    G[bid] = [p, False, numel]
+            else:
+                def fin(p=p, old=cur[0]):
+                    add_step(old, p, numel)
+                    gar.release(p, numel)
+            return p, 0, fin
+
+        def consumed(bid):
+            cur = G.pop(bid, None)
+            if cur is not None and not cur[1]:
+                gar.release(cur[0], cur[2])
+
+        for i in range(hi - 1, lo - 1, -1):
+            op = pl.ops[i]
+            if op["stage"] != stage:
+                if stage is not None:
+                    self.segments.append((self.ns, cur_params))
+                    cur_params = []
+                    for p_, n_ in held_dy:
+                        gar.release(p_, n_)
+                    held_dy = []
+                stage = op["stage"]
+            if op["t"] == "cat":
+                g = G.get(op["out"])
+                if g is None:
+                    continue
+                n = rows[op["level"]]
+                pa, _, fa = contribute(op["a"], n * op["ca"], False)
+                cur_b = G.get(op["b"])
+                if cur_b is not None and not cur_b[1]:
+                    pb, acc_b, fb = cur_b[0], 1, None
+                else:
+                    pb, acc_b, fb = contribute(op["b"], n * op["cb"], False)
+                st = steps[self.ns]
+                self.ns += 1
+                st.op, st.a, st.dst, st.dst2, st.n, st.ca, st.cb, st.accumulate = STEP_SPLIT, g[0], pa, pb, n, op["ca"], \
+                    op["cb"], acc_b
+                for f in (fa, fb):
+                    if f is not None:
+                        f()
+                consumed(op["out"])
+                continue
+            g = G.get(op["out"])
+            if g is None:
+                continue
+            n_out, n_in, cin, cout = rows[op["lout"]], rows[op["lin"]], op["cin"], op["cout"]
+            pdy = gar.take(n_out * cout)
+            pres, fres = None, None
+            if op["res"] is not None:
+                pres, _, fres = contribute(op["res"], n_out * cout, False)
+            need_dx = op["x"] != pl.input
+            pdx, acc, fdx = (None, 0, None)
+            if need_dx:
+                pdx, acc, fdx = contribute(op["x"], n_in * cin, op["kind"] != DOWN)
+            conv, bn = op["conv"], op["bn"]
+            tW, tg, tb = ops._grad_target(conv.kernel), ops._grad_target(bn.weight), ops._grad_target(bn.bias)
+            if tW is None or tg is None or tb is None:
+                raise RuntimeError("step program: a parameter lost its in-place gradient target between forward and "
+                                   "backward (keep p.grad allocated: optimizer.zero_grad(set_to_none=False))")
+            st = steps[self.ns]
+            self.ns += 1
+            st.op, st.kind, st.cin, st.cout = STEP_UNIT_BWD, op["kind"], cin, cout
+            st.map, st.bn = C.addressof(kmaps[i].struct), bnrefs[i][0]
+            st.x, st.W = ptr[op["x"]], conv.kernel.data_ptr()
+            st.y, st.stats = ptr[op["y"]], stats_ptr[i]
+            st.out = ptr[op["out"]] if op["relu"] else None
+            st.dout, st.dy, st.dres, st.dx, st.dx_accumulate = g[0], pdy, pres, pdx, acc
+            st.dW, st.dW_accumulate, st.dgamma, st.dbeta, st.dbn_accumulate = tW.data_ptr(), 1, tg.data_ptr(), \
+                tb.data_ptr(), 1
+            st.defer_wgrad = int(units.GROUP_WGRAD)
+            if split:
+                st.split_planes = split.get(i, 0)
+            cur_params.extend((conv.kernel, bn.weight, bn.bias))
+            for f in (fres, fdx):
+                if f is not None:
+                    f()
+            consumed(op["out"])
+            if st.defer_wgrad and op["kind"] == SAME and op["kvol"] > 1:
+                held_dy.append((pdy, n_out * cout))
+            else:
+                gar.release(pdy, n_out * cout)
+        self.segments.append((self.ns, cur_params))
+
+
+EARLY_STAGE = os.environ.get("USC3D_EARLY_STAGE", "1") == "1"
+EARLY_RUNS = 0
+_EARLY_WS = {}
+_EARLY_OPEN = {}
+
+
+class TrunkHandle:
+
+    __slots__ = ("state", "early", "__weakref__")
+
+    def __init__(self):
+        self.state, self.early = None, None
+
+
+def handle_of(s1_features):
+    return getattr(s1_features, "_usc_trunk", None)
+
+
+def early_possible(handle):
+    if not (EARLY_STAGE and handle is not None and handle.state is not None and handle.early is None):
+        return False
+    if ops.GRAD_WRITTEN_HOOK is not None:
+        return False
+    return units._lane(handle.state[4].device) is not None
+
+
+def _early_ws(nbytes, device):
+    key = units._dev_key(device)
+    ws = _EARLY_WS.get(key)
+    if ws is None or ws.numel() < nbytes:
+        ws = _EARLY_WS[key] = torch.empty(int(nbytes * 1.25) + (1 << 20), dtype=torch.uint8, device=device)
+    return ws
+
+
+def early_backward(handle, g_s1, keep=()):
+    global EARLY_RUNS
+    if not early_possible(handle):
+        raise RuntimeError("program.early_backward: not possible for this forward pass (program.early_possible)")
+    model, pl, cm, ts, feats, car, ptr, stats_ptr, kmaps, bnrefs, rows, split = handle.state
+    dev = feats.device
+    lane_st = units._lane(dev)[0]
+    key = units._dev_key(dev)
+    settle_abandoned(dev)
+    g = g_s1.contiguous()
+    if tuple(g.shape) != (rows[0], pl.bufs[pl.levels[-1]][1]) or g.dtype != torch.float32:
+        raise RuntimeError("program.early_backward: the gradient does not have the s1 output's shape")
+    gar = _Pool(dev, max(rows[0] * 256, 1 << 20))
+    gar.release = lambda p_, n_: None
+    walk = _BackwardWalk(handle.state, gar, {pl.levels[-1]: [g.data_ptr(), True, g.numel()]})
+    walk.emit(len(pl.ops), pl.early_from)
+    car.arena.record_stream(lane_st)
+    g.record_stream(lane_st)
+    for t in gar.chunks:
+        t.record_stream(lane_st)
+    ws = _early_ws(lib.usc_program_ws_bytes(walk.steps, walk.ns), dev)
+    ws.record_stream(lane_st)
+    state = {"task": ops._graph_task(), "G": walk.G, "keep": [gar, g, walk.steps, ws, handle.state, list(keep)], "key": key,
+             "params": [p for _, plist in walk.segments for p in plist]}
+    _EARLY_OPEN[key] = state
+    try:
+        check(lib.usc_program_run_lane(walk.steps, 0, walk.ns, ws.data_ptr(), ws.numel(), ops._stream()),
+              "usc_program_run_lane")
+    except BaseException:
+        lib.usc_wgrad_lane_hold(-1, 0, 0, None)
+        raise
+    handle.early = state
+    EARLY_RUNS += 1
+    units.queue_lane_join(key)
+
+
+def _take_early(holder):
+    early = None if holder is None else holder.early
+    if early is None:
+        return None
+    holder.early = None
+    if early["task"] >= 0 and early["task"] != ops._graph_task():
+        raise RuntimeError("step program: the last stage was issued ahead in another backward pass than this one")
+    return early
+
+
+def _close_early(early, dev):
+    _EARLY_OPEN.pop(early["key"], None)
+    kept = early["keep"]
+    if ops._graph_task() >= 0:
+        torch.autograd.Variable._execution_engine.queue_callback(kept.clear)
+
+
+def settle_abandoned(device=None):
+    key = units._dev_key(device)
+    state = _EARLY_OPEN.pop(key, None)
+    if state is None:
+        return False
+    lib.usc_wgrad_lane_hold(-1, 0, 0, None)
+    with torch.cuda.device(key):
+        units.join_lane()
+    state["G"] = None
+    state["keep"].clear()
+    return True
 
 
 def trunk(model, x):
@@ -430,4 +581,8 @@
                 if planes:
                     split[i] = planes
         split = split or None
-    return list(_Trunk.apply(model, pl, cm, ts, bf16, split, feats, *pl.params))
+    holder = TrunkHandle() if (EARLY_STAGE and torch.is_grad_enabled() and pl.early_from is not None) else None
+    outs = list(_Trunk.apply(model, pl, cm, ts, bf16, split, holder, feats, *pl.params))
+    if holder is not None and holder.state is not None:
+        outs[-1]._usc_trunk = holder
+    return outs
```
